# yz-cnsdqz/PSI-release

Measured on AMD Instinct MI355X. Metric: fitting iters/sec (SMPL-X+SDF+Chamfer), PROX-E batch=32, higher is better.
Workload: dtype f32

## Files before the change

### psi-release_amd/csrc/fit.hip

```cpp
#include "psi_internal.h"
#include "blob.h"
#ifdef PSI_HEAD_STOPS
__device__ int psi_dbg_sstop;
#define PSI_SSTOP(k) do { if (psi_dbg_sstop == (k)) return; } while (0)
__device__ int psi_dbg_pstop;
#define PSI_PSTOP(k) do { if (psi_dbg_pstop == (k)) asm volatile("s_endpgm"); } while (0)
__device__ int psi_dbg_cstop;
#define PSI_CSTOP() do { if (psi_dbg_cstop) asm volatile("s_endpgm"); } while (0)
#define PSI_TRACE(lo, hi) PsiBlockTrace trace_((lo), (hi))
__device__ unsigned long long psi_dbg_tl[4 * 8192];
__device__ unsigned long long psi_dbg_tlw[2 * 4 * 8192];
struct PsiBlockTrace {
    unsigned long long t0;
    int kind;
    int sel_lo, sel_hi;
    __device__ PsiBlockTrace(int lo = 9, int hi = 10) : t0(wall_clock64()), kind(0), sel_lo(lo), sel_hi(hi) {}
    __device__ ~PsiBlockTrace()
    {
        const unsigned bid = blockIdx.y * gridDim.x + blockIdx.x;
        if (psi_dbg_sstop < sel_lo || psi_dbg_sstop > sel_hi || bid >= 8192) return;
        if ((threadIdx.x & 63) == 0 && threadIdx.x < 256) {
            unsigned long long *w = psi_dbg_tlw + 2 * (4 * (size_t)bid + (threadIdx.x >> 6));
            w[0] = wall_clock64();
            w[1] = (unsigned long long)__builtin_amdgcn_s_getreg((31 << 11) | 4);
        }
        if (threadIdx.x != 0) return;
        unsigned long long *o = psi_dbg_tl + 4 * (size_t)bid;
        o[0] = t0;
        o[1] = wall_clock64();
        o[2] = (unsigned long long)__builtin_amdgcn_s_getreg((31 << 11) | 4) | ((unsigned long long)__builtin_amdgcn_s_getreg((31 << 11) | 20) << 32);
        o[3] = (unsigned long long)kind;
    }
};
extern "C" int psi_dbg_timeline(unsigned long long *out, int nblocks)
{
    return (int)hipMemcpyFromSymbol(out, HIP_SYMBOL(psi_dbg_tl), sizeof(unsigned long long) * 4 * (size_t)(nblocks < 8192 ? nblocks : 8192));
}
extern "C" int psi_dbg_timeline_waves(unsigned long long *out, int nblocks)
{
    return (int)hipMemcpyFromSymbol(out, HIP_SYMBOL(psi_dbg_tlw), sizeof(unsigned long long) * 8 * (size_t)(nblocks < 8192 ? nblocks : 8192));
}
#endif
#include "lbs_device.h"
#include "chain_plan.h"
#include "lbs_joint_device.h"
#include "sdf_device.h"
#include "nnindex_device.h"
#include <initializer_list>
#include <limits.h>
#include <memory>
#include <math.h>
#include <stdlib.h>
#include <string.h>
#include <type_traits>
#include <vector>

namespace {

constexpr int NH = 512;
constexpr int NZ = 32;
constexpr int NJ6 = 126;
constexpr int XD = 75;
#ifndef PSI_HEAD_THREADS
#define PSI_HEAD_THREADS 512
#endif
constexpr int HB = PSI_HEAD_THREADS;
static_assert(HB >= 384 && HB % 128 == 0, "the head / tail kernels place work on threads up to 256 + 75");
constexpr int KQ = HB / 128;
constexpr int KS3 = HB / 32;
constexpr int OS1 = HB / 8;
typedef float f4 __attribute__((ext_vector_type(4)));

struct FitDev {
    int B, V, Vpad, J, NB, n_c, m, D, align_corners, world, ncomp, nfp, nsdfblk;
    int indep;
    float w_rec, w_vp, w_contact, w_col, cconst;
    float lr, beta1, beta2, eps;
    float one_m_beta1, one_m_beta2;
    double lr_d, beta1_d, beta2_d;
    const float *W1T, *b1, *W2T, *b2, *W3T, *b3;
    const float *W1, *W2, *W3;
    const float *lhc, *rhc, *pose_mean;
    const int *vid;
    const int *cs_ptr, *cs_idx;
    const int *cs_first;
    const float *scene, *sdf, *gmin, *gmax;
    const float *sdf_cells;
    const float *Wct;
    float *x, *xhr, *cam, *adam_m, *adam_v;
    int *step;
    float *h1, *h2, *o6, *betas20, *pose, *transl, *verts, *og, *gq, *fpart, *penpart, *recpart, *vppart;
    float *cverts;
    float *g_betas, *g_pose, *g_transl, *g_rot;
    unsigned long long *hx_o6, *hx_gh1;
    unsigned *hx_epoch;
    int *hx_err;
    int hc;
#ifdef PSI_HEAD_STOPS
    int stop_h, stop_t;
#define HSTOP(k) do { if (f.stop_h == (k)) return; } while (0)
#define TSTOP(k) do { if (f.stop_t == (k)) return; } while (0)
#else
#define HSTOP(k)
#define TSTOP(k)
#endif
    int *nn_hint;
    float *history;
    int max_hist;
    int fused_bwd, ncp, ncp3;
    float *glc, *gvpc, *vpc;
    float *gtc_part;
#ifndef PSI_GV_SLOTS
#define PSI_GV_SLOTS 1024
#endif
    static_assert(PSI_GV_SLOTS >= 128, "one slot per body and class at least: fused_bwd runs batches up to 128 (merged_scene)");
    unsigned *gvbits;
    int gv_sps;
    const float *dirs_ch;
    const float *WTt_c;
    float *gA_part, *gfeat_part;
    float *spb;
    int nsv, nsv_c, nsn_m, nsn_c, spm, spc;
    unsigned long long *penmask;
    int pen_skip;
};

__device__ __forceinline__ float leaky(float v, float slope) { return v > 0.0f ? v : v * slope; }

__device__ __forceinline__ void gs_forward(const float *x6, float *R)
{
    float a1[3] = {x6[0], x6[2], x6[4]}, a2[3] = {x6[1], x6[3], x6[5]};
    float n1 = fmaxf(sqrtf(a1[0] * a1[0] + a1[1] * a1[1] + a1[2] * a1[2]), 1e-12f);
    float b1[3] = {a1[0] / n1, a1[1] / n1, a1[2] / n1};
    float d = b1[0] * a2[0] + b1[1] * a2[1] + b1[2] * a2[2];
    float u[3] = {a2[0] - d * b1[0], a2[1] - d * b1[1], a2[2] - d * b1[2]};
    float n2 = fmaxf(sqrtf(u[0] * u[0] + u[1] * u[1] + u[2] * u[2]), 1e-12f);
    float b2[3] = {u[0] / n2, u[1] / n2, u[2] / n2};
    float b3[3] = {b1[1] * b2[2] - b1[2] * b2[1], b1[2] * b2[0] - b1[0] * b2[2], b1[0] * b2[1] - b1[1] * b2[0]};
    for (int r = 0; r < 3; r++) {
        R[r * 3 + 0] = b1[r];
        R[r * 3 + 1] = b2[r];
        R[r * 3 + 2] = b3[r];
    }
}

__device__ __forceinline__ void gs_backward(const float *x6, const float *gR, float *g6)
{
    float a1[3] = {x6[0], x6[2], x6[4]}, a2[3] = {x6[1], x6[3], x6[5]};
    float n1 = fmaxf(sqrtf(a1[0] * a1[0] + a1[1] * a1[1] + a1[2] * a1[2]), 1e-12f);
    float b1[3] = {a1[0] / n1, a1[1] / n1, a1[2] / n1};
    float d = b1[0] * a2[0] + b1[1] * a2[1] + b1[2] * a2[2];
    float u[3] = {a2[0] - d * b1[0], a2[1] - d * b1[1], a2[2] - d * b1[2]};
    float n2 = fmaxf(sqrtf(u[0] * u[0] + u[1] * u[1] + u[2] * u[2]), 1e-12f);
    float b2[3] = {u[0] / n2, u[1] / n2, u[2] / n2};
    float gb1[3] = {gR[0], gR[3], gR[6]}, gb2[3] = {gR[1], gR[4], gR[7]}, gb3[3] = {gR[2], gR[5], gR[8]};
    gb1[0] += b2[1] * gb3[2] - b2[2] * gb3[1];
    gb1[1] += b2[2] * gb3[0] - b2[0] * gb3[2];
    gb1[2] += b2[0] * gb3[1] - b2[1] * gb3[0];
    gb2[0] += gb3[1] * b1[2] - gb3[2] * b1[1];
    gb2[1] += gb3[2] * b1[0] - gb3[0] * b1[2];
    gb2[2] += gb3[0] * b1[1] - gb3[1] * b1[0];
    float p = b2[0] * gb2[0] + b2[1] * gb2[1] + b2[2] * gb2[2];
    float gu[3] = {(gb2[0] - b2[0] * p) / n2, (gb2[1] - b2[1] * p) / n2, (gb2[2] - b2[2] * p) / n2};
    float q = gu[0] * b1[0] + gu[1] * b1[1] + gu[2] * b1[2];
    float ga2[3] = {gu[0] - b1[0] * q, gu[1] - b1[1] * q, gu[2] - b1[2] * q};
    for (int i = 0; i < 3; i++) gb1[i] += -d * gu[i] - q * a2[i];
    float r = b1[0] * gb1[0] + b1[1] * gb1[1] + b1[2] * gb1[2];
    float ga1[3] = {(gb1[0] - b1[0] * r) / n1, (gb1[1] - b1[1] * r) / n1, (gb1[2] - b1[2] * r) / n1};
    g6[0] = ga1[0]; g6[2] = ga1[1]; g6[4] = ga1[2];
    g6[1] = ga2[0]; g6[3] = ga2[1]; g6[5] = ga2[2];
}

__device__ __forceinline__ void rotmat_to_aa(const float *R, float *aa)
{
    const float m00 = R[0], m01 = R[3], m02 = R[6], m10 = R[1], m11 = R[4], m12 = R[7], m20 = R[2], m21 = R[5], m22 = R[8];
    float q[4], t;
    if (m22 < 1e-6f) {
        if (m00 > m11) {
            t = 1 + m00 - m11 - m22;
            q[0] = m12 - m21; q[1] = t; q[2] = m01 + m10; q[3] = m20 + m02;
        } else {
            t = 1 - m00 + m11 - m22;
            q[0] = m20 - m02; q[1] = m01 + m10; q[2] = t; q[3] = m12 + m21;
        }
    } else {
        if (m00 < -m11) {
            t = 1 - m00 - m11 + m22;
            q[0] = m01 - m10; q[1] = m20 + m02; q[2] = m12 + m21; q[3] = t;
        } else {
            t = 1 + m00 + m11 + m22;
            q[0] = t; q[1] = m12 - m21; q[2] = m20 - m02; q[3] = m01 - m10;
        }
    }
    float sc = sqrtf(t);
    for (int i = 0; i < 4; i++) q[i] = q[i] / sc * 0.5f;
    float s2 = q[1] * q[1] + q[2] * q[2] + q[3] * q[3];
    float s = sqrtf(s2);
    float two_theta = 2.0f * (q[0] < 0.0f ? atan2f(-s, -q[0]) : atan2f(s, q[0]));
    float k = s2 > 0.0f ? two_theta / s : 2.0f;
    aa[0] = q[1] * k; aa[1] = q[2] * k; aa[2] = q[3] * k;
}

__device__ __forceinline__ float block_sum(float v, float *sh)
{
#pragma unroll
    for (int o = 32; o > 0; o >>= 1) v += __shfl_down(v, o, 64);
    __syncthreads();
    if ((threadIdx.x & 63) == 0) sh[threadIdx.x >> 6] = v;
    __syncthreads();
    float s = 0;
    for (int i = 0; i < (int)(blockDim.x >> 6); i++) s += sh[i];
    return s;
}

__device__ __forceinline__ void block_sum2(float &a, float &c, float *sh2)
{
#pragma unroll
    for (int o = 32; o > 0; o >>= 1) {
        a += __shfl_down(a, o, 64);
        c += __shfl_down(c, o, 64);
    }
    __syncthreads();
    if ((threadIdx.x & 63) == 0) {
        sh2[2 * (threadIdx.x >> 6)] = a;
        sh2[2 * (threadIdx.x >> 6) + 1] = c;
    }
    __syncthreads();
    float sa = 0, sc = 0;
    for (int i = 0; i < (int)(blockDim.x >> 6); i++) {
        sa += sh2[2 * i];
        sc += sh2[2 * i + 1];
    }
    a = sa;
    c = sc;
}

__device__ __forceinline__ void hx_put(unsigned long long *p, float v, unsigned tag)
{
    __hip_atomic_store(p, ((unsigned long long)tag << 32) | (unsigned long long)__float_as_uint(v), __ATOMIC_RELAXED, __HIP_MEMORY_SCOPE_AGENT);
}
__device__ __forceinline__ unsigned long long hx_peek(unsigned long long *p)
{
    return __hip_atomic_load(p, __ATOMIC_RELAXED, __HIP_MEMORY_SCOPE_AGENT);
}
constexpr int HX_MAX_POLLS = 1 << 20;
__device__ __forceinline__ float hx_value(unsigned long long *p, unsigned long long w, unsigned tag, int *err)
{
    int polls = 0;
    while ((unsigned)(w >> 32) != tag) {
        if (++polls > HX_MAX_POLLS) {
            *err = 1;
            break;
        }
        __builtin_amdgcn_s_sleep(1);
        w = hx_peek(p);
    }
    return __uint_as_float((unsigned)w);
}

template <int C, bool LINKS_IN_HEAD>
__global__ __launch_bounds__(HB) void head_fwd_kernel(FitDev f, PsiLbsView lv)
{
    constexpr int NS = NH / C;
    constexpr int NQ = NS / 4;
    constexpr int KSPL = HB / NQ;
    constexpr int KPER = NH / KSPL;
    constexpr int KPER3 = NS / KS3;
    constexpr int K1 = NZ / KQ;
    constexpr int PRE2 = C > 1 ? 16 : 0;
    constexpr int PRE3 = C > 1 ? (KPER3 < 4 ? KPER3 : 4) : 0;
    static_assert(KPER % 16 == 0 && KPER3 >= 1 && NS >= 64, "cluster too wide for the thread layout");
    const int b = blockIdx.x / C, c = blockIdx.x % C, t = threadIdx.x;
    const bool last = c == C - 1;
    __shared__ float sx[XD + 5], sh1[NH], sh2[NS], so6[128], red[HB / 64], spose[PSI_JP * 3], sbetas[32], sJ[PSI_JP][3];
    __shared__ f4 part4[HB], part3[KS3][32];
    const int og1 = t & 127, kq1 = t >> 7, og2 = t % NQ, ks2 = t / NQ, og3 = t & 31, ks3 = t >> 5;
    const float *w1 = f.W1T + (size_t)(kq1 * K1) * NH + og1 * 4;
    const float *w2 = f.W2T + (size_t)(ks2 * KPER) * NH + c * NS + og2 * 4;
    const float *w3 = f.W3T + (size_t)(c * NS + ks3 * KPER3) * 128 + og3 * 4;
    f4 w1p[K1], w2p[PRE2 ? PRE2 : 1], w3p[PRE3 ? PRE3 : 1];
#pragma unroll
    for (int k = 0; k < K1; k++) w1p[k] = *(const f4 *)(w1 + (size_t)k * NH);
#pragma unroll
    for (int k = 0; k < PRE2; k++) w2p[k] = *(const f4 *)(w2 + (size_t)k * NH);
#pragma unroll
    for (int k = 0; k < PRE3; k++) w3p[k] = *(const f4 *)(w3 + (size_t)k * 128);
    const float *x = f.x + (size_t)b * XD;
    if (t < XD) sx[t] = x[t];
    if (t >= 64 && t < 96) sbetas[t - 64] = t - 64 < 10 ? x[9 + (t - 64)] : 0.0f;
    unsigned tag = 0;
    float pm[3] = {0, 0, 0}, b3v = 0.0f;
    PsiJump jp;
    for (int r = 0; r < PSI_NJUMP; r++) jp.a[r] = -1;
    if (C > 1) tag = f.hx_epoch[b] + 1u;
    f4 b1v = {0, 0, 0, 0};
    if (t < 128) b1v = *(const f4 *)(f.b1 + t * 4);
    const float b2v = t < NS ? f.b2[c * NS + t] : 0.0f;
    if (last) {
        if (t < 22)
            for (int e = 0; e < 3; e++) pm[e] = f.pose_mean[t * 3 + e];
        if (t < 128) b3v = f.b3[t];
        if (LINKS_IN_HEAD) jp = psi_load_jump(lv.m);
    }
    __syncthreads();
    HSTOP(1);
    if (c == 0) {
        float dr = t < XD ? fabsf(f.xhr[(size_t)b * XD + t] - sx[t]) : 0.0f;
        float sr = block_sum(dr, red);
        float dz = t < NZ ? sx[19 + t] * sx[19 + t] : 0.0f;
        float sz = block_sum(dz, red);
        if (t == 0) {
            f.recpart[b] = sr;
            f.vppart[b] = sz;
        }
    }
    if (last) {
        if (t >= 64 && t < 64 + 9) {
            int e = 66 + (t - 64);
            spose[e] = f.pose_mean[e];
        } else if (t >= 128 && t < 128 + 90) {
            int e = t - 128;
            const float *comp = e < 45 ? f.lhc : f.rhc;
            const float *hx = sx + (e < 45 ? 51 : 63);
            int cc = e < 45 ? e : e - 45;
            float a = 0;
            for (int i = 0; i < f.ncomp; i++) a += hx[i] * comp[i * 45 + cc];
            spose[75 + e] = a + f.pose_mean[75 + e];
        }
        psi_pose_fwd_rest(lv.m, sbetas, sJ);
    }
    HSTOP(2);
    const float *z = sx + 19;
    {
        f4 a = {0, 0, 0, 0};
#pragma unroll
        for (int k = 0; k < K1; k++) a += w1p[k] * z[kq1 * K1 + k];
        part4[kq1 * 128 + og1] = a;
    }
    __syncthreads();
    if (t < 128) {
        f4 a = b1v;
#pragma unroll
        for (int q = 0; q < KQ; q++) a += part4[q * 128 + t];
        for (int e = 0; e < 4; e++) sh1[t * 4 + e] = leaky(a[e], 0.2f);
    }
    __syncthreads();
    HSTOP(3);
    {
        f4 a0 = {0, 0, 0, 0}, a1 = {0, 0, 0, 0};
        const float *h = sh1 + ks2 * KPER;
#pragma unroll
        for (int k = 0; k < PRE2; k += 2) {
            a0 += w2p[k] * h[k];
            a1 += w2p[k + 1] * h[k + 1];
        }
#pragma unroll 8
        for (int k = PRE2; k < KPER; k += 2) {
            a0 += *(const f4 *)(w2 + (size_t)k * NH) * h[k];
            a1 += *(const f4 *)(w2 + (size_t)(k + 1) * NH) * h[k + 1];
        }
        part4[ks2 * NQ + og2] = a0 + a1;
    }
    __syncthreads();
    if (t < NS) {
        float a = b2v;
        const float *p = (const float *)part4;
#pragma unroll
        for (int q = 0; q < KSPL; q++) a += p[q * NS + t];
        a = leaky(a, 0.2f);
        sh2[t] = a;
        f.h2[(size_t)b * NH + c * NS + t] = a;
    }
    if (c == 0)
        for (int o = t; o < NH; o += HB) f.h1[(size_t)b * NH + o] = sh1[o];
    __syncthreads();
    HSTOP(4);
    {
        f4 a = {0, 0, 0, 0};
        const float *h = sh2 + ks3 * KPER3;
#pragma unroll
        for (int k = 0; k < PRE3; k++) a += w3p[k] * h[k];
#pragma unroll
        for (int k = PRE3; k < KPER3; k++) a += *(const f4 *)(w3 + (size_t)k * 128) * h[k];
        part3[ks3][og3] = a;
    }
    __syncthreads();
    HSTOP(5);
    if (t < 128) {
        float a = 0.0f;
        const float *p = (const float *)part3;
#pragma unroll
        for (int ks = 0; ks < KS3; ks++) a += p[ks * 128 + t];
        if (C == 1) {
            so6[t] = a + b3v;
        } else if (!last) {
            hx_put(f.hx_o6 + ((size_t)b * C + c) * 128 + t, a, tag);
        } else {
            unsigned long long *p8 = f.hx_o6 + (size_t)b * C * 128 + t;
            unsigned long long w[C - 1 ? C - 1 : 1];
#pragma unroll
            for (int cc = 0; cc < C - 1; cc++) w[cc] = hx_peek(p8 + cc * 128);
            float o = b3v;
#pragma unroll
            for (int cc = 0; cc < C - 1; cc++) o += hx_value(p8 + cc * 128, w[cc], tag, f.hx_err);
            so6[t] = o + a;
        }
    }
    if (C > 1 && !last) return;
    __syncthreads();
    HSTOP(6);
    if (t < NJ6) f.o6[(size_t)b * 128 + t] = so6[t];
    if (t < 22) {
        float R[9], aa[3];
        gs_forward(t == 0 ? sx + 3 : so6 + (t - 1) * 6, R);
        rotmat_to_aa(R, aa);
        for (int e = 0; e < 3; e++) spose[t * 3 + e] = aa[e] + pm[e];
    }
    __syncthreads();
    HSTOP(7);
    if constexpr (LINKS_IN_HEAD) {
        psi_pose_fwd_chain(lv.m, spose, nullptr, f.B, b, sJ, jp, lv.feat, lv.R, lv.G, lv.A, nullptr);
    } else {
        float R[9];
        psi_pose_fwd_rot(lv.m, spose, b, t, lv.feat, lv.R, R);
    }
    HSTOP(8);
    psi_pose_fwd_rest_store(lv.m, sbetas, f.B, b, sJ, lv.feat, lv.Jl);
    for (int i = t; i < f.J * 3; i += HB) f.pose[(size_t)b * f.J * 3 + i] = spose[i];
    if (t < f.NB) f.betas20[(size_t)b * f.NB + t] = sbetas[t];
    if (t >= 64 && t < 67) f.transl[(size_t)b * 3 + (t - 64)] = sx[t - 64];
    if (C > 1 && t == 0) f.hx_epoch[b] = tag;
}

struct SdfPenEpilogue {
    PsiSdfGrid G;
    const float *sdf, *gmin, *gmax;
    float *og, *penpart;
    int D, align_corners, Vpad;
    const int *contact_of;
    float s[2];
    bool neg[2];
    float *cverts;
    const int *cs_ptr, *cs_idx;
    int n_c;
    float *gl, *gvp, *gtp;
    int Npad, B;
    float gm[2][3], gs[2][3];
    float gvmax[2];
    unsigned *gmaxp;
    int gv_sps;
    unsigned long long *penmask;
    __device__ __forceinline__ void store(float *verts, size_t body_off, int b, int v, unsigned v12, float x, float y, float z) const
    {
        if (!contact_of) {
            if (verts) psi_st(verts + body_off, v12, psi_p3{x, y, z});
            return;
        }
        const int cw = psi_ld<int>(contact_of, (unsigned)v * 4u);
        if (!(cw >> 24)) return;
        float *row = cverts + (size_t)b * n_c * 3;
        psi_st(row, (unsigned)(cw & 0xffffff) * 12u, psi_p3{x, y, z});
        if ((cw >> 24) > 1)
            for (int ci = cs_ptr[v] + 1; ci < cs_ptr[v + 1]; ci++) psi_st(row, (unsigned)cs_idx[ci] * 12u, psi_p3{x, y, z});
    }
    __device__ __forceinline__ void vertex(int n, int b, int v, float x, float y, float z, bool live) { vertex_at(G, n, b, v, x, y, z, live); }
    __device__ __forceinline__ void vertex_at(const PsiSdfGrid &G, int n, int b, int v, float x, float y, float z, bool live)
    {
        s[n] = 0.0f;
        neg[n] = false;
#pragma unroll
        for (int a = 0; a < 3; a++) gm[n][a] = 0.0f;
        if (!live) return;
        float g[3];
        if (G.cells) {
            bool in[3];
            const float val = psi_sdf_sample_cells(G, x, y, z, g, in);
            neg[n] = val < 0.0f;
#pragma unroll
            for (int a = 0; a < 3; a++) g[a] = (neg[n] && in[a]) ? g[a] : 0.0f;
            s[n] = neg[n] ? -val : 0.0f;
        } else {
            const float val = psi_trilinear(sdf, gmin, gmax, x, y, z, D, align_corners, g);
            neg[n] = val < 0.0f;
#pragma unroll
            for (int a = 0; a < 3; a++) g[a] = neg[n] ? g[a] : 0.0f;
            s[n] = neg[n] ? -val : 0.0f;
        }
        if (gl) {
#pragma unroll
            for (int a = 0; a < 3; a++) gm[n][a] = g[a];
            return;
        }
        psi_st(og + (size_t)b * Vpad * 4, (unsigned)v * 16u, f4{g[0], g[1], g[2], 0.0f});
    }
    __device__ __forceinline__ void backward(int n, int b, unsigned v12, const psi_f2 (&T2)[6], const float *C)
    {
        if (!gl) return;
        const float gx = gm[n][0], gy = gm[n][1], gz = gm[n][2];
        float lx = gx, ly = gy, lz = gz;
        if (C) {
            lx = psi_dot3(C[0], C[4], C[8], gx, gy, gz);
            ly = psi_dot3(C[1], C[5], C[9], gx, gy, gz);
            lz = psi_dot3(C[2], C[6], C[10], gx, gy, gz);
        }
        psi_st(gl + (size_t)b * Npad, v12, psi_p3{lx, ly, lz});
        const float vx = psi_dot3(T2[0].x, T2[2].x, T2[4].x, lx, ly, lz), vy = psi_dot3(T2[0].y, T2[2].y, T2[4].y, lx, ly, lz),
                    vz = psi_dot3(T2[1].x, T2[3].x, T2[5].x, lx, ly, lz);
        psi_st(gvp + (size_t)b * Npad, v12, psi_p3{vx, vy, vz});
        gvmax[n] = fmaxf(gvmax[n], fmaxf(fabsf(vx), fmaxf(fabsf(vy), fabsf(vz))));
        gs[n][0] = lx; gs[n][1] = ly; gs[n][2] = lz;
    }
    __device__ __forceinline__ void finish(int n, int b, int vblock, int nvb)
    {
        __shared__ psi_f2 red[PSI_SKIN_BLK / 64];
        __shared__ float red3[PSI_SKIN_BLK / 64][3];
        __shared__ float redm[PSI_SKIN_BLK / 64];
        const float ws = psi_wave_sum(s[n]);
        const unsigned long long negm = __builtin_amdgcn_ballot_w64(neg[n]);
        const float wc = (float)(int)__builtin_popcountll(negm);
        if ((threadIdx.x & 63) == 0) red[threadIdx.x >> 6] = (psi_f2){ws, wc};
        if (gl) {
            if ((threadIdx.x & 63) == 0) penmask[((size_t)b * nvb + vblock) * (PSI_SKIN_BLK / 64) + (threadIdx.x >> 6)] = negm;
            const float sx = psi_wave_sum(gs[n][0]), sy = psi_wave_sum(gs[n][1]), sz = psi_wave_sum(gs[n][2]);
            float mx = gvmax[n];
#pragma unroll
            for (int o2 = 32; o2 > 0; o2 >>= 1) mx = fmaxf(mx, __shfl_xor(mx, o2, 64));
            if ((threadIdx.x & 63) == 0) {
                red3[threadIdx.x >> 6][0] = sx;
                red3[threadIdx.x >> 6][1] = sy;
                red3[threadIdx.x >> 6][2] = sz;
                redm[threadIdx.x >> 6] = mx;
            }
        }
        __syncthreads();
        if (gl && threadIdx.x == 64) {
            float mx = redm[0];
#pragma unroll
            for (int w = 1; w < PSI_SKIN_BLK / 64; w++) mx = fmaxf(mx, redm[w]);
            if (mx > 0.0f) atomicMax(gmaxp + (size_t)b * gv_sps + (vblock & (gv_sps - 1)), __float_as_uint(mx));
        }
        if (threadIdx.x == 0) {
            psi_f2 a = red[0];
#pragma unroll
            for (int w = 1; w < PSI_SKIN_BLK / 64; w++) a += red[w];
            *(psi_f2 *)(penpart + ((size_t)b * nvb + vblock) * 2) = a;
        }
        if (gl && threadIdx.x < 3) {
            float a = 0.0f;
#pragma unroll
            for (int w = 0; w < PSI_SKIN_BLK / 64; w++) a += red3[w][threadIdx.x];
            gtp[((size_t)vblock * B + b) * 4 + threadIdx.x] = a;
        }
    }
};

struct SdfPenEpilogueScenes : SdfPenEpilogue {
    const PsiSdfGrid *gtab;
    const int *slot;
    PsiSdfGrid Gb[2];
    template <int NB>
    __device__ __forceinline__ void load_grids(int b0, int B)
    {
#pragma unroll
        for (int n = 0; n < NB; n++) Gb[n] = gtab[slot[min(b0 + n, B - 1)]];
    }
    __device__ __forceinline__ void vertex(int n, int b, int v, float x, float y, float z, bool live) { vertex_at(Gb[n], n, b, v, x, y, z, live); }
};

template <bool SCENES>
using SdfEpilogue = std::conditional_t<SCENES, SdfPenEpilogueScenes, SdfPenEpilogue>;

template <bool SCENES>
static inline SdfEpilogue<SCENES> make_sdf_epilogue(const FitDev &f, const PsiSdfGrid &G, bool contact_vertices_only, const PsiLbsView *bwd,
                                                    const PsiSdfGrid *gtab = nullptr, const int *slot = nullptr)
{
    SdfEpilogue<SCENES> e;
    static_cast<SdfPenEpilogue &>(e) = {SCENES ? PsiSdfGrid{} : G, f.sdf, f.gmin, f.gmax, f.og, f.penpart, f.D, f.align_corners, f.Vpad,
                                        contact_vertices_only ? f.cs_first : nullptr, {0.0f, 0.0f}, {false, false}, f.cverts, f.cs_ptr, f.cs_idx, f.n_c,
                                        nullptr, nullptr, nullptr, 0, f.B, {}, {}, {0.0f, 0.0f}, f.gvbits, f.gv_sps, nullptr};
    if (bwd) {
        e.penmask = f.penmask;
        e.gl = bwd->gl;
        e.gvp = bwd->g_vp;
        e.gtp = bwd->gt_part_w;
        e.Npad = bwd->m.Npad;
    }
    if constexpr (SCENES) {
        e.gtab = gtab;
        e.slot = slot;
        e.Gb[0] = e.Gb[1] = PsiSdfGrid{};
    }
    return e;
}

template <int LPQ>
__device__ __forceinline__ void psi_contact_part_sums(float x, float (&out)[psi_sum_parts_per_wave(LPQ)])
{
    x += psi_dpp<0xB1, 0xf>(x);
    x += psi_dpp<0x4E, 0xf>(x);
    x += psi_dpp<0x124, 0xf>(x);
    x += psi_dpp<0x128, 0xf>(x);
    x += psi_dpp<0x142, 0xa>(x);
    if (psi_sum_part_lanes(LPQ) == 64) x += psi_dpp<0x143, 0xc>(x);
#pragma unroll
    for (int p = 0; p < psi_sum_parts_per_wave(LPQ); p++)
        out[p] = __builtin_bit_cast(float, __builtin_amdgcn_readlane(__builtin_bit_cast(int, x), psi_sum_last_lane(LPQ, p)));
}

template <int LPQ, int SPW = 1>
struct ContactSkinSrc {
    static_assert(LPQ == 2 || LPQ == 4, "the query's lane group skins its own vertex with 2 or 4 lanes");
    static_assert(SPW == 1 || (SPW == 2 && LPQ == 2), "two slices per workgroup: the 2-lane search");
    static constexpr int NT = SPW * psikd::kd_threads(LPQ);
    static constexpr int NST = (PSI_JP * 6 + NT - 1) / NT;
    static constexpr int CT0 = NT == 128 ? 80 : 128;
    FitDev f;
    LbsDev m;
    const float *As, *v_posed;
    psi_f2 (*sA)[6];
    psi_f2 st[NST];
    float ct;
    int v;
    float px, py, pz;
    float *sCT;
    static constexpr int NWQ = PSI_JP / 4 - 2, NWE = 10;
    f4 wq[NWE];
    int jslot;
    float (*sTR)[9] = nullptr;
    float gvm = 0.0f;
    float gs[3] = {0.0f, 0.0f, 0.0f};
    int bq = 0;
    bool live = false;
    __device__ __forceinline__ void issue(int b, int j, bool active)
    {
        jslot = j;
        bq = b;
        live = active;
#pragma unroll
        for (int q = 0; q < NST; q++) {
            const int idx = threadIdx.x + q * NT;
            st[q] = idx < m.J * 6 ? psi_ld<psi_f2>(As + (size_t)b * m.J * 12, (unsigned)idx * 8u) : (psi_f2){0.0f, 0.0f};
        }
        const int k = (int)threadIdx.x - CT0;
        ct = 0.0f;
        if (k >= 0 && k < 12) ct = f.cam[(size_t)b * 16 + k];
        else if (k >= 12 && k < 15) ct = f.transl[(size_t)b * 3 + (k - 12)];
        v = f.vid[j];
    }
    __device__ __forceinline__ void fetch(int b)
    {
        const psi_p3 p = psi_ld<psi_p3>(v_posed + (size_t)b * m.Npad, (unsigned)v * 12u);
        px = p.x; py = p.y; pz = p.z;
        const f4 *wrow = (const f4 *)(f.Wct + (size_t)jslot * PSI_JP);
#pragma unroll
        for (int q = 0; q < NWE; q++) wq[q] = wrow[q];
    }
    __device__ __forceinline__ void prepare(int)
    {
        psi_f2 (*sA_)[6] = psi_transform_stage<1>()[0];
        __shared__ float sCT_[16];
        __shared__ float sTR_[SPW * psikd::kd_qpb(LPQ)][9];
#pragma unroll
        for (int q = 0; q < NST; q++) {
            const int idx = threadIdx.x + q * NT;
            if (idx < PSI_JP * 6) (&sA_[0][0])[idx] = st[q];
        }
        const int k = (int)threadIdx.x - CT0;
        if (k >= 0 && k < 16) sCT_[k] = ct;
        __syncthreads();
        sA = sA_;
        sCT = sCT_;
        sTR = sTR_;
    }
    __device__ __forceinline__ void point(int b, int j, int c, float &qx, float &qy, float &qz) const
    {
        if constexpr (LPQ == 2) {
            const f4 *wrow = (const f4 *)(f.Wct + (size_t)j * PSI_JP);
            psi_f2 T0 = {0.0f, 0.0f}, T1 = {0.0f, 0.0f}, U0 = {0.0f, 0.0f}, U1 = {0.0f, 0.0f};
#pragma unroll
            for (int q = 0; q < NWQ; q++) {
                const f4 w4 = q < NWE ? wq[q] : wrow[q];
#pragma unroll
                for (int t = 0; t < 4; t++) {
                    const psi_f2 w2 = {w4[t], w4[t]};
                    T0 = __builtin_elementwise_fma(w2, sA[q * 4 + t][2 * c], T0);
                    T1 = __builtin_elementwise_fma(w2, sA[q * 4 + t][2 * c + 1], T1);
                    U0 = __builtin_elementwise_fma(w2, sA[q * 4 + t][4], U0);
                    U1 = __builtin_elementwise_fma(w2, sA[q * 4 + t][5], U1);
                }
            }
            if (f.fused_bwd) {
                float *tr = sTR[threadIdx.x / LPQ];
                tr[3 * c] = T0.x; tr[3 * c + 1] = T0.y; tr[3 * c + 2] = T1.x;
                if (c == 0) { tr[6] = U0.x; tr[7] = U0.y; tr[8] = U1.x; }
                if (c == 0 && live) psi_st(f.vpc + (size_t)b * f.ncp3, (unsigned)j * 12u, psi_p3{px, py, pz});
            }
            const float xr = psi_dot3p(T0.x, T0.y, T1.x, T1.y, px, py, pz) + sCT[12 + c];
            const float xr2 = psi_dot3p(U0.x, U0.y, U1.x, U1.y, px, py, pz) + sCT[14];
            const int base = (threadIdx.x & 63) & ~1;
            const float x = __shfl(xr, base, 64), y = __shfl(xr, base + 1, 64), z = __shfl(xr2, base, 64);
            const float *C = sCT;
            qx = psi_dot3p(C[0], C[1], C[2], C[3], x, y, z);
            qy = psi_dot3p(C[4], C[5], C[6], C[7], x, y, z);
            qz = psi_dot3p(C[8], C[9], C[10], C[11], x, y, z);
            return;
        }
        const int r = c < 2 ? c : 2;
        const f4 *wrow = (const f4 *)(f.Wct + (size_t)j * PSI_JP);
        psi_f2 T0 = {0.0f, 0.0f}, T1 = {0.0f, 0.0f};
#pragma unroll
        for (int q = 0; q < NWQ; q++) {
            const f4 w4 = q < NWE ? wq[q] : wrow[q];
#pragma unroll
            for (int t = 0; t < 4; t++) {
                const psi_f2 w2 = {w4[t], w4[t]};
                T0 = __builtin_elementwise_fma(w2, sA[q * 4 + t][2 * r], T0);
                T1 = __builtin_elementwise_fma(w2, sA[q * 4 + t][2 * r + 1], T1);
            }
        }
        if (f.fused_bwd && c < 3) {
            float *tr = &sTR[threadIdx.x / LPQ][3 * c];
            tr[0] = T0.x; tr[1] = T0.y; tr[2] = T1.x;
        }
        float xr = psi_dot3p(T0.x, T0.y, T1.x, T1.y, px, py, pz) + sCT[12 + r];
        const int base = (threadIdx.x & 63) & ~3;
        const float x = __shfl(xr, base, 64), y = __shfl(xr, base + 1, 64), z = __shfl(xr, base + 2, 64);
        const float *C = sCT;
        qx = psi_dot3p(C[0], C[1], C[2], C[3], x, y, z);
        qy = psi_dot3p(C[4], C[5], C[6], C[7], x, y, z);
        qz = psi_dot3p(C[8], C[9], C[10], C[11], x, y, z);
    }
    __device__ __forceinline__ void contact_post(size_t, float gx, float gy, float gz)
    {
        if (!f.fused_bwd) return;
        const float *C = sCT;
        const float lx = psi_dot3(C[0], C[4], C[8], gx, gy, gz), ly = psi_dot3(C[1], C[5], C[9], gx, gy, gz), lz = psi_dot3(C[2], C[6], C[10], gx, gy, gz);
        const float *R = sTR[threadIdx.x / LPQ];
        const size_t row = (size_t)bq * f.ncp3;
        const unsigned off = (unsigned)jslot * 12u;
        psi_st(f.glc + row, off, psi_p3{lx, ly, lz});
        const float vx = psi_dot3(R[0], R[3], R[6], lx, ly, lz), vy = psi_dot3(R[1], R[4], R[7], lx, ly, lz), vz = psi_dot3(R[2], R[5], R[8], lx, ly, lz);
        psi_st(f.gvpc + row, off, psi_p3{vx, vy, vz});
        gvm = fmaxf(fabsf(vx), fmaxf(fabsf(vy), fabsf(vz)));
        if constexpr (LPQ != 2) psi_st(f.vpc + row, off, psi_p3{px, py, pz});
        gs[0] = lx; gs[1] = ly; gs[2] = lz;
    }
    __device__ __forceinline__ void contact_finish(int b, int bx, int nbx)
    {
        if (!f.fused_bwd) return;
        constexpr int PPW = psi_sum_parts_per_wave(LPQ);
        __shared__ float wsum3_[SPW == 2 ? 1 : psi_sum_parts(LPQ)][3];
        __shared__ float wmax_[SPW == 2 ? 1 : psi_sum_waves(LPQ)];
        float (*wsum3)[3] = wsum3_;
        float *wmax = wmax_;
        if constexpr (SPW == 2) {
            static_assert(sizeof(psi_f2) * 6 * PSI_JP >= sizeof(float) * (SPW * psi_sum_parts(LPQ) * 3 + SPW * psi_sum_waves(LPQ)), "the staging area holds both tables");
            float *dead = (float *)&psi_transform_stage<1>()[0][0][0];
            wsum3 = (float (*)[3])dead;
            wmax = dead + SPW * psi_sum_parts(LPQ) * 3;
        }
        const int pr = SPW == 2 ? (bx & 1) : 0, t0 = pr * psi_sum_wg_pair_threads(LPQ);
        float sx[PPW], sy[PPW], sz[PPW];
        psi_contact_part_sums<LPQ>(gs[0], sx);
        psi_contact_part_sums<LPQ>(gs[1], sy);
        psi_contact_part_sums<LPQ>(gs[2], sz);
        float mx = gvm;
#pragma unroll
        for (int o2 = 32; o2 > 0; o2 >>= 1) mx = fmaxf(mx, __shfl_xor(mx, o2, 64));
        if ((threadIdx.x & 63) == 0) {
#pragma unroll
            for (int p = 0; p < PPW; p++) {
                const unsigned s = SPW == 2 ? psi_sum_wg_slot(LPQ, SPW, threadIdx.x >> 6, p) : psi_sum_slot(LPQ, threadIdx.x >> 6, p);
                wsum3[s][0] = sx[p];
                wsum3[s][1] = sy[p];
                wsum3[s][2] = sz[p];
            }
            wmax[threadIdx.x >> 6] = mx;
        }
        __syncthreads();
        if ((int)threadIdx.x == t0 + 64) {
            float m2 = wmax[pr * psi_sum_waves(LPQ)];
#pragma unroll
            for (int w = 1; w < psi_sum_waves(LPQ); w++) m2 = fmaxf(m2, wmax[pr * psi_sum_waves(LPQ) + w]);
            if (m2 > 0.0f) atomicMax(f.gvbits + PSI_GV_SLOTS + (size_t)b * f.gv_sps + (bx & (f.gv_sps - 1)), __float_as_uint(m2));
        }
        if ((int)threadIdx.x >= t0 && (int)threadIdx.x < t0 + 3) {
            float a = 0.0f;
#pragma unroll
            for (int w = 0; w < psi_sum_parts(LPQ); w++) a += wsum3[pr * psi_sum_parts(LPQ) + w][(int)threadIdx.x - t0];
            f.gtc_part[((size_t)b * nbx + bx) * 4 + ((int)threadIdx.x - t0)] = a;
        }
    }
};

#ifdef PSI_HEAD_STOPS
extern "C" int psi_dbg_kd_mark(unsigned long long *out, int nblocks)
{
    return (int)hipMemcpyFromSymbol(out, HIP_SYMBOL(psi_kd_mark), sizeof(unsigned long long) * 4 * (size_t)(nblocks < 8192 ? nblocks : 8192));
}
extern "C" int psi_dbg_kd_reason(int *out) { return (int)hipMemcpyFromSymbol(out, HIP_SYMBOL(psi_kd_reason), sizeof(int) * 8); }
extern "C" int psi_dbg_kd_stat(int *out, int nblocks)
{
    return (int)hipMemcpyFromSymbol(out, HIP_SYMBOL(psi_kd_stat), sizeof(int) * 4 * (size_t)(nblocks < 8192 ? nblocks : 8192));
}
#endif
template <bool SCENES>
using SceneTrees = std::conditional_t<SCENES, const psikd::KdDev *__restrict__, psikd::KdDev>;

template <int NB, bool SCENES, int LPQ, int SPW>
__global__ __launch_bounds__(256, 6) void fwd_scene_kernel(FitDev f, LbsDev m, const float *__restrict__ As, const float *__restrict__ v_posed,
                                                           SceneTrees<SCENES> T, int n_kd, int nqb, int rows, float gscale, int skin_first, SdfEpilogue<SCENES> epi,
                                                           int *__restrict__ kd_stack)
{
    extern __shared__ int smem_i[];
#ifdef PSI_HEAD_STOPS
    if (psi_dbg_sstop == 1 && (int)blockIdx.x >= n_kd) return;
    if (psi_dbg_sstop == 2 && (int)blockIdx.x < n_kd) return;
    if (psi_dbg_sstop == 3) return;
    PsiBlockTrace trace;
    if (threadIdx.x < 4 && blockIdx.x < 8192) psi_kd_stat[4 * blockIdx.x + threadIdx.x] = 0;
    trace.kind = skin_first ? ((int)blockIdx.x >= (int)gridDim.x - n_kd) : ((int)blockIdx.x < n_kd);
#endif
    int bid = blockIdx.x;
    bool is_kd;
    if (skin_first) {
        const int n_sk = (int)gridDim.x - n_kd;
        is_kd = bid >= n_sk;
        if (is_kd) bid -= n_sk;
    } else {
        is_kd = bid < n_kd;
        if (!is_kd) bid -= n_kd;
    }
    if (is_kd) {
        const int b = bid / nqb, bx = bid % nqb;
        psikd::KdDev tree = psikd::KdDev();
        const psikd::KdDev *__restrict__ tab = nullptr;
        const int *slot = nullptr;
        if constexpr (SCENES) {
            tab = T;
            slot = epi.slot;
        } else tree = T;
        psikd::kd_query_body<LPQ, true, SCENES, SPW>(tree, ContactSkinSrc<LPQ, SPW>{f, m, As, v_posed, nullptr, {}, 0.0f, 0, 0.0f, 0.0f, 0.0f, nullptr, {}, 0}, f.n_c, (float *)nullptr, (int *)nullptr,
                                           f.cconst, gscale, f.fused_bwd ? (float *)nullptr : f.gq, f.fpart, f.nn_hint, rows, tab, slot, bx, b, SPW == 2 ? f.nfp : nqb, smem_i, kd_stack);
    } else {
        const int i = bid;
        if constexpr (SCENES) epi.template load_grids<NB>((i / f.nsdfblk) * NB, f.B);
        psi_skin_fwd_body<NB, PsiBlendCompact>(m, As, v_posed, f.transl, f.cam, f.B, f.verts, epi, i % f.nsdfblk, (i / f.nsdfblk) * NB, f.nsdfblk);
    }
}

template <int NB, bool SCENES>
__global__ __launch_bounds__(PSI_SKIN_BLK, 6) void skin_fwd_sdf_kernel(LbsDev m, const float *__restrict__ As, const float *__restrict__ v_posed,
                                                                     const float *__restrict__ transl, const float *__restrict__ cam_ext,
                                                                     int B, float *__restrict__ verts, SdfEpilogue<SCENES> epi)
{
    if constexpr (SCENES) epi.template load_grids<NB>((int)blockIdx.y * NB, B);
    psi_skin_fwd_body<NB, PsiBlendPipelined>(m, As, v_posed, transl, cam_ext, B, verts, epi, (int)blockIdx.x, (int)blockIdx.y * NB, (int)gridDim.x);
}

__global__ void contact_weight_table_kernel(const float *__restrict__ WT, int Vpad, const int *__restrict__ vid, int n_c, int J, float *__restrict__ Wct)
{
    const int i = blockIdx.x * 256 + threadIdx.x;
    if (i >= n_c * PSI_JP) return;
    const int slot = i / PSI_JP, j = i % PSI_JP;
    Wct[i] = j < J ? WT[(size_t)j * Vpad + vid[slot]] : 0.0f;
}

__global__ __launch_bounds__(1024) void loss_finalize_kernel(FitDev f, float *stats)
{
    __shared__ float red[16];
    const int t = threadIdx.x, nt = 1024;
    auto total = [&](const float *p, int n, int stride) {
        float a0 = 0, a1 = 0, a2 = 0, a3 = 0;
        int i = t;
        for (; i + 3 * nt < n; i += 4 * nt) {
            a0 += p[(size_t)i * stride];
            a1 += p[(size_t)(i + nt) * stride];
            a2 += p[(size_t)(i + 2 * nt) * stride];
            a3 += p[(size_t)(i + 3 * nt) * stride];
        }
        for (; i < n; i += nt) a0 += p[(size_t)i * stride];
        return block_sum((a0 + a1) + (a2 + a3), red);
    };
    float s_rec = total(f.recpart, f.B, 1);
    float s_vp = total(f.vppart, f.B, 1);
    float s_f = total(f.fpart, f.B * f.nfp, 1);
    float s_pen = total(f.penpart, f.B * f.nsdfblk, 2);
    float n_pen = total(f.penpart + 1, f.B * f.nsdfblk, 2);
    if (t == 0) {
        stats[0] = s_rec; stats[1] = s_vp; stats[2] = s_f; stats[3] = s_pen; stats[4] = n_pen; stats[5] = 0.0f;
        *f.step += 1;
    }
}

__device__ __forceinline__ void fit_stats_body(const FitDev &f, float *__restrict__ stats)
{
    __shared__ float red[16];
    const int t = threadIdx.x, nt = blockDim.x;
    if (f.indep) {
        float a0 = 0, a1 = 0, a2 = 0, a3 = 0;
        for (int b = t; b < f.B; b += nt) {
            a0 += f.recpart[b];
            a1 += f.vppart[b];
            float sf = 0, sp = 0, cn = 0;
            for (int k = 0; k < f.nfp; k++) sf += f.fpart[(size_t)b * f.nfp + k];
            for (int k = 0; k < f.nsdfblk; k++) {
                sp += f.penpart[2 * ((size_t)b * f.nsdfblk + k)];
                cn += f.penpart[2 * ((size_t)b * f.nsdfblk + k) + 1];
            }
            a2 += sf;
            a3 += cn > 0.0f ? sp / cn : 0.0f;
            f.spb[b] = cn > 0.0f ? -f.w_col / cn : 0.0f;
        }
        const float s0 = block_sum(a0, red), s1 = block_sum(a1, red), s2 = block_sum(a2, red), s3 = block_sum(a3, red);
        if (t == 0) {
            stats[0] = s0; stats[1] = s1; stats[2] = s2; stats[3] = s3; stats[4] = 0.0f; stats[5] = 0.0f;
            *f.step += 1;
        }
        return;
    }
    auto total = [&](const float *p, int n, int stride) {
        float a0 = 0, a1 = 0, a2 = 0, a3 = 0;
        int i = t;
        for (; i + 3 * nt < n; i += 4 * nt) {
            a0 += p[(size_t)i * stride];
            a1 += p[(size_t)(i + nt) * stride];
            a2 += p[(size_t)(i + 2 * nt) * stride];
            a3 += p[(size_t)(i + 3 * nt) * stride];
        }
        for (; i < n; i += nt) a0 += p[(size_t)i * stride];
        return block_sum((a0 + a1) + (a2 + a3), red);
    };
    const float s_rec = total(f.recpart, f.B, 1);
    const float s_vp = total(f.vppart, f.B, 1);
    const float s_f = total(f.fpart, f.B * f.nfp, 1);
    const float s_pen = total(f.penpart, f.B * f.nsdfblk, 2);
    const float n_pen = total(f.penpart + 1, f.B * f.nsdfblk, 2);
    if (t == 0) {
        stats[0] = s_rec; stats[1] = s_vp; stats[2] = s_f; stats[3] = s_pen; stats[4] = n_pen; stats[5] = 0.0f;
        *f.step += 1;
    }
}

#ifndef PSI_FIT_PF_MODEL
#define PSI_FIT_PF_MODEL 1
#endif
#ifndef PSI_FIT_PF_CONTACT
#define PSI_FIT_PF_CONTACT 2
#endif
template <int MT, int PF_MODEL, int PF_CONTACT>
__global__ __launch_bounds__(256) __attribute__((amdgpu_waves_per_eu(2, 2))) void fit_bwd_joint_kernel(
    FitDev f, LbsDev m, const float *__restrict__ g_vp, const float *__restrict__ gl, const float *__restrict__ v_posed, PsiSkaPlan ska, int n_blend,
    int kgroups, float *__restrict__ stats)
{
    const int n_ska = ska.n_ska;
    constexpr int SMEM_B = psi_blend_bwd_h_smem_f4<(MT + 1) / 2>();
    __shared__ f4 smem[SMEM_B > SKA_SMEM_F4 ? SMEM_B : SKA_SMEM_F4];
    const int bid = blockIdx.x;
#ifdef PSI_HEAD_STOPS
    PsiBlockTrace trace(11, 11);
    trace.kind = bid < n_ska ? (bid < ska.n_c ? 1 : 0) : (bid < n_ska + n_blend ? 2 : 4);
#endif
    if (bid < n_ska) {
        int sl, b0, nbody;
        psi_ska_map(ska, bid, sl, b0, nbody);
        float *part = f.gA_part + (size_t)sl * f.B * PSI_JP * 16;
        if (sl < f.nsv) {
            const PsiSkaSlice o = {m.WTt + (size_t)sl * 4 * PSI_JP * 64, gl + (size_t)sl * 768, v_posed + (size_t)sl * 768, (size_t)m.Npad, part};
            const unsigned all = (1u << min(nbody, f.B - b0)) - 1u;
            const unsigned live = f.pen_skip ? psi_pen_slice_live(f.penmask, f.Vpad / 64, sl, f.B, b0, nbody) : all;
            skin_bwd_A_zero(o, b0, all & ~live);
            if (live) skin_bwd_A_dispatch_live(o, b0, live, smem);
        } else {
            const int c = sl - f.nsv;
            const PsiSkaSlice o = {f.WTt_c + (size_t)c * 4 * PSI_JP * 64, f.glc + (size_t)c * 768, f.vpc + (size_t)c * 768, (size_t)f.ncp3, part};
            skin_bwd_A_dispatch(o, f.B, b0, nbody, smem);
        }
    } else if (bid < n_ska + n_blend) {
        int kg, slice, bg;
        psi_blend_bwd_place(bid - n_ska, kgroups, f.nsn_m + f.nsn_c, kg, slice, bg);
#ifdef PSI_HEAD_STOPS
        trace.kind = slice < f.nsn_m ? 2 : 3;
#endif
        float *part = f.gfeat_part + (size_t)slice * f.B * m.Kpad;
        const float dsc_inv = m.dirs_unscale * PSI_FEAT_SCALE;
        if (slice < f.nsn_m) {
            const PsiBlendBwdColsH o = {m.dirs_bh, g_vp, (size_t)m.Npad, m.Kpad, m.Npad / 16, f.gvbits, f.gv_sps, dsc_inv, f.pen_skip ? f.penmask : nullptr, f.Vpad / 64};
            blend_bwd_h_body<(MT + 1) / 2, PF_MODEL>(o, f.B, slice * f.spm, (slice + 1) * f.spm, part, kg, bg, smem);
        } else {
            const int c = slice - f.nsn_m;
            const PsiBlendBwdColsH o = {f.dirs_ch, f.gvpc, (size_t)f.ncp3, m.Kpad, f.ncp3 / 16, f.gvbits + PSI_GV_SLOTS, f.gv_sps, dsc_inv, nullptr, 0};
            blend_bwd_h_body<(MT + 1) / 2, PF_CONTACT>(o, f.B, c * f.spc, (c + 1) * f.spc, part, kg, bg, smem);
        }
    } else {
        fit_stats_body(f, stats);
    }
}

__global__ __launch_bounds__(256) void fit_reduce_kernel(FitDev f, PsiLbsView lv, const float *__restrict__ stats)
{
    const int B = f.B, Kpad = lv.m.Kpad;
    const long nA = (long)B * PSI_JP * 16, nF = (long)B * Kpad, nT = (long)B * 4;
    const long t = (long)blockIdx.x * 256 + threadIdx.x;
    const long i = t / PSI_RSPL;
    const int s0 = (int)(t % PSI_RSPL);
    float spg = 0.0f;
    if (!f.indep) {
        const float N = stats[4];
        spg = N > 0.0f ? -f.w_col / N : 0.0f;
    }
    if (i < nA) {
        const int b = (int)(i / (PSI_JP * 16));
        const float sp = f.indep ? f.spb[b] : spg;
        float r = 0.0f;
        if ((i & 15) < 12) {
            const float pen = psi_sum_slices_split<12>(f.gA_part + i, (size_t)nA, f.nsv, s0);
            const float con = psi_sum_slices_split<2>(f.gA_part + (size_t)f.nsv * nA + i, (size_t)nA, f.nsv_c, s0);
            r = __builtin_fmaf(sp, pen, con);
        }
        if (s0 == 0) ((float *)lv.gA)[i] = r;
    } else if (i < nA + nF) {
        const long k = i - nA;
        const int b = (int)(k / Kpad);
        const float sp = f.indep ? f.spb[b] : spg;
        const float pen = psi_sum_slices_split<8>(f.gfeat_part + k, (size_t)nF, f.nsn_m, s0);
        const float con = psi_sum_slices_split<2>(f.gfeat_part + (size_t)f.nsn_m * nF + k, (size_t)nF, f.nsn_c, s0);
        if (s0 == 0) ((float *)lv.gfeat)[k] = __builtin_fmaf(sp, pen, con);
    } else if (i < nA + nF + nT) {
        const long k = i - nA - nF;
        const int b = (int)(k >> 2), c = (int)(k & 3), cc = c < 3 ? c : 0;
        const float sp = f.indep ? f.spb[b] : spg;
        const float pen = psi_sum_slices_split<12>(lv.gt_part + (size_t)b * 4 + cc, (size_t)B * 4, lv.nvb, s0);
        const float con = psi_sum_slices_split<8>(f.gtc_part + (size_t)b * f.nfp * 4 + cc, (size_t)4, f.nfp, s0);
        if (s0 == 0 && c < 3) f.g_transl[(size_t)b * 3 + c] = __builtin_fmaf(sp, pen, con);
    }
    if (t >= 64 && t < 64 + 2 * PSI_GV_SLOTS) f.gvbits[t - 64] = 0u;
    if (t == 0) {
        const int it = *f.step - 1;
        if (it >= 0) {
            float *h = f.history + (size_t)(it % f.max_hist) * 4;
            if (f.indep) {
                h[0] = f.w_rec * stats[0] / ((float)B * XD);
                h[1] = f.w_vp * stats[1] / ((float)B * NZ);
                h[2] = f.w_contact * stats[2] / ((float)B * f.n_c);
                h[3] = f.w_col * stats[3] / (float)B;
            } else {
                const float Bg = (float)B * (float)f.world, N = stats[4];
                h[0] = f.w_rec * stats[0] / (Bg * XD);
                h[1] = f.w_vp * stats[1] / (Bg * NZ);
                h[2] = f.w_contact * stats[2] / (Bg * f.n_c);
                h[3] = N > 0.0f ? f.w_col * stats[3] / N : 0.0f;
            }
        }
    }
}

__global__ void contact_weight_tiles_kernel(const float *__restrict__ Wct, int n_c, int ncp, float *__restrict__ WTt_c)
{
    const int i = blockIdx.x * 256 + threadIdx.x;
    if (i >= ncp * PSI_JP) return;
    const int tile = i / (PSI_JP * 64), j = (i / 64) % PSI_JP, s = tile * 64 + (i & 63);
    WTt_c[i] = s < n_c ? Wct[(size_t)s * PSI_JP + j] : 0.0f;
}
__global__ void contact_dirs_h_kernel(const float *__restrict__ dirs_bh, int Kpad, const int *__restrict__ vid, int n_c, int ncp3, float *__restrict__ dirs_ch)
{
    const size_t i = (size_t)blockIdx.x * 256 + threadIdx.x, n_all = (size_t)ncp3 * Kpad;
    if (i >= n_all) return;
    const int ne = (int)(i & 7), kr = (int)((i >> 3) & 31), nh = (int)((i >> 8) & 1), KT = Kpad / 32;
    const int kt = (int)((i >> 9) % KT), s = (int)((i >> 9) / KT);
    const int n = s * 16 + nh * 8 + ne;
    const int slot = n / 3, comp = n - 3 * slot;
    _Float16 hi = (_Float16)0.0f, lo = (_Float16)0.0f;
    if (slot < n_c) {
        const int sn = 3 * vid[slot] + comp;
        const size_t so = ((((size_t)(sn >> 4) * KT + kt) * 2) * 2 + ((sn >> 3) & 1)) * 256 + (size_t)kr * 8 + (sn & 7);
        hi = ((const _Float16 *)dirs_bh)[so];
        lo = ((const _Float16 *)dirs_bh)[so + 512];
    }
    const size_t o = ((((size_t)s * KT + kt) * 2) * 2 + nh) * 256 + (size_t)kr * 8 + ne;
    ((_Float16 *)dirs_ch)[o] = hi;
    ((_Float16 *)dirs_ch)[o + 512] = lo;
}
template <bool LOCAL>
struct FitGradSource {
    FitDev f;
    float *stats;
    float N;
    float *sNb;
    int b0;
    static constexpr int NPF = 4;
    psi_f2 pp[NPF];
    bool pp_valid;
    struct Pre { float og[3], q[3]; int cw; };
    __device__ __forceinline__ Pre issue(int b, int v, bool live)
    {
        Pre p;
        p.cw = live ? psi_ld<int>(f.cs_first, (unsigned)v * 4u) : 0;
        for (int e = 0; e < 3; e++) { p.og[e] = 0.0f; p.q[e] = 0.0f; }
        if (live) {
            const f4 o = psi_ld<f4>(f.og + (size_t)b * f.Vpad * 4, (unsigned)v * 16u);
            p.og[0] = o.x; p.og[1] = o.y; p.og[2] = o.z;
        }
        pp_valid = LOCAL && !f.indep;
        if (pp_valid) {
            const int n = f.B * f.nsdfblk;
#pragma unroll
            for (int k = 0; k < NPF; k++) {
                const int i = threadIdx.x + k * PSI_SKIN_BLK;
                pp[k] = i < n ? *(const psi_f2 *)(f.penpart + 2 * (size_t)i) : (psi_f2){0.0f, 0.0f};
            }
        }
        return p;
    }
    __device__ __forceinline__ void issue_late(Pre &p, int b) const
    {
        if (p.cw >> 24) {
            const psi_p3 q = psi_ld<psi_p3>(f.gq + (size_t)b * f.n_c * 3, (unsigned)(p.cw & 0xffffff) * 12u);
            p.q[0] = q.x; p.q[1] = q.y; p.q[2] = q.z;
        }
    }
    __device__ __forceinline__ void take(const Pre &p, int b, int v, float &gx, float &gy, float &gz) const
    {
        const float Nb = sNb ? sNb[b - b0] : N;
        const float sp = Nb > 0.0f ? -f.w_col / Nb : 0.0f;
        gx = sp * p.og[0]; gy = sp * p.og[1]; gz = sp * p.og[2];
        const int cnt = p.cw >> 24;
        if (cnt) { gx += p.q[0]; gy += p.q[1]; gz += p.q[2]; }
        if (cnt > 1)
            for (int ci = f.cs_ptr[v] + 1; ci < f.cs_ptr[v + 1]; ci++) {
                const float *q = f.gq + ((size_t)b * f.n_c + f.cs_idx[ci]) * 3;
                gx += q[0]; gy += q[1]; gz += q[2];
            }
    }
    __device__ __forceinline__ void prepare(int b0_, int nb)
    {
        const int t = threadIdx.x;
        const bool first = blockIdx.x == 0 && blockIdx.y == 0;
        b0 = b0_;
        sNb = nullptr;
        __shared__ float red[4];
        if (f.indep) {
            __shared__ float sN[PSI_SKIN_MB];
            for (int i0 = 0; i0 < nb; i0 += PSI_SKIN_BLK / 64) {
                const int i = i0 + (t >> 6);
                float c = 0.0f;
                if (i < nb)
                    for (int k = t & 63; k < f.nsdfblk; k += 64) c += f.penpart[2 * ((size_t)(b0 + i) * f.nsdfblk + k) + 1];
                c = psi_wave_sum(c);
                if (i < nb && (t & 63) == 0) sN[i] = c;
            }
            __syncthreads();
            sNb = sN;
            N = 0.0f;
            if (first) {
                float a0 = 0, a1 = 0, a2 = 0, a3 = 0;
                for (int b = t; b < f.B; b += PSI_SKIN_BLK) {
                    a0 += f.recpart[b];
                    a1 += f.vppart[b];
                    float sf = 0, sp = 0, cn = 0;
                    for (int k = 0; k < f.nfp; k++) sf += f.fpart[(size_t)b * f.nfp + k];
                    for (int k = 0; k < f.nsdfblk; k++) {
                        sp += f.penpart[2 * ((size_t)b * f.nsdfblk + k)];
                        cn += f.penpart[2 * ((size_t)b * f.nsdfblk + k) + 1];
                    }
                    a2 += sf;
                    a3 += cn > 0.0f ? sp / cn : 0.0f;
                }
                const float s0 = block_sum(a0, red), s1 = block_sum(a1, red), s2 = block_sum(a2, red), s3 = block_sum(a3, red);
                if (t == 0) {
                    if (LOCAL) {
                        stats[0] = s0; stats[1] = s1; stats[2] = s2; stats[3] = s3; stats[4] = 0.0f; stats[5] = 0.0f;
                        *f.step += 1;
                    }
                    const int it = *f.step - 1;
                    if (it >= 0) {
                        float *h = f.history + (size_t)(it % f.max_hist) * 4;
                        h[0] = f.w_rec * s0 / ((float)f.B * XD);
                        h[1] = f.w_vp * s1 / ((float)f.B * NZ);
                        h[2] = f.w_contact * s2 / ((float)f.B * f.n_c);
                        h[3] = f.w_col * s3 / (float)f.B;
                    }
                }
            }
            return;
        }
        float st[5];
        if (LOCAL) {
            float a = 0, c = 0;
            int i = t;
            if (pp_valid) {
#pragma unroll
                for (int k = 0; k < NPF; k++) { a += pp[k].x; c += pp[k].y; }
                i += NPF * PSI_SKIN_BLK;
            }
            for (; i < f.B * f.nsdfblk; i += PSI_SKIN_BLK) {
                a += f.penpart[2 * i];
                c += f.penpart[2 * i + 1];
            }
            __shared__ float red2[2 * PSI_SKIN_BLK / 64];
            block_sum2(a, c, red2);
            st[3] = a;
            st[4] = c;
            if (first) {
                a = 0;
                for (int i = t; i < f.B; i += PSI_SKIN_BLK) a += f.recpart[i];
                st[0] = block_sum(a, red);
                a = 0;
                for (int i = t; i < f.B; i += PSI_SKIN_BLK) a += f.vppart[i];
                st[1] = block_sum(a, red);
                a = 0;
                for (int i = t; i < f.B * f.nfp; i += PSI_SKIN_BLK) a += f.fpart[i];
                st[2] = block_sum(a, red);
            }
        } else {
#pragma unroll
            for (int i = 0; i < 5; i++) st[i] = stats[i];
        }
        N = st[4];
        if (first && t == 0) {
            if (LOCAL) {
                stats[0] = st[0]; stats[1] = st[1]; stats[2] = st[2]; stats[3] = st[3]; stats[4] = st[4]; stats[5] = 0.0f;
                *f.step += 1;
            }
            const float Bg = (float)f.B * (float)f.world;
            int it = *f.step - 1;
            if (it >= 0) {
                float *h = f.history + (size_t)(it % f.max_hist) * 4;
                h[0] = f.w_rec * st[0] / (Bg * XD);
                h[1] = f.w_vp * st[1] / (Bg * NZ);
                h[2] = f.w_contact * st[2] / (Bg * f.n_c);
                h[3] = N > 0.0f ? f.w_col * st[3] / N : 0.0f;
            }
        }
    }
    __device__ __forceinline__ void load(int b, int v, float &gx, float &gy, float &gz) const
    {
        const float Nb = sNb ? sNb[b - b0] : N;
        const float sp = Nb > 0.0f ? -f.w_col / Nb : 0.0f;
        const f4 o = *(const f4 *)(f.og + ((size_t)b * f.Vpad + v) * 4);
        gx = sp * o.x; gy = sp * o.y; gz = sp * o.z;
        for (int ci = f.cs_ptr[v]; ci < f.cs_ptr[v + 1]; ci++) {
            const float *q = f.gq + ((size_t)b * f.n_c + f.cs_idx[ci]) * 3;
            gx += q[0]; gy += q[1]; gz += q[2];
        }
    }
};

template <int C, bool ADAM>
__global__ __launch_bounds__(HB) void head_bwd_adam_kernel(FitDev f, PsiLbsView lv, float *__restrict__ g_out)
{
    constexpr int NS = NH / C, NQ = NS / 4;
    constexpr int OSPL = HB / NQ;
    constexpr int OPER = 128 / OSPL;
    constexpr int RPER = NS / KQ;
    constexpr int O1 = NH / OS1;
    constexpr int PRE3 = C > 1 ? (OPER < 16 ? OPER : 16) : 0;
    constexpr int PRE2 = C > 1 ? 16 : 0;
    static_assert(RPER % 16 == 0, "cluster too wide for the thread layout");
    const int b = blockIdx.x / C, c = blockIdx.x % C, t = threadIdx.x;
    const bool last = c == C - 1;
    __shared__ float sx[XD + 5], sg6[128], sga2[NS], sga1[NH], sgx[XD + 5];
    __shared__ float sgbetas[32], sgpose[PSI_JP * 3], sgrot[PSI_JP * 9];
    __shared__ f4 part4[HB], part1[OS1][8];
    const int og3 = t % NQ, os3 = t / NQ, og2 = t & 127, kq2 = t >> 7, kg1 = t & 7, os1 = t >> 3;
    const int o0 = os3 * OPER, o1 = min(o0 + OPER, NJ6);
    const float *w3 = f.W3 + c * NS + og3 * 4;
    const float *w2 = f.W2 + (size_t)(c * NS + kq2 * RPER) * NH + og2 * 4;
    const float *w1 = f.W1 + (size_t)(os1 * O1) * NZ + kg1 * 4;
    f4 w3p[PRE3 ? PRE3 : 1], w2p[PRE2 ? PRE2 : 1], w1p[O1];
#pragma unroll
    for (int i = 0; i < PRE3; i++) w3p[i] = *(const f4 *)(w3 + (size_t)min(o0 + i, NJ6 - 1) * NH);
#pragma unroll
    for (int i = 0; i < PRE2; i++) w2p[i] = *(const f4 *)(w2 + (size_t)i * NH);
    const float *h1 = f.h1 + (size_t)b * NH, *h2 = f.h2 + (size_t)b * NH;
    const float h2v = t < NS ? h2[c * NS + t] : 0.0f;
    unsigned tag = 0;
    if (C > 1) tag = f.hx_epoch[f.B + b] + 1u;
    float h1v = 0.0f, xhrv = 0.0f, am = 0.0f, av = 0.0f, step_size = 0.0f, bc2_sqrt = 1.0f;
    int step = 0;
    const int ta = (int)threadIdx.x - 256;
    float o6v[6] = {0, 0, 0, 0, 0, 0}, gtv = 0.0f;
    if (t >= 1 && t < 22)
        for (int i = 0; i < 6; i++) o6v[i] = f.o6[(size_t)b * 128 + (t - 1) * 6 + i];
    if (t >= 128 && t < 128 + 3) gtv = f.g_transl[(size_t)b * 3 + (t - 128)];
    TSTOP(1);
    if (last) {
#pragma unroll
        for (int i = 0; i < O1; i++) w1p[i] = *(const f4 *)(w1 + (size_t)i * NZ);
        h1v = h1[t];
        if (ADAM && ta >= 0 && ta < XD) {
            xhrv = f.xhr[(size_t)b * XD + ta];
            am = f.adam_m[(size_t)b * XD + ta];
            av = f.adam_v[(size_t)b * XD + ta];
            step = *f.step;
            const double bc1 = 1.0 - pow(f.beta1_d, (double)step);
            const double bc2 = 1.0 - pow(f.beta2_d, (double)step);
            step_size = (float)(f.lr_d / bc1);
            bc2_sqrt = (float)sqrt(bc2);
        }
    }
    psi_pose_bwd_body(lv.m, f.pose + (size_t)b * f.J * 3, lv.R, lv.Jl, lv.G, lv.gA + (size_t)b * PSI_JP * 16, lv.gfeat + (size_t)b * lv.m.Kpad, b,
                      sgbetas, sgpose, sgrot);
    const float *x = f.x + (size_t)b * XD;
    if (t < XD) { sx[t] = x[t]; sgx[t] = 0.0f; }
    if (t < 128) sg6[t] = 0.0f;
    __syncthreads();
    TSTOP(2);
    if (c == 0) {
        for (int i = t; i < f.J * 9; i += HB) f.g_rot[(size_t)b * f.J * 9 + i] = sgrot[i];
        for (int i = t; i < f.J * 3; i += HB) f.g_pose[(size_t)b * f.J * 3 + i] = sgpose[i];
        if (t < f.NB) f.g_betas[(size_t)b * f.NB + t] = sgbetas[t];
    }
    if (t == 0) {
        float g6[6];
        gs_backward(sx + 3, sgrot, g6);
        for (int i = 0; i < 6; i++) sgx[3 + i] = g6[i];
    } else if (t >= 1 && t < 22) {
        float g6[6];
        gs_backward(o6v, sgrot + t * 9, g6);
        for (int i = 0; i < 6; i++) sg6[(t - 1) * 6 + i] = g6[i];
    } else if (t >= 64 && t < 64 + 2 * f.ncomp) {
        int i = t - 64;
        const float *comp = i < f.ncomp ? f.lhc : f.rhc;
        int ii = i < f.ncomp ? i : i - f.ncomp;
        const float *gp = sgpose + (i < f.ncomp ? 75 : 120);
        float a = 0;
        for (int e = 0; e < 45; e++) a += comp[ii * 45 + e] * gp[e];
        sgx[(i < f.ncomp ? 51 : 63) + ii] = a;
    } else if (t >= 128 && t < 128 + 3) {
        sgx[t - 128] = gtv;
    } else if (t >= 160 && t < 160 + 10) {
        sgx[9 + (t - 160)] = sgbetas[t - 160];
    }
    __syncthreads();
    TSTOP(3);
    {
        f4 a = {0, 0, 0, 0};
#pragma unroll
        for (int i = 0; i < PRE3; i++) a += w3p[i] * sg6[o0 + i];
#pragma unroll 8
        for (int o = o0 + PRE3; o < o1; o++) a += *(const f4 *)(w3 + (size_t)o * NH) * sg6[o];
        part4[os3 * NQ + og3] = a;
    }
    __syncthreads();
    if (t < NS) {
        float a = 0.0f;
        const float *p = (const float *)part4;
#pragma unroll
        for (int q = 0; q < OSPL; q++) a += p[q * NS + t];
        sga2[t] = a * (h2v > 0.0f ? 1.0f : 0.2f);
    }
    __syncthreads();
    TSTOP(4);
    {
        f4 a0 = {0, 0, 0, 0}, a1 = {0, 0, 0, 0};
        const float *g = sga2 + kq2 * RPER;
#pragma unroll
        for (int o = 0; o < PRE2; o += 2) {
            a0 += w2p[o] * g[o];
            a1 += w2p[o + 1] * g[o + 1];
        }
#pragma unroll 8
        for (int o = PRE2; o < RPER; o += 2) {
            a0 += *(const f4 *)(w2 + (size_t)o * NH) * g[o];
            a1 += *(const f4 *)(w2 + (size_t)(o + 1) * NH) * g[o + 1];
        }
        part4[kq2 * 128 + og2] = a0 + a1;
    }
    __syncthreads();
    TSTOP(5);
    {
        const float *p = (const float *)part4;
        float a = p[t];
#pragma unroll
        for (int q = 1; q < KQ; q++) a += p[q * NH + t];
        if (C == 1) {
            sga1[t] = a * (h1[t] > 0.0f ? 1.0f : 0.2f);
        } else if (!last) {
            hx_put(f.hx_gh1 + ((size_t)b * C + c) * NH + t, a, tag);
            return;
        } else {
            unsigned long long *p8 = f.hx_gh1 + (size_t)b * C * NH + t;
            unsigned long long w[C - 1 ? C - 1 : 1];
#pragma unroll
            for (int cc = 0; cc < C - 1; cc++) w[cc] = hx_peek(p8 + (size_t)cc * NH);
            float o = 0.0f;
#pragma unroll
            for (int cc = 0; cc < C - 1; cc++) o += hx_value(p8 + (size_t)cc * NH, w[cc], tag, f.hx_err);
            sga1[t] = (o + a) * (h1v > 0.0f ? 1.0f : 0.2f);
        }
    }
    __syncthreads();
    TSTOP(6);
    {
        f4 a = {0, 0, 0, 0};
        if (C == 1) {
#pragma unroll
            for (int i = 0; i < O1; i++) a += *(const f4 *)(w1 + (size_t)i * NZ) * sga1[os1 * O1 + i];
        } else {
#pragma unroll
            for (int i = 0; i < O1; i++) a += w1p[i] * sga1[os1 * O1 + i];
        }
        part1[os1][kg1] = a;
    }
    __syncthreads();
    if (t < 8) {
        f4 a = {0, 0, 0, 0};
        for (int os = 0; os < OS1; os++) a += part1[os][t];
        for (int e = 0; e < 4; e++) sgx[19 + t * 4 + e] = a[e];
    }
    __syncthreads();
    TSTOP(7);
    if (C > 1 && t == 0) f.hx_epoch[f.B + b] = tag;
    if (!ADAM) {
        if (t < XD) g_out[(size_t)b * XD + t] = sgx[t];
        return;
    }
    if (ta >= 0 && ta < XD) {
        const float Bg = f.indep ? 1.0f : (float)f.B * (float)f.world;
        float g = sgx[ta];
        float df = xhrv - sx[ta];
        g += f.w_rec / (Bg * XD) * (df > 0.0f ? -1.0f : (df < 0.0f ? 1.0f : 0.0f));
        if (ta >= 19 && ta < 19 + NZ) g += f.w_vp / (Bg * NZ) * 2.0f * sx[ta];
        size_t o = (size_t)b * XD + ta;
        float m = am * f.beta1 + f.one_m_beta1 * g;
        float v = av * f.beta2 + f.one_m_beta2 * g * g;
        f.adam_m[o] = m;
        f.adam_v[o] = v;
        float denom = sqrtf(v) / bc2_sqrt + f.eps;
        f.x[o] = sx[ta] - step_size * (m / denom);
    }
}

__global__ void sdf_to_cells_kernel(const float *__restrict__ src, float *__restrict__ dst, int D)
{
    const int nbr = D >> 2;
    const size_t i = (size_t)blockIdx.x * 256 + threadIdx.x, n = (size_t)D * D * D * 8;
    if (i >= n) return;
    const int c = (int)(i & 7), l = (int)((i >> 3) & 63);
    const size_t br = i >> 9;
    const int bz = (int)(br % nbr), by = (int)((br / nbr) % nbr), bx = (int)(br / ((size_t)nbr * nbr));
    const int ix = min(4 * bx + (l >> 4) + (c >> 2), D - 1), iy = min(4 * by + ((l >> 2) & 3) + ((c >> 1) & 1), D - 1),
              iz = min(4 * bz + (l & 3) + (c & 1), D - 1);
    dst[i] = src[((size_t)ix * D + iy) * D + iz];
}

__global__ void scene_slots_kernel(const int *__restrict__ src, int *__restrict__ dst, int B, int S)
{
    const int b = blockIdx.x * 256 + threadIdx.x;
    if (b < B) dst[b] = min(max(src[b], 0), S - 1);
}

__global__ void adam_reset_kernel(float *m, float *v, int *step, int n)
{
    int i = blockIdx.x * 256 + threadIdx.x;
    if (i < n) { m[i] = 0.0f; v[i] = 0.0f; }
    if (i == 0) *step = 0;
}

}

#ifndef PSI_FIT_SEARCH_LANES_DEFAULT
#define PSI_FIT_SEARCH_LANES_DEFAULT 2
#endif
#ifndef PSI_GRAPH_UNROLL
#define PSI_GRAPH_UNROLL 10
#endif
constexpr int GRAPH_UNROLL = PSI_GRAPH_UNROLL;

struct FitKnobs {
    bool split_scene, keep_verts, no_fused_bwd, sdf_linear, scene_skin_first, bwdv_mb, no_pen_skip, bwd_pf1, chain_in_head;
    int head_cluster, skin_nb, ska_nbody, search_lanes, search_spw;
#ifdef PSI_HEAD_STOPS
    int head_stop, tail_stop, skin_stop;
#endif
};

static FitKnobs fit_read_knobs()
{
    auto is = [](const char *name, char c) { const char *v = getenv(name); return v && v[0] == c; };
    auto num = [](const char *name) { const char *v = getenv(name); return v ? atoi(v) : 0; };
    FitKnobs k = {};
    k.split_scene = is("PSI_SPLIT_SCENE", '1');
    k.keep_verts = is("PSI_KEEP_VERTS", '1');
    k.no_fused_bwd = is("PSI_FIT_FUSED_BWD", '0');
    k.no_pen_skip = is("PSI_FIT_PEN_SKIP", '0');
    k.bwd_pf1 = is("PSI_FIT_BWD_PF", '1');
    k.chain_in_head = is("PSI_FIT_CHAIN_IN_HEAD", '1');
    k.sdf_linear = is("PSI_SDF_LINEAR", '1');
    k.scene_skin_first = is("PSI_SCENE_ORDER", '1');
    k.bwdv_mb = is("PSI_BWDV_MB", '1');
    const int hc = num("PSI_HEAD_CLUSTER");
    if (hc == 1 || hc == 2 || hc == 4 || hc == 8) k.head_cluster = hc;
    if (getenv("PSI_SKIN_NB")) k.skin_nb = num("PSI_SKIN_NB") == 2 ? 2 : 1;
    k.ska_nbody = psi_ska_nbody_override(SKA_NBODY);
    const int sl = num("PSI_FIT_SEARCH_LANES");
    if (sl == 2 || sl == 4) k.search_lanes = sl;
    if (num("PSI_FIT_SEARCH_SPW") == 1) k.search_spw = 1;
#ifdef PSI_HEAD_STOPS
    k.head_stop = num("PSI_HEAD_STOP");
    k.tail_stop = num("PSI_TAIL_STOP");
    k.skin_stop = num("PSI_SKIN_STOP");
#endif
    return k;
}

struct FitModes {
    bool self_skin;
    bool merged_scene;
    bool keep_verts;
    bool fused_bwd;
    int skin_nb;
    int search_lanes;
    int search_spw;
    int hc;
    int gv_sps;
    PsiStreamSplit split;
    PsiChainPlan chain;
};

static FitModes fit_decide(const psi_fit_config *cfg, const FitKnobs &knobs, int J, int ncp3, const PsiLbsCounts &mc, int cus)
{
    FitModes d = {};
    d.self_skin = cfg->nn_mode == 1 && J <= PSI_JP - 8 && psikd::kd_qpb(psikd::LPQ_OPS) == psikd::kd_qpb(2);
    d.search_lanes = knobs.search_lanes ? knobs.search_lanes : mc.compressed_weights ? 4 : PSI_FIT_SEARCH_LANES_DEFAULT;
    d.merged_scene = d.self_skin && cfg->B <= 128 && !knobs.split_scene;
    d.search_spw = d.search_lanes == 2 && !knobs.search_spw ? 2 : 1;
    d.keep_verts = !d.merged_scene || knobs.keep_verts;
    const long bodies = (long)cfg->B * (cfg->concurrent_engines > 1 ? cfg->concurrent_engines : 1);
    d.hc = bodies <= 32 ? 8 : bodies <= 64 ? 4 : bodies <= 128 ? 2 : 1;
    if (knobs.head_cluster) d.hc = knobs.head_cluster;
    d.gv_sps = 16;
    while (d.gv_sps > 1 && (long)d.gv_sps * cfg->B > PSI_GV_SLOTS) d.gv_sps >>= 1;
    d.split = psi_stream_split(mc.Npad / 16, ncp3 / 16, mc.nsn);
    d.fused_bwd = d.merged_scene && !knobs.no_fused_bwd && d.split.nsn_c > 0;
    d.skin_nb = cfg->B > 128 && !mc.compressed_weights ? 2 : 1;
    if (knobs.skin_nb) d.skin_nb = knobs.skin_nb;
    d.chain = knobs.chain_in_head ? PsiChainPlan{0, 0} : psi_chain_plan(cfg->B, d.hc, mc.blend_wg, mc.blend_gy, cus);
    return d;
}

struct FitPlan {
    int mt;
    int kgroups, n_blend;
    PsiSkaPlan ska;
    bool pf1;
};
static FitPlan fit_plan_make(const FitDev &f, const LbsDev &m, int ska_nbody_override, bool pf1)
{
    FitPlan p;
    p.kgroups = m.Kpad / 64;
    p.mt = f.B > 32 ? 4 : (f.B > 16 ? 2 : 1);
    p.n_blend = p.kgroups * (f.nsn_m + f.nsn_c) * psi_cdiv(f.B, 16 * p.mt);
    p.ska = psi_ska_plan(f.B, f.nsv, f.nsv_c, SKA_NBODY, ska_nbody_override);
    p.pf1 = pf1;
    return p;
}

struct FitGraph { hipGraph_t g; hipGraphExec_t exec; bool ready; };

struct FitCaptured {
    enum Kind { Ok, Refused, Error } kind;
    int rc;
};

template <class Seq>
static FitCaptured fit_graph_capture(FitGraph *G, hipStream_t st, Seq &&seq)
{
    auto failed = [](const char *what, hipError_t he) {
        psi_set_error("%s failed: %s", what, hipGetErrorString(he));
        return FitCaptured{FitCaptured::Error, (int)he};
    };
    if (!st) {
        psi_set_error("invalid argument: graph capture needs a non-default stream");
        return {FitCaptured::Error, PSI_EINVAL};
    }
    hipError_t he = hipStreamBeginCapture(st, hipStreamCaptureModeRelaxed);
    if (he != hipSuccess) return failed("begin of the stream capture", he);
    const int rc = seq();
    hipGraph_t g = nullptr;
    he = hipStreamEndCapture(st, &g);
    if (!rc && he == hipSuccess) {
        he = hipGraphInstantiate(&G->exec, g, nullptr, nullptr, 0);
        if (he != hipSuccess) {
            (void)hipGraphDestroy(g);
            return failed("hipGraphInstantiate", he);
        }
        G->g = g;
        G->ready = true;
        return {FitCaptured::Ok, 0};
    }
    if (g) (void)hipGraphDestroy(g);
    if (!rc) (void)failed("hipStreamEndCapture", he);
    const bool refused = (he >= hipErrorStreamCaptureUnsupported && he <= hipErrorStreamCaptureWrongThread) || rc == 1000 + 4 || rc == 1000 + 5;
    return {refused ? FitCaptured::Refused : FitCaptured::Error, rc ? rc : (int)he};
}

static int fit_graph_launch(const FitGraph &G, hipStream_t st)
{
    PSI_CHECK_HIP(hipGraphLaunch(G.exec, st));
    return 0;
}

static void fit_graph_drop(FitGraph *G)
{
    if (G->ready) {
        (void)hipGraphExecDestroy(G->exec);
        (void)hipGraphDestroy(G->g);
    }
    *G = FitGraph{};
}

struct FitGraphTier { int iters; FitGraph *graph; };

template <class Seq>
static FitCaptured fit_run_graphs(hipStream_t st, int n_iter, int *done, std::initializer_list<FitGraphTier> tiers, Seq &&one)
{
    for (const FitGraphTier &t : tiers) {
        if (n_iter - *done < t.iters) continue;
        if (!t.graph->ready) {
            const FitCaptured c = fit_graph_capture(t.graph, st, [&]() {
                int rc = 0;
                for (int i = 0; i < t.iters && !rc; i++) rc = one();
                return rc;
            });
            if (c.kind != FitCaptured::Ok) return c;
        }
        for (; *done + t.iters <= n_iter; *done += t.iters)
            if (int rc = fit_graph_launch(*t.graph, st)) return {FitCaptured::Error, rc};
    }
    return {FitCaptured::Ok, 0};
}

enum {
    FIT_G_ITER_1, FIT_G_ITER_N, FIT_G_ITER_2N,
    FIT_G_HALF_FWD, FIT_G_HALF_BWD,
    FIT_G_DP_1, FIT_G_DP_N,
    FIT_N_GRAPHS
};

struct psi_fit_engine {
    FitDev d;
    PsiSdfGrid grid;
    const psi_lbs_model *lbs;
    psi_nn_index *nn_index;
    float *lbs_ws;
    PsiLbsView lv;
    void *nn_ws;
    char *blob;
    PsiBlob table;
    float *stats_local;
    FitKnobs knobs;
    FitModes mode;
    FitPlan plan;
    int n_scenes;
    psi_nn_index **scene_index;
    float **scene_vol;
    char *scene_blob;
    psikd::KdDev *d_kd_tab;
    PsiSdfGrid *d_grid_tab;
    int *d_slot;
    int kd_rows;
    char *search_blob;
    int *kd_stack;
    FitGraph graphs[FIT_N_GRAPHS];
    const float *half_stats[2];
    const void *dp_comm;
    const float *dp_stats;
    bool dp_warm;
    bool dp_no_graph;
};

template <bool LINKS_IN_HEAD>
static void launch_head_fwd(const FitDev &f, const PsiLbsView &lv, hipStream_t st)
{
    const dim3 g(f.B * f.hc), blk(HB);
    switch (f.hc) {
    case 8: hipLaunchKernelGGL((head_fwd_kernel<8, LINKS_IN_HEAD>), g, blk, 0, st, f, lv); break;
    case 4: hipLaunchKernelGGL((head_fwd_kernel<4, LINKS_IN_HEAD>), g, blk, 0, st, f, lv); break;
    case 2: hipLaunchKernelGGL((head_fwd_kernel<2, LINKS_IN_HEAD>), g, blk, 0, st, f, lv); break;
    default: hipLaunchKernelGGL((head_fwd_kernel<1, true>), g, blk, 0, st, f, lv); break;
    }
}

static int fit_head_blend(psi_fit_engine *e, hipStream_t st)
{
    const FitDev &f = e->d;
    const PsiChainPlan &cp = e->mode.chain;
    const bool role = cp.n_links_wg > 0 && f.hc > 1;
    if (role) launch_head_fwd<false>(f, e->lv, st);
    else launch_head_fwd<true>(f, e->lv, st);
    PSI_CHECK_LAUNCH("head_fwd_kernel");
    psi_mark("head_fwd_kernel", st);
    return role ? psi_lbs_blend_forward_links(e->lbs, f.B, e->lbs_ws, cp.n_links_wg, cp.bodies_per_wave, st)
                : psi_lbs_blend_forward(e->lbs, f.B, e->lbs_ws, st);
}

template <bool ADAM>
static void launch_head_bwd(const FitDev &f, const PsiLbsView &lv, float *g_out, hipStream_t st)
{
    const dim3 g(f.B * f.hc), blk(HB);
    switch (f.hc) {
    case 8: hipLaunchKernelGGL((head_bwd_adam_kernel<8, ADAM>), g, blk, 0, st, f, lv, g_out); break;
    case 4: hipLaunchKernelGGL((head_bwd_adam_kernel<4, ADAM>), g, blk, 0, st, f, lv, g_out); break;
    case 2: hipLaunchKernelGGL((head_bwd_adam_kernel<2, ADAM>), g, blk, 0, st, f, lv, g_out); break;
    default: hipLaunchKernelGGL((head_bwd_adam_kernel<1, ADAM>), g, blk, 0, st, f, lv, g_out); break;
    }
}

enum class FitStats {
    Finalize,
    Backward,
    Caller
};

static inline FitStats fit_stats_source(const psi_fit_engine *e, FitStats wish)
{
    return wish == FitStats::Backward && !e->mode.fused_bwd && e->d.B >= PSI_SKIN_MB_MIN_B ? FitStats::Finalize : wish;
}

static int fit_launch_stats(psi_fit_engine *e, float *stats, hipStream_t st)
{
    hipLaunchKernelGGL(loss_finalize_kernel, dim3(1), dim3(1024), 0, st, e->d, stats);
    PSI_CHECK_LAUNCH("loss_finalize_kernel");
    psi_mark("loss_finalize_kernel", st);
    return 0;
}

template <int NB, bool SCENES, int LPQ, int SPW>
static void launch_fwd_scene(const psi_fit_engine *e, float gscale, hipStream_t st)
{
    const FitDev &f = e->d;
    const int nqb = psi_cdiv(f.nfp, SPW), n_kd = nqb * f.B, skin_first = e->knobs.scene_skin_first ? 1 : 0;
    const dim3 grid(n_kd + f.nsdfblk * psi_cdiv(f.B, NB));
    FitDev fk = f;
    if (!e->mode.keep_verts) fk.verts = nullptr;
    const auto epi = make_sdf_epilogue<SCENES>(f, e->grid, false, e->mode.fused_bwd ? &e->lv : nullptr, e->d_grid_tab, e->d_slot);
    SceneTrees<SCENES> T;
    int rows;
    if constexpr (SCENES) {
        T = e->d_kd_tab;
        rows = e->kd_rows;
    } else {
        T = psi_nn_index_dev(e->nn_index);
        rows = T.rows;
    }
    hipLaunchKernelGGL((fwd_scene_kernel<NB, SCENES, LPQ, SPW>), grid, dim3(256), psikd::kd_lds_bytes(LPQ, rows), st, fk, e->lv.m, e->lv.A, e->lv.v_posed, T, n_kd, nqb, rows,
                       gscale, skin_first, epi, e->kd_stack);
}

template <int NB, bool SCENES>
static void launch_skin_fwd_sdf(const psi_fit_engine *e, bool all_verts, hipStream_t st)
{
    const FitDev &f = e->d;
    hipLaunchKernelGGL((skin_fwd_sdf_kernel<NB, SCENES>), dim3(f.nsdfblk, psi_cdiv(f.B, NB)), dim3(PSI_SKIN_BLK), 0, st, e->lv.m, e->lv.A, e->lv.v_posed,
                       f.transl, f.cam, f.B, f.verts, make_sdf_epilogue<SCENES>(f, e->grid, !all_verts, nullptr, e->d_grid_tab, e->d_slot));
}

template <class L>
static void fit_scene_dispatch(const psi_fit_engine *e, L &&launch)
{
    using One = std::integral_constant<int, 1>;
    using Two = std::integral_constant<int, 2>;
    switch ((e->n_scenes ? 2 : 0) | (e->mode.skin_nb == 2 ? 1 : 0)) {
    case 0: launch(One{}, std::false_type{}); break;
    case 1: launch(Two{}, std::false_type{}); break;
    case 2: launch(One{}, std::true_type{}); break;
    default: launch(Two{}, std::true_type{}); break;
    }
}

static int fit_forward(psi_fit_engine *e, float *stats, hipStream_t st, FitStats who)
{
    FitDev &f = e->d;
    int rc = fit_head_blend(e, st);
    if (rc) return rc;
    float gscale = f.w_contact / ((f.indep ? 1.0f : (float)f.B * (float)f.world) * (float)f.n_c);
    if (e->nn_index && e->mode.merged_scene) {
        fit_scene_dispatch(e, [&](auto nb, auto scenes) {
            if (e->mode.search_lanes == 2 && e->mode.search_spw == 2) launch_fwd_scene<decltype(nb)::value, decltype(scenes)::value, 2, 2>(e, gscale, st);
            else if (e->mode.search_lanes == 2) launch_fwd_scene<decltype(nb)::value, decltype(scenes)::value, 2, 1>(e, gscale, st);
            else launch_fwd_scene<decltype(nb)::value, decltype(scenes)::value, 4, 1>(e, gscale, st);
        });
        PSI_CHECK_LAUNCH("fwd_scene_kernel");
        psi_mark("fwd_scene_kernel", st);
    } else {
        const bool all_verts = !e->nn_index || e->knobs.keep_verts;
        fit_scene_dispatch(e, [&](auto nb, auto scenes) { launch_skin_fwd_sdf<decltype(nb)::value, decltype(scenes)::value>(e, all_verts, st); });
        PSI_CHECK_LAUNCH("skin_fwd_sdf_kernel");
        psi_mark("skin_fwd_sdf_kernel", st);
        if (e->n_scenes)
            rc = psi_nn_index_contact_set(e->d_kd_tab, e->d_slot, e->kd_rows, all_verts ? f.verts : f.cverts, all_verts ? (long)f.V * 3 : (long)f.n_c * 3,
                                          all_verts ? f.vid : nullptr, f.B, f.n_c, f.cconst, gscale, f.gq, f.fpart, f.nn_hint, st);
        else if (e->nn_index && !all_verts)
            rc = psi_nn_index_contact(e->nn_index, f.cverts, (long)f.n_c * 3, nullptr, f.B, f.n_c, f.cconst, gscale, f.gq, f.fpart, f.nn_hint, st);
        else if (e->nn_index)
            rc = psi_nn_index_contact(e->nn_index, f.verts, (long)f.V * 3, f.vid, f.B, f.n_c, f.cconst, gscale, f.gq, f.fpart, f.nn_hint, st);
        else
            rc = psi_nn_contact(f.verts, (long)f.V * 3, f.vid, f.scene, f.B, f.n_c, f.m, e->nn_ws, f.cconst, gscale, f.gq, f.fpart, nullptr, st);
        if (rc) return rc;
    }
    return fit_stats_source(e, who) == FitStats::Finalize ? fit_launch_stats(e, stats, st) : 0;
}

static int fit_backward_joint(psi_fit_engine *e, float *stats, hipStream_t st, FitStats who)
{
    FitDev &f = e->d;
    const FitPlan &p = e->plan;
    const dim3 grid(p.ska.n_ska + p.n_blend + (fit_stats_source(e, who) == FitStats::Backward ? 1 : 0));
#define PSI_LAUNCH_FIT_JOINT(MT_, PFM_, PFC_)                                                                                      \
    hipLaunchKernelGGL((fit_bwd_joint_kernel<MT_, PFM_, PFC_>), grid, dim3(256), 0, st, f, e->lv.m, e->lv.g_vp, e->lv.gl, e->lv.v_posed, p.ska, p.n_blend, p.kgroups, stats)
#define PSI_LAUNCH_FIT_JOINT_MT(MT_)                                                                                               \
    do {                                                                                                                           \
        if (p.pf1) PSI_LAUNCH_FIT_JOINT(MT_, 1, 1);                                                                                \
        else PSI_LAUNCH_FIT_JOINT(MT_, PSI_FIT_PF_MODEL, PSI_FIT_PF_CONTACT);                                                      \
    } while (0)
    if (p.mt == 4) PSI_LAUNCH_FIT_JOINT_MT(4);
    else if (p.mt == 2) PSI_LAUNCH_FIT_JOINT_MT(2);
    else PSI_LAUNCH_FIT_JOINT_MT(1);
#undef PSI_LAUNCH_FIT_JOINT_MT
#undef PSI_LAUNCH_FIT_JOINT
    PSI_CHECK_LAUNCH("fit_bwd_joint_kernel");
    psi_mark("bwd_joint_kernel", st);
    return 0;
}

static int fit_backward_tail(psi_fit_engine *e, float *stats, hipStream_t st)
{
    FitDev &f = e->d;
    const long nred = (long)f.B * PSI_JP * 16 + (long)f.B * e->lv.m.Kpad + (long)f.B * 4;
    hipLaunchKernelGGL(fit_reduce_kernel, dim3(psi_cdiv(nred * PSI_RSPL, 256)), dim3(256), 0, st, f, e->lv, stats);
    PSI_CHECK_LAUNCH("fit_reduce_kernel");
    psi_mark("reduce_partials_kernel", st);
    launch_head_bwd<true>(f, e->lv, nullptr, st);
    PSI_CHECK_LAUNCH("head_bwd_adam_kernel");
    psi_mark("head_bwd_adam_kernel", st);
    return 0;
}

static int fit_backward(psi_fit_engine *e, float *stats, hipStream_t st, FitStats who)
{
    FitDev &f = e->d;
    if (e->mode.fused_bwd) {
        int rc = fit_backward_joint(e, stats, st, who);
        return rc ? rc : fit_backward_tail(e, stats, st);
    }
    const bool big = f.B >= PSI_SKIN_MB_MIN_B;
    const bool mb = big && (e->lv.m.Wc || e->knobs.bwdv_mb);
    const dim3 bgrid(f.nsdfblk, mb ? psi_cdiv(f.B, PSI_SKIN_MB) : f.B);
#define PSI_LAUNCH_BWD_V(...)                                                                                                      \
    hipLaunchKernelGGL((psi_skin_bwd_v_kernel<__VA_ARGS__>), bgrid, dim3(PSI_SKIN_BLK), 0, st, e->lv.m, e->lv.A, src, f.cam, f.B, e->lv.gl, e->lv.g_vp, e->lv.gt_part_w)
    if (fit_stats_source(e, who) == FitStats::Backward) {
        const FitGradSource<true> src{f, stats, 0.0f, nullptr, 0, {}, false};
        if (mb) psi_launch_skin_bwd_v_mb(e->lv.m, e->lv.A, src, f.cam, f.B, e->lv.gl, e->lv.g_vp, e->lv.gt_part_w, st);
        else PSI_LAUNCH_BWD_V(FitGradSource<true>);
    } else {
        const FitGradSource<false> src{f, stats, 0.0f, nullptr, 0, {}, false};
        if (mb) psi_launch_skin_bwd_v_mb(e->lv.m, e->lv.A, src, f.cam, f.B, e->lv.gl, e->lv.g_vp, e->lv.gt_part_w, st);
        else if (big) PSI_LAUNCH_BWD_V(FitGradSource<false>, PsiBlendPipelined);
        else PSI_LAUNCH_BWD_V(FitGradSource<false>);
    }
#undef PSI_LAUNCH_BWD_V
    PSI_CHECK_LAUNCH("skin_bwd_v_grad_kernel");
    psi_mark("skin_bwd_v_grad_kernel", st);
    int rc = psi_lbs_backward_joint_parts(e->lbs, f.B, e->lbs_ws, f.g_transl, st);
    if (rc) return rc;
    launch_head_bwd<true>(f, e->lv, nullptr, st);
    PSI_CHECK_LAUNCH("head_bwd_adam_kernel");
    psi_mark("head_bwd_adam_kernel", st);
    return 0;
}

static int fit_build_scenes(psi_fit_engine *e, const psi_fit_scene *h_scenes, int S);

static inline size_t fit_x_bytes(const FitDev &f) { return (size_t)f.B * XD * 4; }
static inline size_t fit_cam_bytes(const FitDev &f) { return (size_t)f.B * 16 * 4; }
static inline size_t fit_hint_bytes(const FitDev &f) { return (size_t)f.B * f.n_c * 4; }
static inline hipError_t fit_hints_reset(const FitDev &f, hipStream_t st) { return hipMemsetAsync(f.nn_hint, 0xff, fit_hint_bytes(f), st); }

static inline size_t sdf_cells_bytes(int D) { return (size_t)D * D * D * 32; }
static void sdf_cells_fill(const float *d_sdf, float *d_cells, int D)
{
    hipLaunchKernelGGL(sdf_to_cells_kernel, dim3((unsigned)psi_cdiv((long)(sdf_cells_bytes(D) / 4), 256)), dim3(256), 0, 0, d_sdf, d_cells, D);
}

static int fit_scene_index(psi_nn_index **out, const float *d_verts, int m, hipError_t *err)
{
    std::vector<float> hs((size_t)m * 3);
    *err = hipMemcpy(hs.data(), d_verts, hs.size() * 4, hipMemcpyDeviceToHost);
    return *err == hipSuccess ? psi_nn_index_create(out, hs.data(), m) : (int)*err;
}

template <int NB, bool SCENES, int SPW>
static size_t fwd_scene_static_lds()
{
    hipFuncAttributes a;
    if (hipFuncGetAttributes(&a, reinterpret_cast<const void *>(&fwd_scene_kernel<NB, SCENES, 2, SPW>)) != hipSuccess) {
        (void)hipGetLastError();
        return 0;
    }
    return a.sharedSizeBytes;
}
static int fit_search_shape(psi_fit_engine *e)
{
    const FitDev &f = e->d;
    const char *who = e->n_scenes ? "psi_fit_create_scenes" : "psi_fit_create";
    const int rows = e->n_scenes ? e->kd_rows : psi_nn_index_dev(e->nn_index).rows;
    int dev = 0, lds_cu = 0;
    PSI_CHECK_HIP(hipGetDevice(&dev));
    if (hipDeviceGetAttribute(&lds_cu, hipDeviceAttributeMaxSharedMemoryPerMultiprocessor, dev) != hipSuccess) {
        (void)hipGetLastError();
        lds_cu = 0;
    }
    size_t s1 = 0, s2 = 0;
    fit_scene_dispatch(e, [&](auto nb, auto scenes) {
        s1 = fwd_scene_static_lds<decltype(nb)::value, decltype(scenes)::value, 1>();
        s2 = fwd_scene_static_lds<decltype(nb)::value, decltype(scenes)::value, 2>();
    });
    e->mode.search_spw = psi_search_stack_fits(f.n_c, rows) ? psi_search_spw_for((size_t)lds_cu, s1, s2, psikd::kd_lds_bytes(2, rows), 6) : 1;
    if (e->mode.search_spw != 2) return 0;
    PsiBlob T;
    T.raw(e->kd_stack, psi_search_stack_bytes(f.B, f.n_c, rows));
    return psi_blob_realise(T, &e->search_blob, who);
}

static int fit_create(psi_fit_engine **out, const psi_lbs_model *lbs, const psi_fit_config *cfg,
                      const float *h_w1, const float *h_b1, const float *h_w2, const float *h_b2,
                      const float *h_w3, const float *h_b3, const float *h_lh_comp, const float *h_rh_comp,
                      const float *h_pose_mean, const int32_t *h_contact_ids,
                      const float *d_scene_verts, const float *d_sdf, const float *h_gmin, const float *h_gmax,
                      const psi_fit_scene *h_scenes, int S)
{
    PSI_REQUIRE(out && lbs && cfg && h_w1 && h_b1 && h_w2 && h_b2 && h_w3 && h_b3 && h_lh_comp && h_rh_comp && h_pose_mean &&
                h_contact_ids && d_scene_verts && d_sdf && h_gmin && h_gmax, "null pointer");
    int V, J, NB;
    psi_lbs_dims(lbs, &V, &J, &NB);
    PSI_REQUIRE(J == 55 && NB >= 10 && NB <= 32, "the fused engine is SMPL-X shaped (J=55, 10..32 betas)");
    PSI_REQUIRE(cfg->B > 0 && cfg->n_contact > 0 && cfg->n_contact < (1 << 24) && cfg->m_scene > 0 && cfg->D >= 2 && cfg->world_size >= 1, "bad sizes");
    PSI_REQUIRE(cfg->num_pca_comps > 0 && cfg->num_pca_comps <= 12, "1..12 hand PCA components");
    PSI_REQUIRE(!(cfg->independent_bodies && cfg->world_size > 1), "independent bodies have no cross-rank coupling: use world_size 1");
    for (int i = 0; i < 66; i++) PSI_REQUIRE(h_pose_mean[i] == 0.0f, "pose_mean must be zero for global_orient/body joints");
    for (int i = 0; i < cfg->n_contact; i++) PSI_REQUIRE(h_contact_ids[i] >= 0 && h_contact_ids[i] < V, "contact id out of range");
    PsiLbsCounts mc;
    if (int rcv = psi_lbs_counts(lbs, cfg->B, &mc)) return rcv;
    psi_fit_engine *e = new psi_fit_engine();
    std::unique_ptr<psi_fit_engine, void (*)(psi_fit_engine *)> owner(e, psi_fit_destroy);
    const FitKnobs &knobs = e->knobs = fit_read_knobs();
    e->lbs = lbs;
    FitDev &f = e->d;
    f.B = cfg->B; f.V = V; f.J = J; f.NB = NB; f.n_c = cfg->n_contact; f.m = cfg->m_scene; f.D = cfg->D;
    f.align_corners = cfg->align_corners; f.world = cfg->world_size; f.ncomp = cfg->num_pca_comps;
    f.indep = cfg->independent_bodies ? 1 : 0;
    f.w_rec = cfg->w_rec; f.w_vp = cfg->w_vposer; f.w_contact = cfg->w_contact; f.w_col = cfg->w_collision; f.cconst = cfg->contact_const;
    f.lr = cfg->lr; f.beta1 = cfg->beta1; f.beta2 = cfg->beta2; f.eps = cfg->eps;
    f.lr_d = cfg->lr_d != 0.0 ? cfg->lr_d : (double)cfg->lr;
    f.beta1_d = cfg->beta1_d != 0.0 ? cfg->beta1_d : (double)cfg->beta1;
    f.beta2_d = cfg->beta2_d != 0.0 ? cfg->beta2_d : (double)cfg->beta2;
    f.one_m_beta1 = (float)(1.0 - f.beta1_d);
    f.one_m_beta2 = (float)(1.0 - f.beta2_d);
    f.nsdfblk = psi_cdiv(V, 256);
    f.Vpad = f.nsdfblk * 256;
    f.nfp = cfg->nn_mode == 1 ? psi_nn_index_fparts(f.n_c) : psi_nn_contact_fparts(f.n_c);
    f.max_hist = cfg->max_history > 0 ? cfg->max_history : 1024;
    f.ncp = psi_cdiv(f.n_c, 256) * 256;
    f.ncp3 = 3 * f.ncp;
    f.nsv = mc.nsv;
    f.nsv_c = f.ncp / 256;
    f.scene = d_scene_verts;
    f.sdf = d_sdf;
    int dev = 0, cus = 0;
    PSI_CHECK_HIP(hipGetDevice(&dev));
    PSI_CHECK_HIP(hipDeviceGetAttribute(&cus, hipDeviceAttributeMultiprocessorCount, dev));
    const FitModes &mode = e->mode = fit_decide(cfg, knobs, J, f.ncp3, mc, cus);
    f.hc = mode.hc;
    f.gv_sps = mode.gv_sps;
    f.fused_bwd = mode.fused_bwd ? 1 : 0;
    f.pen_skip = mode.fused_bwd && !knobs.no_pen_skip ? 1 : 0;
    f.nsn_m = mode.split.nsn_m; f.nsn_c = mode.split.nsn_c; f.spm = mode.split.spm; f.spc = mode.split.spc;
#ifdef PSI_HEAD_STOPS
    f.stop_h = knobs.head_stop;
    f.stop_t = knobs.tail_stop;
    (void)hipMemcpyToSymbol(HIP_SYMBOL(psi_dbg_sstop), &knobs.skin_stop, sizeof(int));
    (void)hipMemcpyToSymbol(HIP_SYMBOL(psi_dbg_pstop), &f.stop_t, sizeof(int));
    const int cstop = knobs.head_stop == 9;
    (void)hipMemcpyToSymbol(HIP_SYMBOL(psi_dbg_cstop), &cstop, sizeof(int));
#endif
    const size_t B = (size_t)f.B;
    std::vector<float> W1T((size_t)NZ * NH), W2T((size_t)NH * NH), W3T((size_t)NH * 128, 0.0f), b3p(128, 0.0f);
    memcpy(b3p.data(), h_b3, NJ6 * 4);
    for (int o = 0; o < NH; o++) for (int k = 0; k < NZ; k++) W1T[(size_t)k * NH + o] = h_w1[(size_t)o * NZ + k];
    for (int o = 0; o < NH; o++) for (int k = 0; k < NH; k++) W2T[(size_t)k * NH + o] = h_w2[(size_t)o * NH + k];
    for (int o = 0; o < NJ6; o++) for (int k = 0; k < NH; k++) W3T[(size_t)k * 128 + o] = h_w3[(size_t)o * NH + k];
    std::vector<int> cs_ptr(V + 1, 0), cs_idx(f.n_c), cs_first(V, 0);
    for (int i = 0; i < f.n_c; i++) cs_ptr[h_contact_ids[i] + 1]++;
    for (int v = 0; v < V; v++) cs_ptr[v + 1] += cs_ptr[v];
    {
        std::vector<int> fill(cs_ptr.begin(), cs_ptr.end() - 1);
        for (int i = 0; i < f.n_c; i++) cs_idx[fill[h_contact_ids[i]]++] = i;
        for (int v = 0; v < V; v++)
            if (cs_ptr[v + 1] > cs_ptr[v]) cs_first[v] = cs_idx[cs_ptr[v]] | (std::min(cs_ptr[v + 1] - cs_ptr[v], 127) << 24);
    }
    const size_t hand_pca = (size_t)f.ncomp * 45 * 4, hidden = B * NH * 4, betas = B * NB * 4, pose = B * J * 3 * 4, transl = B * 3 * 4,
                 crows = B * f.n_c * 3 * 4, per_body = B * 4, slot_rows = B * f.ncp3 * 4;
    PsiBlob &T = e->table;
    T.upload(f.W1T, W1T.data(), W1T.size() * 4);
    T.upload(f.b1, h_b1, NH * 4);
    T.upload(f.W2T, W2T.data(), W2T.size() * 4);
    T.upload(f.b2, h_b2, NH * 4);
    T.upload(f.W3T, W3T.data(), W3T.size() * 4);
    T.upload(f.b3, b3p.data(), 128 * 4);
    T.upload(f.W1, h_w1, (size_t)NH * NZ * 4);
    T.upload(f.W2, h_w2, (size_t)NH * NH * 4);
    T.upload(f.W3, h_w3, (size_t)NJ6 * NH * 4);
    T.upload(f.lhc, h_lh_comp, hand_pca);
    T.upload(f.rhc, h_rh_comp, hand_pca);
    T.upload(f.pose_mean, h_pose_mean, (size_t)J * 3 * 4);
    T.upload(f.vid, h_contact_ids, (size_t)f.n_c * sizeof(int32_t));
    T.upload(f.cs_ptr, cs_ptr.data(), cs_ptr.size() * sizeof(int));
    T.upload(f.cs_idx, cs_idx.data(), cs_idx.size() * sizeof(int));
    T.upload(f.cs_first, cs_first.data(), cs_first.size() * sizeof(int));
    T.upload(f.gmin, h_gmin, 12);
    T.upload(f.gmax, h_gmax, 12);
    T.zero_begin = T.size;
    T.zero(f.x, fit_x_bytes(f));
    T.zero(f.xhr, fit_x_bytes(f));
    T.zero(f.cam, fit_cam_bytes(f));
    T.zero(f.adam_m, fit_x_bytes(f), "adam_m");
    T.zero(f.adam_v, fit_x_bytes(f), "adam_v");
    T.zero(f.step, 256);
    T.zero(f.h1, hidden);
    T.zero(f.h2, hidden);
    T.zero(f.o6, B * 128 * 4);
    T.zero(f.betas20, betas);
    T.zero(f.pose, pose, "pose");
    T.zero(f.transl, transl);
    T.zero(f.verts, B * V * 3 * 4, "verts");
    T.zero(f.cverts, crows);
    T.zero(f.og, B * f.Vpad * 4 * 4);
    T.zero(f.gq, crows);
    T.zero(f.fpart, B * f.nfp * 4, "fpart");
    T.zero(f.penpart, B * f.nsdfblk * 2 * 4);
    T.zero(f.recpart, per_body);
    T.zero(f.vppart, per_body);
    T.zero(f.g_betas, betas);
    T.zero(f.g_pose, pose, "g_pose");
    T.zero(f.g_transl, transl, "g_transl");
    T.zero(f.g_rot, B * J * 9 * 4, "g_rot");
    T.zero(f.history, (size_t)f.max_hist * 4 * 4);
    T.zero(e->stats_local, 256);
    T.ones(f.nn_hint, fit_hint_bytes(f), "nn_hint");
    T.zero(f.hx_o6, B * f.hc * 128 * 8);
    T.zero(f.hx_gh1, B * f.hc * NH * 8);
    T.zero(f.hx_epoch, 2 * B * 4);
    T.zero(f.Wct, (size_t)f.n_c * PSI_JP * 4);
    if (mode.fused_bwd) {
        T.zero(f.glc, slot_rows, "glc");
        T.zero(f.gvpc, slot_rows, "gvpc");
        T.zero(f.vpc, slot_rows, "vpc");
        T.zero(f.gtc_part, B * f.nfp * 4 * 4, "gtc_part");
        T.zero(f.gvbits, 2 * PSI_GV_SLOTS * 4);
        T.zero(f.WTt_c, (size_t)f.ncp * PSI_JP * 4);
        T.zero(f.dirs_ch, (size_t)f.ncp3 * mc.Kpad * 4);
        T.zero(f.gA_part, (size_t)(f.nsv + f.nsv_c) * B * PSI_JP * 16 * 4);
        T.zero(f.gfeat_part, (size_t)(f.nsn_m + f.nsn_c) * B * mc.Kpad * 4);
        T.zero(f.spb, per_body, "spb");
        T.zero(f.penmask, B * (f.Vpad / 64) * 8, "penmask");
    }
    const bool cells = !h_scenes && psi_sdf_cells_fit(f.D) && !knobs.sdf_linear;
    if (cells) T.zero(f.sdf_cells, sdf_cells_bytes(f.D));
    T.zero(e->lbs_ws, psi_lbs_workspace_floats(lbs, f.B) * 4);
    T.zero(e->nn_ws, psi_nn_ws_bytes(f.B, f.n_c, f.m));
    if (int rc = psi_blob_realise(T, &e->blob, "psi_fit_create")) return rc;
    f.hx_err = f.step + 1;
    if (int rcv = psi_lbs_view(lbs, f.B, e->lbs_ws, &e->lv)) return rcv;
    e->plan = fit_plan_make(f, e->lv.m, knobs.ska_nbody, knobs.bwd_pf1);
    hipLaunchKernelGGL(contact_weight_table_kernel, dim3(psi_cdiv((long)f.n_c * PSI_JP, 256)), dim3(256), 0, 0, e->lv.m.WT, e->lv.m.Vpad, f.vid,
                       f.n_c, J, (float *)f.Wct);
    if (mode.fused_bwd) {
        hipLaunchKernelGGL(contact_weight_tiles_kernel, dim3(psi_cdiv((long)f.ncp * PSI_JP, 256)), dim3(256), 0, 0, f.Wct, f.n_c, f.ncp, (float *)f.WTt_c);
        hipLaunchKernelGGL(contact_dirs_h_kernel, dim3(psi_cdiv((long)f.ncp3 * e->lv.m.Kpad, 256)), dim3(256), 0, 0, e->lv.m.dirs_bh, e->lv.m.Kpad, f.vid,
                           f.n_c, f.ncp3, (float *)f.dirs_ch);
    }
    if (cells) sdf_cells_fill(d_sdf, (float *)f.sdf_cells, f.D);
    e->grid = psi_sdf_grid_make(f.sdf_cells, h_gmin, h_gmax, f.D, f.align_corners);
    hipError_t err = hipDeviceSynchronize();
    if (err == hipSuccess) err = hipGetLastError();
    if (err != hipSuccess) {
        psi_set_error("psi_fit_create: layout kernels failed: %s", hipGetErrorString(err));
        return (int)err;
    }
    if (h_scenes) {
        if (int rc = fit_build_scenes(e, h_scenes, S)) return rc;
    } else if (cfg->nn_mode == 1) {
        if (int rc = fit_scene_index(&e->nn_index, d_scene_verts, f.m, &err)) return rc;
    }
    if (e->nn_index && mode.merged_scene && mode.search_spw == 2)
        if (int rc = fit_search_shape(e)) return rc;
    owner.release();
    *out = e;
    return 0;
}

extern "C" int psi_fit_create(psi_fit_engine **out, const psi_lbs_model *lbs, const psi_fit_config *cfg,
                              const float *h_w1, const float *h_b1, const float *h_w2, const float *h_b2,
                              const float *h_w3, const float *h_b3, const float *h_lh_comp, const float *h_rh_comp,
                              const float *h_pose_mean, const int32_t *h_contact_ids,
                              const float *d_scene_verts, const float *d_sdf, const float *h_gmin, const float *h_gmax)
{
    return fit_create(out, lbs, cfg, h_w1, h_b1, h_w2, h_b2, h_w3, h_b3, h_lh_comp, h_rh_comp, h_pose_mean, h_contact_ids, d_scene_verts, d_sdf,
                      h_gmin, h_gmax, nullptr, 0);
}

static int fit_build_scenes(psi_fit_engine *e, const psi_fit_scene *h_scenes, int S)
{
    FitDev &f = e->d;
    e->n_scenes = S;
    e->scene_index = new psi_nn_index *[S]();
    e->scene_vol = new float *[S]();
    std::vector<psikd::KdDev> kd(S);
    std::vector<PsiSdfGrid> grids(S);
    for (int s = 0; s < S; s++) {
        const psi_fit_scene &sc = h_scenes[s];
        const int D = sc.D;
        const size_t bytes = sdf_cells_bytes(D);
        hipError_t err = hipMalloc((void **)&e->scene_vol[s], bytes);
        if (err != hipSuccess) {
            (void)hipGetLastError();
            e->scene_vol[s] = nullptr;
            psi_set_error("psi_fit_create_scenes: no memory for the copy of scene %d's volume (%zu bytes, 8 x the volume): %s", s, bytes, hipGetErrorString(err));
            return PSI_ENOMEM;
        }
        sdf_cells_fill(sc.d_sdf, e->scene_vol[s], D);
        grids[s] = psi_sdf_grid_make(e->scene_vol[s], sc.gmin, sc.gmax, D, f.align_corners);
        if (int rc = fit_scene_index(&e->scene_index[s], sc.d_verts, sc.m, &err)) {
            if (err != hipSuccess) psi_set_error("psi_fit_create_scenes: reading scene %d's vertices failed: %s", s, hipGetErrorString(err));
            return rc;
        }
        kd[s] = psi_nn_index_dev(e->scene_index[s]);
        e->kd_rows = std::max(e->kd_rows, kd[s].rows);
    }
    e->nn_index = e->scene_index[0];
    PsiBlob T;
    T.upload(e->d_kd_tab, kd.data(), sizeof(psikd::KdDev) * S);
    T.upload(e->d_grid_tab, grids.data(), sizeof(PsiSdfGrid) * S);
    T.zero(e->d_slot, sizeof(int) * (size_t)f.B);
    if (int rc = psi_blob_realise(T, &e->scene_blob, "psi_fit_create_scenes")) return rc;
    hipError_t err = hipDeviceSynchronize();
    if (err == hipSuccess) err = hipGetLastError();
    if (err != hipSuccess) {
        psi_set_error("psi_fit_create_scenes: layout kernels failed: %s", hipGetErrorString(err));
        return (int)err;
    }
    return 0;
}

extern "C" int psi_fit_create_scenes(psi_fit_engine **out, const psi_lbs_model *lbs, const psi_fit_config *cfg,
                                     const float *h_w1, const float *h_b1, const float *h_w2, const float *h_b2,
                                     const float *h_w3, const float *h_b3, const float *h_lh_comp, const float *h_rh_comp,
                                     const float *h_pose_mean, const int32_t *h_contact_ids,
                                     const psi_fit_scene *h_scenes, int S)
{
    PSI_REQUIRE(out, "null pointer");
    *out = nullptr;
    PSI_REQUIRE(cfg, "null pointer");
    PSI_REQUIRE(S >= 1, "psi_fit_create_scenes: S must be at least 1");
    PSI_REQUIRE(h_scenes, "psi_fit_create_scenes: null scene table");
    PSI_REQUIRE(cfg->nn_mode == 1, "psi_fit_create_scenes: nn_mode must be 1 (there is no brute-force search over several scenes)");
    PSI_REQUIRE(cfg->world_size <= 1, "psi_fit_create_scenes: world_size > 1 (data-parallel runs over several scenes) is not supported");
    for (int s = 0; s < S; s++) {
        const psi_fit_scene &sc = h_scenes[s];
        PSI_REQUIRE(sc.d_verts && sc.d_sdf, "psi_fit_create_scenes: null scene pointer");
        PSI_REQUIRE(sc.m > 0, "psi_fit_create_scenes: a scene without vertices");
        if (!psi_sdf_cells_fit(sc.D)) {
            psi_set_error("invalid argument: psi_fit_create_scenes: D = %d of scene %d: D must be a multiple of 4, at least 4 and at most %d (the engine samples "
                          "a cell-major copy of the volume and has no plain-volume fallback)", sc.D, s, PSI_SDF_CELLS_MAX_D);
            return PSI_EINVAL;
        }
    }
    psi_fit_config c = *cfg;
    c.m_scene = h_scenes[0].m;
    c.D = h_scenes[0].D;
    c.world_size = 1;
    return fit_create(out, lbs, &c, h_w1, h_b1, h_w2, h_b2, h_w3, h_b3, h_lh_comp, h_rh_comp, h_pose_mean, h_contact_ids, h_scenes[0].d_verts,
                      h_scenes[0].d_sdf, h_scenes[0].gmin, h_scenes[0].gmax, h_scenes, S);
}

extern "C" int psi_fit_scene_count(const psi_fit_engine *e) { return e ? (e->n_scenes ? e->n_scenes : 1) : 0; }

extern "C" int psi_fit_set_scene_slots(psi_fit_engine *e, const int32_t *d_slot, void *stream)
{
    PSI_REQUIRE(e && d_slot, "null pointer");
    hipStream_t st = (hipStream_t)stream;
    hipStreamCaptureStatus cap = hipStreamCaptureStatusNone;
    PSI_CHECK_HIP(hipStreamIsCapturing(st, &cap));
    PSI_REQUIRE(cap == hipStreamCaptureStatusNone, "psi_fit_set_scene_slots: not inside a stream capture (the captured iterations read the engine's own slot buffer)");
    FitDev &f = e->d;
    if (e->n_scenes) {
        hipLaunchKernelGGL(scene_slots_kernel, dim3(psi_cdiv(f.B, 256)), dim3(256), 0, st, (const int *)d_slot, e->d_slot, f.B, e->n_scenes);
        PSI_CHECK_LAUNCH("scene_slots_kernel");
    }
    PSI_CHECK_HIP(fit_hints_reset(f, st));
    return 0;
}

extern "C" void psi_fit_destroy(psi_fit_engine *e)
{
    if (!e) return;
    if (e->scene_index) {
        for (int s = 0; s < e->n_scenes; s++)
            if (e->scene_index[s]) psi_nn_index_destroy(e->scene_index[s]);
        delete[] e->scene_index;
    } else if (e->nn_index) psi_nn_index_destroy(e->nn_index);
    if (e->scene_vol) {
        for (int s = 0; s < e->n_scenes; s++) (void)hipFree(e->scene_vol[s]);
        delete[] e->scene_vol;
    }
    (void)hipFree(e->scene_blob);
    (void)hipFree(e->search_blob);
    for (FitGraph &G : e->graphs) fit_graph_drop(&G);
    (void)hipFree(e->blob);
    delete e;
}

extern "C" int psi_fit_set_problem(psi_fit_engine *e, const float *d_xhr, const float *d_x_init, const float *d_cam_ext,
                                   int reset_optimizer, void *stream)
{
    PSI_REQUIRE(e && d_xhr && d_cam_ext, "null pointer");
    FitDev &f = e->d;
    hipStream_t st = (hipStream_t)stream;
    PSI_CHECK_HIP(hipMemcpyAsync(f.xhr, d_xhr, fit_x_bytes(f), hipMemcpyDeviceToDevice, st));
    PSI_CHECK_HIP(hipMemcpyAsync(f.x, d_x_init ? d_x_init : d_xhr, fit_x_bytes(f), hipMemcpyDeviceToDevice, st));
    PSI_CHECK_HIP(hipMemcpyAsync(f.cam, d_cam_ext, fit_cam_bytes(f), hipMemcpyDeviceToDevice, st));
    PSI_CHECK_HIP(fit_hints_reset(f, st));
    if (reset_optimizer) {
        hipLaunchKernelGGL(adam_reset_kernel, dim3(psi_cdiv((long)f.B * XD, 256)), dim3(256), 0, st, f.adam_m, f.adam_v, f.step, f.B * XD);
        PSI_CHECK_LAUNCH("adam_reset_kernel");
    psi_mark("adam_reset_kernel", st);
    }
    return 0;
}

static int fit_iteration(psi_fit_engine *e, hipStream_t st)
{
    int rc = fit_forward(e, e->stats_local, st, FitStats::Backward);
    return rc ? rc : fit_backward(e, e->stats_local, st, FitStats::Backward);
}

static int fit_half(psi_fit_engine *e, int which, float *stats, int use_graph, hipStream_t st)
{
    auto half = [&]() { return which == 0 ? fit_forward(e, stats, st, FitStats::Finalize) : fit_backward(e, stats, st, FitStats::Caller); };
    if (!use_graph) return half();
    FitGraph *G = &e->graphs[FIT_G_HALF_FWD + which];
    if (G->ready && e->half_stats[which] != stats) fit_graph_drop(G);
    if (!G->ready) {
        const FitCaptured c = fit_graph_capture(G, st, half);
        if (c.kind != FitCaptured::Ok) return c.rc;
        e->half_stats[which] = stats;
    }
    return fit_graph_launch(*G, st);
}

extern "C" int psi_fit_forward(psi_fit_engine *e, float *d_stats, int use_graph, void *stream)
{
    PSI_REQUIRE(e, "null engine");
    return fit_half(e, 0, d_stats ? d_stats : e->stats_local, use_graph, (hipStream_t)stream);
}

extern "C" int psi_fit_backward_step(psi_fit_engine *e, const float *d_stats, int use_graph, void *stream)
{
    PSI_REQUIRE(e, "null engine");
    return fit_half(e, 1, (float *)(d_stats ? d_stats : e->stats_local), use_graph, (hipStream_t)stream);
}

extern "C" int psi_fit_iterate(psi_fit_engine *e, int n_iter, int use_graph, void *stream)
{
    PSI_REQUIRE(e && n_iter >= 0, "bad arguments");
    PSI_REQUIRE(e->d.world == 1, "psi_fit_iterate is the single-process path; data-parallel runs call forward / all-reduce / backward_step");
    hipStream_t st = (hipStream_t)stream;
    auto one = [&]() { return fit_iteration(e, st); };
    int done = 0, rc = 0;
    if (!use_graph) {
        for (; done < n_iter && !rc; done++) rc = one();
        return rc;
    }
    return fit_run_graphs(st, n_iter, &done,
                          {{2 * GRAPH_UNROLL, &e->graphs[FIT_G_ITER_2N]}, {GRAPH_UNROLL, &e->graphs[FIT_G_ITER_N]}, {1, &e->graphs[FIT_G_ITER_1]}}, one).rc;
}

extern "C" int psi_fit_iterate_dp(psi_fit_engine *e, psi_dp_comm *comm, int n_iter, int use_graph, float *d_stats, void *stream)
{
    PSI_REQUIRE(e && comm && n_iter >= 0, "bad arguments");
    PSI_REQUIRE(psi_dp_world(comm) == e->d.world, "the communicator's size differs from psi_fit_config.world_size");
    hipStream_t st = (hipStream_t)stream;
    float *stats = d_stats ? d_stats : e->stats_local;
    auto one = [&]() -> int {
        if (e->mode.fused_bwd) {
            int rc = fit_forward(e, stats, st, FitStats::Backward);
            if (!rc) rc = fit_backward_joint(e, stats, st, FitStats::Backward);
            if (!rc) rc = psi_dp_allreduce_sum(comm, stats, 6, st);
            return rc ? rc : fit_backward_tail(e, stats, st);
        }
        int rc = fit_forward(e, stats, st, FitStats::Finalize);
        if (!rc) rc = psi_dp_allreduce_sum(comm, stats, 6, st);
        if (!rc) rc = fit_backward(e, stats, st, FitStats::Finalize);
        return rc;
    };
    if (e->dp_comm != comm || e->dp_stats != stats) {
        fit_graph_drop(&e->graphs[FIT_G_DP_1]);
        fit_graph_drop(&e->graphs[FIT_G_DP_N]);
        e->dp_warm = e->dp_warm && e->dp_comm == comm;
        e->dp_comm = comm;
        e->dp_stats = stats;
    }
    int done = 0;
    auto eager = [&](int upto) {
        int rc = 0;
        for (; done < upto && !rc; done++) rc = one();
        return rc;
    };
    if (!use_graph || (!e->dp_warm && n_iter > 0)) {
        if (int rc = eager(use_graph ? 1 : n_iter)) return rc;
        e->dp_warm = true;
        if (!use_graph) return 0;
    }
    if (!e->dp_no_graph) {
        const FitCaptured c = fit_run_graphs(st, n_iter, &done, {{GRAPH_UNROLL, &e->graphs[FIT_G_DP_N]}, {1, &e->graphs[FIT_G_DP_1]}}, one);
        if (c.kind != FitCaptured::Refused) return c.rc;
        (void)hipGetLastError();
        e->dp_no_graph = true;
    }
    return eager(n_iter);
}

extern "C" int psi_fit_chain_mode(const psi_fit_engine *e)
{
    return e && e->mode.chain.n_links_wg > 0 && e->d.hc > 1 ? 1 : 0;
}

extern "C" int psi_fit_dp_mode(const psi_fit_engine *e)
{
    if (!e || !e->dp_warm) return 0;
    return e->dp_no_graph ? 2 : 1;
}

extern "C" int psi_fit_decode_forward(psi_fit_engine *e, const float *d_x75, const float *d_cam_ext, float *d_verts, void *stream)
{
    PSI_REQUIRE(e && d_x75 && d_cam_ext && d_verts, "null pointer");
    FitDev &f = e->d;
    hipStream_t st = (hipStream_t)stream;
    PSI_CHECK_HIP(hipMemcpyAsync(f.x, d_x75, fit_x_bytes(f), hipMemcpyDeviceToDevice, st));
    PSI_CHECK_HIP(hipMemcpyAsync(f.cam, d_cam_ext, fit_cam_bytes(f), hipMemcpyDeviceToDevice, st));
    int rc = fit_head_blend(e, st);
    if (rc) return rc;
    hipLaunchKernelGGL(psi_skin_fwd_kernel<PsiSkinNoEpilogue>, dim3(f.nsdfblk, f.B), dim3(PSI_SKIN_BLK), 0, st, e->lv.m, e->lv.A,
                       e->lv.v_posed, f.transl, f.cam, f.B, d_verts, PsiSkinNoEpilogue());
    PSI_CHECK_LAUNCH("skin_fwd_kernel");
    return 0;
}

extern "C" int psi_fit_decode_backward(psi_fit_engine *e, const float *d_grad_verts, float *d_grad_x75, void *stream)
{
    PSI_REQUIRE(e && d_grad_verts && d_grad_x75, "null pointer");
    FitDev &f = e->d;
    hipStream_t st = (hipStream_t)stream;
    if (f.B >= PSI_SKIN_MB_MIN_B)
        psi_launch_skin_bwd_v_mb(e->lv.m, e->lv.A, PsiGradFromMemory{d_grad_verts, f.V}, f.cam, f.B, e->lv.gl, e->lv.g_vp, e->lv.gt_part_w, st);
    else
        hipLaunchKernelGGL(psi_skin_bwd_v_kernel<PsiGradFromMemory>, dim3(f.nsdfblk, f.B), dim3(PSI_SKIN_BLK), 0, st, e->lv.m, e->lv.A,
                           PsiGradFromMemory{d_grad_verts, f.V}, f.cam, f.B, e->lv.gl, e->lv.g_vp, e->lv.gt_part_w);
    PSI_CHECK_LAUNCH("skin_bwd_v_kernel");
    int rc = psi_lbs_backward_joint_parts(e->lbs, f.B, e->lbs_ws, f.g_transl, st);
    if (rc) return rc;
    launch_head_bwd<false>(f, e->lv, d_grad_x75, st);
    PSI_CHECK_LAUNCH("head_bwd_kernel");
    return 0;
}

extern "C" int psi_fit_profile(psi_fit_engine *e, int n_rep, char *h_names, int name_stride, float *h_ms, int max_stages,
                               int *h_n_stages, void *stream)
{
    PSI_REQUIRE(e && h_names && h_ms && h_n_stages && n_rep > 0 && max_stages > 0 && name_stride >= 16, "bad arguments");
    PSI_REQUIRE(e->d.world == 1, "profile the single-process path");
    hipStream_t st = (hipStream_t)stream;
    PsiStageTimer tm;
    memset(&tm, 0, sizeof(tm));
    for (int i = 0; i < 48; i++) PSI_CHECK_HIP(hipEventCreate(&tm.ev[i]));
    std::vector<double> acc(48, 0.0);
    int n_st = 0, rc = 0;
    for (int r = 0; r < n_rep && !rc; r++) {
        tm.n = 0;
        (void)hipEventRecord(tm.ev[0], st);
        tm.name[0] = "start";
        tm.n = 1;
        g_psi_timer = &tm;
        rc = fit_iteration(e, st);
        g_psi_timer = nullptr;
        if (rc) break;
        PSI_CHECK_HIP(hipStreamSynchronize(st));
        n_st = tm.n - 1;
        for (int i = 1; i < tm.n; i++) {
            float ms = 0;
            (void)hipEventElapsedTime(&ms, tm.ev[i - 1], tm.ev[i]);
            acc[i - 1] += ms;
        }
    }
    for (int i = 0; i < 48; i++) (void)hipEventDestroy(tm.ev[i]);
    if (rc) return rc;
    if (n_st > max_stages) n_st = max_stages;
    for (int i = 0; i < n_st; i++) {
        h_ms[i] = (float)(acc[i] / n_rep);
        strncpy(h_names + (size_t)i * name_stride, tm.name[i + 1], name_stride - 1);
        h_names[(size_t)i * name_stride + name_stride - 1] = 0;
    }
    *h_n_stages = n_st;
    return 0;
}

extern "C" int psi_fit_read(psi_fit_engine *e, float *d_x_out, float *d_history_out, int n_hist, int *h_step, void *stream)
{
    PSI_REQUIRE(e, "null engine");
    FitDev &f = e->d;
    hipStream_t st = (hipStream_t)stream;
    if (d_x_out) PSI_CHECK_HIP(hipMemcpyAsync(d_x_out, f.x, fit_x_bytes(f), hipMemcpyDeviceToDevice, st));
    if (d_history_out && n_hist > 0) {
        if (n_hist > f.max_hist) n_hist = f.max_hist;
        PSI_CHECK_HIP(hipMemcpyAsync(d_history_out, f.history, (size_t)n_hist * 16, hipMemcpyDeviceToDevice, st));
    }
    if (h_step) {
        int hs[2] = {0, 0};
        PSI_CHECK_HIP(hipMemcpyAsync(hs, f.step, 8, hipMemcpyDeviceToHost, st));
        PSI_CHECK_HIP(hipStreamSynchronize(st));
        *h_step = hs[0];
        if (hs[1]) {
            (void)hipMemsetAsync(f.hx_err, 0, 4, st);
            psi_set_error("psi_fit_read: a head / tail cluster exchange timed out (a producer workgroup never published its partials); "
                          "the results of this fit are invalid.  PSI_HEAD_CLUSTER=1 runs the kernels without clusters");
            return 902;
        }
    }
    return 0;
}

extern "C" int psi_fit_read_losses(psi_fit_engine *e, int adam_step, float *d_out4, void *stream)
{
    PSI_REQUIRE(e && d_out4 && adam_step >= 1, "bad arguments");
    FitDev &f = e->d;
    PSI_CHECK_HIP(hipMemcpyAsync(d_out4, f.history + (size_t)((adam_step - 1) % f.max_hist) * 4, 16, hipMemcpyDeviceToDevice, (hipStream_t)stream));
    return 0;
}

extern "C" int psi_fit_search_shape(const psi_fit_engine *e, int *lanes, int *slices, int *workgroups)
{
    PSI_REQUIRE(e && lanes && slices && workgroups, "null pointer");
    const bool shared = e->nn_index && e->mode.merged_scene;
    *lanes = shared ? e->mode.search_lanes : 0;
    *slices = shared ? e->mode.search_spw : 0;
    *workgroups = shared ? e->d.B * psi_cdiv(e->d.nfp, e->mode.search_spw) : 0;
    return 0;
}

extern "C" int psi_fit_copy_buffer(psi_fit_engine *e, const char *name, float *d_out, long n_floats, void *stream)
{
    PSI_REQUIRE(e && name && d_out && n_floats >= 0, "bad arguments");
    FitDev &f = e->d;
    const PsiLbsView &lv = e->lv;
    const float *src = nullptr;
    long cap = 0;
    if (const PsiBuf *b = e->table.find(name)) { src = (const float *)(e->blob + b->off); cap = (long)(b->bytes / 4); }
    const struct { const char *name; const float *src; long cap; } more[] = {
        {"stats", e->stats_local, 8},
        {"gA", lv.gA, (long)f.B * PSI_JP * 16},
        {"gfeat", lv.gfeat, (long)f.B * lv.m.Kpad},
        {"gl", lv.gl, (long)f.B * lv.m.Npad},
        {"g_vp", lv.g_vp, (long)f.B * lv.m.Npad},
        {"v_posed", lv.v_posed, (long)f.B * lv.m.Npad},
        {"R", lv.R, (long)f.B * lv.m.J * 12},
        {"G", lv.G, (long)f.B * lv.m.J * 12},
        {"A", lv.A, (long)f.B * lv.m.J * 12 + PSI_A_TAIL * 12},
        {"feat", lv.feat, (long)((f.B + 31) & ~31) * lv.m.Kpad},
    };
    for (const auto &b : more)
        if (!strcmp(name, b.name)) { src = b.src; cap = b.cap; }
    if (!strcmp(name, "verts") && e->nn_index) {
        hipLaunchKernelGGL(psi_skin_fwd_kernel<PsiSkinNoEpilogue>, dim3(f.nsdfblk, f.B), dim3(PSI_SKIN_BLK), 0, (hipStream_t)stream, lv.m, lv.A,
                           lv.v_posed, f.transl, f.cam, f.B, f.verts, PsiSkinNoEpilogue());
        PSI_CHECK_LAUNCH("skin_fwd_kernel");
    }
    PSI_REQUIRE(src != nullptr, "unknown buffer name");
    PSI_REQUIRE(n_floats <= cap, "buffer is smaller than requested");
    PSI_CHECK_HIP(hipMemcpyAsync(d_out, src, (size_t)n_floats * 4, hipMemcpyDeviceToDevice, (hipStream_t)stream));
    return 0;
}
```

### psi-release_amd/csrc/lbs_device.h

```cpp
#pragma once
#ifndef PSI_TRACE
#define PSI_TRACE(lo, hi)
#endif
#ifndef PSI_SSTOP
#define PSI_SSTOP(k)
#endif
#ifndef PSI_CSTOP
#define PSI_CSTOP()
#endif
#ifndef PSI_PSTOP
#define PSI_PSTOP(k)
#endif
#include <hip/hip_runtime.h>

typedef float psi_f4 __attribute__((ext_vector_type(4)));

constexpr int PSI_JP = 64;
constexpr int PSI_SUB_MAX = PSI_JP * (PSI_JP + 1) / 2;
constexpr int PSI_ITEM_MAX = 2 * PSI_JP;
constexpr int PSI_NJUMP = 6;
constexpr int PSI_WNZ = 8;
constexpr int PSI_A_TAIL = 16;

struct LbsDev {
    int V, J, NB, P, K, Kpad, N, Npad, Vpad, maxlevel, njump;
    int dirs_tile;
    float dirs_unscale;
    const float *dirs, *v_template, *WT, *J_t, *J_s;
    const float *dirs_bh;
    const float *WTt;
    const float *Wc;
    const unsigned *Wj;
    const int *parents, *level, *child_ptr, *child_idx;
    const int *jump;
    const unsigned char *sub_list;
    const unsigned int *sub_item;
    const unsigned char *sub_first;
    int n_sub, n_items;
};

struct PsiLbsView {
    LbsDev m;
    float *feat, *R, *Jl, *G, *A, *v_posed, *gl, *g_vp, *gt_part_w;
    const float *gA_part, *gfeat_part, *gt_part;
    const float *gA, *gfeat;
    int nsv, nsn, nvb;
};

__device__ __forceinline__ void psi_rodrigues(const float *aa, float *R)
{
#pragma clang fp contract(off)
    float x = aa[0] + 1e-8f, y = aa[1] + 1e-8f, z = aa[2] + 1e-8f;
    float angle = sqrtf(__builtin_fmaf(y, y, x * x) + z * z);
    float rx = aa[0] / angle, ry = aa[1] / angle, rz = aa[2] / angle;
    float s = sinf(angle), c1 = 1.0f - cosf(angle);
    const float cxy = c1 * (rx * ry), cxz = c1 * (rx * rz), cyz = c1 * (ry * rz);
    R[0] = 1.0f - c1 * __builtin_fmaf(ry, ry, rz * rz);
    R[1] = cxy - rz * s;
    R[2] = __builtin_fmaf(ry, s, cxz);
    R[3] = __builtin_fmaf(rz, s, cxy);
    R[4] = __builtin_fmaf(-(rx * rx + rz * rz), c1, 1.0f);
    R[5] = cyz - rx * s;
    R[6] = cxz - ry * s;
    R[7] = __builtin_fmaf(rx, s, cyz);
    R[8] = __builtin_fmaf(-__builtin_fmaf(ry, ry, rx * rx), c1, 1.0f);
}

__device__ __forceinline__ void psi_pose_fwd_rest(const LbsDev &m, const float *betas_b, float (*sJ)[3])
{
    for (int q = threadIdx.x; q < m.J * 3; q += blockDim.x) {
        float a = m.J_t[q];
        const float *js = m.J_s + (size_t)q * m.NB;
        for (int l = 0; l < m.NB; l++) a += js[l] * betas_b[l];
        (&sJ[0][0])[q] = a;
    }
}

constexpr float PSI_FEAT_SCALE = 16.0f;
__device__ __forceinline__ void psi_feat_store(const LbsDev &m, float *__restrict__ feat, int b, int k, float v)
{
    float x = v * PSI_FEAT_SCALE;
    x = x > 65504.0f ? 65504.0f : (x < -65504.0f ? -65504.0f : x);
    const _Float16 hi = (_Float16)x;
    const _Float16 lo = (_Float16)((x - (float)hi) * 2048.0f);
    _Float16 *o = (_Float16 *)feat + (((size_t)(b >> 5) * (m.Kpad >> 4) + (k >> 4)) * 4 + ((k >> 3) & 1)) * 256 + (size_t)(b & 31) * 8 + (k & 7);
    o[0] = hi;
    o[512] = lo;
}

__device__ __forceinline__ void psi_pose_fwd_rest_store(const LbsDev &m, const float *betas_b, int B, int b, const float (*sJ)[3],
                                                        float *__restrict__ feat, float *__restrict__ Jls)
{
    const int j = threadIdx.x, nthr = blockDim.x;
    for (int q = j; q < m.J * 3; q += nthr) Jls[(size_t)b * m.J * 3 + q] = (&sJ[0][0])[q];
    for (int l = j; l < m.NB; l += nthr) psi_feat_store(m, feat, b, l, betas_b[l]);
    for (int l = m.K + j; l < m.Kpad; l += nthr) psi_feat_store(m, feat, b, l, 0.0f);
}

struct PsiJump { int a[PSI_NJUMP]; };

__device__ __forceinline__ PsiJump psi_load_jump(const LbsDev &m)
{
    PsiJump jp;
#pragma unroll
    for (int r = 0; r < PSI_NJUMP; r++) jp.a[r] = (threadIdx.x < m.J && r < m.njump) ? m.jump[r * PSI_JP + threadIdx.x] : -1;
    return jp;
}

__device__ __forceinline__ void psi_pose_fwd_rot(const LbsDev &m, const float *pose_b, int b, int j, float *feat, float *Rs, float (&R)[9])
{
    if (j < m.J) {
        psi_rodrigues(pose_b + j * 3, R);
        psi_f4 *Ro = (psi_f4 *)(Rs + ((size_t)b * m.J + j) * 12);
        Ro[0] = psi_f4{R[0], R[1], R[2], 0.0f};
        Ro[1] = psi_f4{R[3], R[4], R[5], 0.0f};
        Ro[2] = psi_f4{R[6], R[7], R[8], 0.0f};
        if (j >= 1)
            for (int e = 0; e < 9; e++) {
                int k = m.NB + (j - 1) * 9 + e;
                psi_feat_store(m, feat, b, k, R[e] - ((e == 0 || e == 4 || e == 8) ? 1.0f : 0.0f));
            }
    }
}

__device__ __forceinline__ void psi_pose_fwd_links(const LbsDev &m, const float *transl, int B, int b, int j, int nthr, const float (&R)[9],
                                                   const float (*J3)[3], const PsiJump &jp, float (*sG)[12], int (*sJmp)[PSI_JP], float *Gs,
                                                   float *As, float *joints)
{
#pragma clang fp contract(off)
    const bool act = j < m.J;
    float Jl[3] = {0, 0, 0};
    float G[12];
    if (act) {
        const int par = jp.a[0];
        for (int c = 0; c < 3; c++) Jl[c] = J3[j][c];
        for (int r = 0; r < 3; r++) {
            for (int c = 0; c < 3; c++) G[r * 4 + c] = R[r * 3 + c];
            G[r * 4 + 3] = par >= 0 ? Jl[r] - J3[par][r] : Jl[r];
        }
        for (int e = 0; e < 12; e++) sG[j][e] = G[e];
    }
#pragma nounroll
    for (int r = 0; r < m.njump && j < 64; r++) {
        __builtin_amdgcn_wave_barrier();
        const int a = sJmp[r][j];
        float P[12];
        if (act && a >= 0)
            for (int e = 0; e < 12; e++) P[e] = sG[a][e];
        __builtin_amdgcn_wave_barrier();
        if (act && a >= 0) {
            float N[12];
            for (int q = 0; q < 3; q++) {
                const float p0 = P[q * 4 + 0], p1 = P[q * 4 + 1], p2 = P[q * 4 + 2];
                for (int c = 0; c < 2; c++) N[q * 4 + c] = __builtin_fmaf(p2, G[8 + c], __builtin_fmaf(p0, G[c], p1 * G[4 + c]));
                N[q * 4 + 2] = p2 * G[10] + (q < 2 ? __builtin_fmaf(p0, G[2], p1 * G[6]) : p0 * G[2] + p1 * G[6]);
                N[q * 4 + 3] = P[q * 4 + 3] + (q < 2 ? __builtin_fmaf(p2, G[11], __builtin_fmaf(p1, G[7], p0 * G[3]))
                                                    : p2 * G[11] + __builtin_fmaf(p0, G[3], p1 * G[7]));
            }
            for (int e = 0; e < 12; e++) { G[e] = N[e]; sG[j][e] = N[e]; }
        }
    }
    if (act) {
        psi_f4 *Go = (psi_f4 *)(Gs + ((size_t)b * m.J + j) * 12), *Ao = (psi_f4 *)(As + ((size_t)b * m.J + j) * 12);
        for (int r = 0; r < 3; r++) {
            Go[r] = psi_f4{G[r * 4 + 0], G[r * 4 + 1], G[r * 4 + 2], G[r * 4 + 3]};
            Ao[r] = psi_f4{G[r * 4 + 0], G[r * 4 + 1], G[r * 4 + 2],
                           G[r * 4 + 3] - (G[r * 4 + 2] * Jl[2] + __builtin_fmaf(G[r * 4 + 0], Jl[0], G[r * 4 + 1] * Jl[1]))};
        }
        if (joints)
            for (int r = 0; r < 3; r++) joints[((size_t)b * m.J + j) * 3 + r] = G[r * 4 + 3] + (transl ? transl[(size_t)b * 3 + r] : 0.0f);
    }
    if (b == B - 1)
        for (int q = j; q < PSI_A_TAIL * 3; q += nthr) ((psi_f4 *)(As + (size_t)B * m.J * 12))[q] = psi_f4{0.0f, 0.0f, 0.0f, 0.0f};
}

__device__ __forceinline__ void psi_pose_fwd_chain(const LbsDev &m, const float *pose_b, const float *__restrict__ transl, int B, int b,
                                                   const float (*sJ)[3], const PsiJump &jp, float *__restrict__ feat,
                                                   float *__restrict__ Rs, float *__restrict__ Gs, float *__restrict__ As,
                                                   float *__restrict__ joints)
{
    const int j = threadIdx.x;
    __shared__ float sG[PSI_JP][12];
    __shared__ int sJmp[PSI_NJUMP][PSI_JP];
    float R[9];
    if (j < PSI_JP)
#pragma unroll
        for (int r = 0; r < PSI_NJUMP; r++) sJmp[r][j] = jp.a[r];
    psi_pose_fwd_rot(m, pose_b, b, j, feat, Rs, R);
    PSI_CSTOP();
    __syncthreads();
    psi_pose_fwd_links(m, transl, B, b, j, blockDim.x, R, sJ, jp, sG, sJmp, Gs, As, joints);
}


__device__ __forceinline__ void psi_pose_fwd_body(const LbsDev &m, const float *betas_b, const float *pose_b,
                                                  const float *__restrict__ transl, int B, int b, float *__restrict__ feat,
                                                  float *__restrict__ Rs, float *__restrict__ Jls, float *__restrict__ Gs,
                                                  float *__restrict__ As, float *__restrict__ joints)
{
    __shared__ float sJ[PSI_JP][3];
    const PsiJump jp = psi_load_jump(m);
    psi_pose_fwd_rest(m, betas_b, sJ);
    __syncthreads();
    psi_pose_fwd_rest_store(m, betas_b, B, b, sJ, feat, Jls);
    psi_pose_fwd_chain(m, pose_b, transl, B, b, sJ, jp, feat, Rs, Gs, As, joints);
}


constexpr int PSI_POSE_JSP = 8;
struct PsiPoseBwdPre {
    float aa[3], js[PSI_POSE_JSP], G[12], Jl[3], P[12];
    int cp0, cp1, par;
};
struct PsiPoseBwdShared {
    float sX[PSI_JP][12];
    float sS[PSI_JP][12];
    float sP[PSI_ITEM_MAX][12];
    unsigned int sItem[PSI_ITEM_MAX];
    unsigned char sList[PSI_SUB_MAX], sFirst[PSI_JP + 1];
    float sgJ[PSI_JP][3];
    float sgrel[PSI_JP][3];
    int sChild[PSI_JP];
    float sgb[32][32];
};

__device__ __forceinline__ PsiPoseBwdPre psi_pose_bwd_issue(const LbsDev &m, const float *pose_b, const float *__restrict__ Jls,
                                                            const float *__restrict__ Gs, int b, bool want_betas, bool want_pose,
                                                            PsiPoseBwdShared &sh)
{
    const int j = threadIdx.x, nthr = blockDim.x;
    const bool act = j < m.J;
    PsiPoseBwdPre p;
    for (int e = 0; e < 3; e++) p.aa[e] = 0.0f;
    if (act && want_pose)
        for (int e = 0; e < 3; e++) p.aa[e] = pose_b[j * 3 + e];
    constexpr int JSP = PSI_POSE_JSP;
    const int nq = m.J * 3;
    const int npart = m.NB > 0 ? min(32, max(1, nthr / m.NB)) : 1;
    const int per = (nq + npart - 1) / npart;
    const bool par_ok = m.NB <= 32, js_pre = want_betas && par_ok && per <= JSP && j < npart * m.NB;
    const int bpart = m.NB > 0 ? j / m.NB : 0, bl = j - bpart * m.NB;
    for (int i = 0; i < JSP; i++) p.js[i] = 0.0f;
    if (js_pre)
        for (int i = 0; i < JSP; i++) {
            const int q = bpart * per + i;
            if (i < per && q < nq) p.js[i] = m.J_s[(size_t)q * m.NB + bl];
        }
    p.cp0 = act ? m.child_ptr[j] : 0;
    p.cp1 = act ? m.child_ptr[j + 1] : 0;
    p.par = act ? m.parents[j] : -1;
    if (j < m.J - 1) sh.sChild[j] = m.child_idx[j];
    for (int i = j; i < m.n_sub; i += nthr) sh.sList[i] = m.sub_list[i];
    for (int i = j; i < m.n_items; i += nthr) sh.sItem[i] = m.sub_item[i];
    for (int i = j; i <= m.J; i += nthr) sh.sFirst[i] = m.sub_first[i];
    for (int e = 0; e < 12; e++) { p.G[e] = 0.0f; p.P[e] = 0.0f; }
    for (int c = 0; c < 3; c++) p.Jl[c] = 0.0f;
    if (act) {
        const psi_f4 *Gp = (const psi_f4 *)(Gs + ((size_t)b * m.J + j) * 12);
        for (int r = 0; r < 3; r++) {
            const psi_f4 gg = Gp[r];
            for (int c = 0; c < 4; c++) p.G[r * 4 + c] = gg[c];
        }
        for (int c = 0; c < 3; c++) p.Jl[c] = Jls[((size_t)b * m.J + j) * 3 + c];
    }
    if (act && p.par >= 0) {
        const psi_f4 *Pp = (const psi_f4 *)(Gs + ((size_t)b * m.J + p.par) * 12);
        for (int r = 0; r < 3; r++) {
            const psi_f4 pr = Pp[r];
            for (int c = 0; c < 4; c++) p.P[r * 4 + c] = pr[c];
        }
    }
    return p;
}

__device__ __forceinline__ void psi_pose_bwd_finish(const LbsDev &m, const PsiPoseBwdPre &pre, PsiPoseBwdShared &sh, const float *gA_b,
                                                    const float *gfeat_b, float *g_betas_b, float *g_pose_b, float *g_rot_b)
{
    const int j = threadIdx.x, nthr = blockDim.x;
    const bool act = j < m.J;
    float (&sX)[PSI_JP][12] = sh.sX;
    float (&sS)[PSI_JP][12] = sh.sS;
    float (&sP)[PSI_ITEM_MAX][12] = sh.sP;
    unsigned int (&sItem)[PSI_ITEM_MAX] = sh.sItem;
    unsigned char (&sList)[PSI_SUB_MAX] = sh.sList;
    unsigned char (&sFirst)[PSI_JP + 1] = sh.sFirst;
    float (&sgJ)[PSI_JP][3] = sh.sgJ;
    float (&sgrel)[PSI_JP][3] = sh.sgrel;
    int (&sChild)[PSI_JP] = sh.sChild;
    float gf9[9];
    const float *aa = pre.aa;
    for (int e = 0; e < 9; e++) gf9[e] = 0.0f;
    if (act && (g_pose_b || g_rot_b) && j >= 1)
        for (int e = 0; e < 9; e++) gf9[e] = gfeat_b[m.NB + (j - 1) * 9 + e];
    constexpr int JSP = PSI_POSE_JSP;
    const int nq = m.J * 3;
    const int npart = m.NB > 0 ? min(32, max(1, nthr / m.NB)) : 1;
    const int per = (nq + npart - 1) / npart;
    const bool par_ok = m.NB <= 32, js_pre = g_betas_b && par_ok && per <= JSP && j < npart * m.NB;
    const int bpart = m.NB > 0 ? j / m.NB : 0, bl = j - bpart * m.NB;
    const float *js = pre.js;
    const int cp0 = pre.cp0, cp1 = pre.cp1, par = pre.par;
    float G[12], gJ[3] = {0, 0, 0};
    for (int e = 0; e < 12; e++) G[e] = pre.G[e];
    if (act) {
        const psi_f4 *Ap = (const psi_f4 *)(gA_b + j * 16);
        float gA[12], Jl[3];
        for (int r = 0; r < 3; r++) {
            const psi_f4 aa4 = Ap[r];
            for (int c = 0; c < 4; c++) gA[r * 4 + c] = aa4[c];
        }
        for (int c = 0; c < 3; c++) Jl[c] = pre.Jl[c];
        float go[9], w[3];
        for (int r = 0; r < 3; r++) {
            w[r] = gA[r * 4 + 3];
            for (int c = 0; c < 3; c++) go[r * 3 + c] = gA[r * 4 + c] - w[r] * Jl[c];
        }
        for (int c = 0; c < 3; c++)
            gJ[c] = -(G[0 * 4 + c] * gA[0 * 4 + 3] + G[1 * 4 + c] * gA[1 * 4 + 3] + G[2 * 4 + c] * gA[2 * 4 + 3]);
        for (int r = 0; r < 3; r++) {
            for (int c = 0; c < 3; c++)
                sX[j][r * 3 + c] = go[r * 3 + 0] * G[c * 4 + 0] + go[r * 3 + 1] * G[c * 4 + 1] + go[r * 3 + 2] * G[c * 4 + 2] + w[r] * G[c * 4 + 3];
            sX[j][9 + r] = w[r];
        }
    }
    const float *P = pre.P;
    __syncthreads();
    PSI_PSTOP(21);
    for (int i = j; i < m.n_items * 12; i += nthr) {
        const int it = i / 12, e = i - it * 12;
        const unsigned int d = sItem[it];
        const unsigned char *l = sList + (d & 0xffffu);
        const int cnt = (int)(d >> 16);
        float a = 0.0f;
        for (int q = 0; q < cnt; q++) a += sX[l[q]][e];
        sP[it][e] = a;
    }
    __syncthreads();
    for (int i = j; i < m.J * 12; i += nthr) {
        const int jj = i / 12, e = i - jj * 12;
        float a = 0.0f;
        for (int it = sFirst[jj]; it < sFirst[jj + 1]; it++) a += sP[it][e];
        sS[jj][e] = a;
    }
    __syncthreads();
    PSI_PSTOP(22);
    float gR[9], grel[3] = {0, 0, 0};
    for (int e = 0; e < 9; e++) gR[e] = 0.0f;
    if (act) {
        float gG[12];
        for (int r = 0; r < 3; r++) {
            const float wr = sS[j][9 + r];
            float T[3];
            for (int k = 0; k < 3; k++) T[k] = sS[j][r * 3 + k] - wr * G[k * 4 + 3];
            for (int c = 0; c < 3; c++) gG[r * 4 + c] = T[0] * G[0 * 4 + c] + T[1] * G[1 * 4 + c] + T[2] * G[2 * 4 + c];
            gG[r * 4 + 3] = wr;
        }
        if (par >= 0) {
            for (int r = 0; r < 3; r++) {
                for (int c = 0; c < 3; c++) gR[r * 3 + c] = P[0 * 4 + r] * gG[0 * 4 + c] + P[1 * 4 + r] * gG[1 * 4 + c] + P[2 * 4 + r] * gG[2 * 4 + c];
                grel[r] = P[0 * 4 + r] * gG[0 * 4 + 3] + P[1 * 4 + r] * gG[1 * 4 + 3] + P[2 * 4 + r] * gG[2 * 4 + 3];
            }
        } else {
            for (int r = 0; r < 3; r++) {
                for (int c = 0; c < 3; c++) gR[r * 3 + c] = gG[r * 4 + c];
                grel[r] = gG[r * 4 + 3];
            }
        }
        for (int c = 0; c < 3; c++) sgrel[j][c] = grel[c];
    }
    __syncthreads();
    if (act) {
        for (int c = 0; c < 3; c++) gJ[c] += grel[c];
        for (int ci = cp0; ci < cp1; ci++)
            for (int c = 0; c < 3; c++) gJ[c] -= sgrel[sChild[ci]][c];
        for (int c = 0; c < 3; c++) sgJ[j][c] = gJ[c];
    }
    __syncthreads();
    PSI_PSTOP(23);
    if (g_betas_b) {
        float (&sgb)[32][32] = sh.sgb;
        if (js_pre) {
            float a = 0.0f;
#pragma unroll
            for (int i = 0; i < JSP; i++) {
                const int q = bpart * per + i;
                if (i < per && q < nq) a += (&sgJ[0][0])[q] * js[i];
            }
            sgb[bpart][bl] = a;
        }
        for (int i = j; i < npart * m.NB && par_ok && per > JSP; i += nthr) {
            const int part = i / m.NB, l = i - part * m.NB;
            const int q1 = min(nq, (part + 1) * per);
            float a = 0.0f;
#pragma unroll 8
            for (int q = part * per; q < q1; q++) a += (&sgJ[0][0])[q] * m.J_s[(size_t)q * m.NB + l];
            sgb[part][l] = a;
        }
        __syncthreads();
        for (int l = j; l < m.NB; l += nthr) {
            float a = gfeat_b[l];
            if (par_ok) {
                for (int part = 0; part < npart; part++) a += sgb[part][l];
            } else {
                for (int q = 0; q < nq; q++) a += (&sgJ[0][0])[q] * m.J_s[(size_t)q * m.NB + l];
            }
            g_betas_b[l] = a;
        }
    }
    PSI_PSTOP(24);
    if (act && (g_pose_b || g_rot_b)) {
        if (j >= 1)
            for (int e = 0; e < 9; e++) gR[e] += gf9[e];
        if (g_rot_b)
            for (int e = 0; e < 9; e++) g_rot_b[j * 9 + e] = gR[e];
    }
    if (act && g_pose_b) {
        float x = aa[0] + 1e-8f, y = aa[1] + 1e-8f, z = aa[2] + 1e-8f;
        float th = sqrtf(x * x + y * y + z * z);
        float d[3] = {aa[0] / th, aa[1] / th, aa[2] / th};
        float s = sinf(th), c = cosf(th), c1 = 1.0f - c;
        float K[9] = {0, -d[2], d[1], d[2], 0, -d[0], -d[1], d[0], 0};
        float KK[9];
        for (int r = 0; r < 3; r++)
            for (int q = 0; q < 3; q++) KK[r * 3 + q] = K[r * 3 + 0] * K[0 * 3 + q] + K[r * 3 + 1] * K[1 * 3 + q] + K[r * 3 + 2] * K[2 * 3 + q];
        float gs = 0, gc1 = 0;
        for (int e = 0; e < 9; e++) { gs += gR[e] * K[e]; gc1 += gR[e] * KK[e]; }
        float gK[9];
        for (int r = 0; r < 3; r++)
            for (int q = 0; q < 3; q++) {
                float a = 0;
                for (int k = 0; k < 3; k++) a += gR[r * 3 + k] * K[q * 3 + k] + K[k * 3 + r] * gR[k * 3 + q];
                gK[r * 3 + q] = s * gR[r * 3 + q] + c1 * a;
            }
        float gd[3] = {gK[7] - gK[5], gK[2] - gK[6], gK[3] - gK[1]};
        float gth = gs * c + gc1 * s;
        gth -= (gd[0] * aa[0] + gd[1] * aa[1] + gd[2] * aa[2]) / (th * th);
        float ga[3] = {gd[0] / th + gth * x / th, gd[1] / th + gth * y / th, gd[2] / th + gth * z / th};
        for (int q = 0; q < 3; q++) g_pose_b[j * 3 + q] = ga[q];
    }
}

__device__ __forceinline__ void psi_pose_bwd_body(const LbsDev &m, const float *pose_b,
                                                  const float *__restrict__ Rs, const float *__restrict__ Jls,
                                                  const float *__restrict__ Gs, const float *gA_b, const float *gfeat_b, int b,
                                                  float *g_betas_b, float *g_pose_b, float *g_rot_b)
{
    (void)Rs;
    __shared__ PsiPoseBwdShared sh;
    const PsiPoseBwdPre pre = psi_pose_bwd_issue(m, pose_b, Jls, Gs, b, g_betas_b != nullptr, g_pose_b != nullptr, sh);
    psi_pose_bwd_finish(m, pre, sh, gA_b, gfeat_b, g_betas_b, g_pose_b, g_rot_b);
}


constexpr int PSI_RSPL = 4;
template <int MAXS>
__device__ __forceinline__ void psi_slices_load(const float *__restrict__ p, size_t stride, int n, int s0, float (&v)[MAXS])
{
#pragma unroll
    for (int k = 0; k < MAXS; k++) {
        const int sl = s0 + k * PSI_RSPL;
        v[k] = sl < n ? p[(size_t)sl * stride] : 0.0f;
    }
}
template <int MAXS>
__device__ __forceinline__ float psi_slices_sum(const float (&v)[MAXS], const float *__restrict__ p, size_t stride, int n, int s0)
{
    float a0 = 0, a1 = 0;
#pragma unroll
    for (int k = 0; k < MAXS; k += 2) { a0 += v[k]; a1 += v[k + 1]; }
    float r = a0 + a1;
    for (int sl = s0 + MAXS * PSI_RSPL; sl < n; sl += PSI_RSPL) r += p[(size_t)sl * stride];
    r += __shfl_xor(r, 1, 64);
    r += __shfl_xor(r, 2, 64);
    return r;
}
template <int MAXS>
__device__ __forceinline__ float psi_sum_slices_split(const float *__restrict__ p, size_t stride, int n, int s0)
{
    float v[MAXS];
    psi_slices_load<MAXS>(p, stride, n, s0, v);
    return psi_slices_sum<MAXS>(v, p, stride, n, s0);
}


typedef float psi_f2 __attribute__((ext_vector_type(2)));
constexpr int PSI_SKIN_BLK = 256;

template <int CTRL, int ROWS>
__device__ __forceinline__ float psi_dpp(float x)
{
    return __builtin_bit_cast(float, __builtin_amdgcn_update_dpp(0, __builtin_bit_cast(int, x), CTRL, ROWS, 0xf, false));
}
__device__ __forceinline__ float psi_wave_sum(float x)
{
    x += psi_dpp<0xB1, 0xf>(x);
    x += psi_dpp<0x4E, 0xf>(x);
    x += psi_dpp<0x124, 0xf>(x);
    x += psi_dpp<0x128, 0xf>(x);
    x += psi_dpp<0x142, 0xa>(x);
    x += psi_dpp<0x143, 0xc>(x);
    return __builtin_bit_cast(float, __builtin_amdgcn_readlane(__builtin_bit_cast(int, x), 63));
}

struct psi_p3 { float x, y, z; };
template <class T>
__device__ __forceinline__ T psi_ld(const void *uniform_base, unsigned lane_off)
{
    return *(const T *)((const char *)uniform_base + lane_off);
}
template <class T>
__device__ __forceinline__ void psi_st(void *uniform_base, unsigned lane_off, const T &val)
{
    *(T *)((char *)uniform_base + lane_off) = val;
}

#ifndef PSI_DENSE_UNROLL
#define PSI_DENSE_UNROLL 11
#endif
enum PsiBlendForm { PsiBlendCompact = 0, PsiBlendPipelined = 1 };
static __device__ const psi_f2 psi_zero_row[6] = {};
template <int NB>
__device__ __forceinline__ psi_f2 (*psi_transform_stage())[PSI_JP][6]
{
    __shared__ psi_f2 sA[NB][PSI_JP][6];
    return sA;
}
template <int NB>
struct PsiBlendN {
    psi_f2 st[NB][2];
    float wk[PSI_WNZ];
    unsigned jk[PSI_WNZ / 4];
    const float *As_b[NB];
    typedef psi_f2 (*Staged)[PSI_JP][6];
    __device__ __forceinline__ void issue(const LbsDev &m, const float *__restrict__ As, const int (&b)[NB], int v)
    {
#pragma unroll
        for (int n = 0; n < NB; n++) As_b[n] = As + (size_t)b[n] * m.J * 12;
        if (m.Wc) {
#pragma unroll
            for (int n = 0; n < NB; n++)
#pragma unroll
                for (int q = 0; q < 2; q++) {
                    const int idx = threadIdx.x + q * PSI_SKIN_BLK;
                    st[n][q] = idx < m.J * 6 ? *(const psi_f2 *)(As_b[n] + idx * 2) : (psi_f2){0.0f, 0.0f};
                }
            const __amdgpu_buffer_rsrc_t rc = __builtin_amdgcn_make_buffer_rsrc((void *)m.Wc, 0, PSI_WNZ * m.Vpad * 4, 0x00020000);
            const __amdgpu_buffer_rsrc_t rj = __builtin_amdgcn_make_buffer_rsrc((void *)m.Wj, 0, PSI_WNZ / 4 * m.Vpad * 4, 0x00020000);
#pragma unroll
            for (int k = 0; k < PSI_WNZ; k++)
                wk[k] = __builtin_bit_cast(float, __builtin_amdgcn_raw_buffer_load_b32(rc, (unsigned)v * 4u, (unsigned)(k * m.Vpad) * 4u, 0));
#pragma unroll
            for (int k = 0; k < PSI_WNZ / 4; k++) jk[k] = __builtin_amdgcn_raw_buffer_load_b32(rj, (unsigned)v * 4u, (unsigned)(k * m.Vpad) * 4u, 0);
        }
    }
    __device__ __forceinline__ Staged commit(const LbsDev &m)
    {
        const Staged sA = psi_transform_stage<NB>();
        if (!m.Wc) return sA;
#pragma unroll
        for (int n = 0; n < NB; n++)
#pragma unroll
            for (int q = 0; q < 2; q++) {
                const int idx = threadIdx.x + q * PSI_SKIN_BLK;
                if (idx < m.J * 6) (&sA[n][0][0])[idx] = st[n][q];
            }
        __syncthreads();
        return sA;
    }
    template <PsiBlendForm FORM = PsiBlendCompact>
    __device__ __forceinline__ void blend(const LbsDev &m, Staged sA, int v, psi_f2 (&T2)[NB][6]) const
    {
#pragma unroll
        for (int n = 0; n < NB; n++)
#pragma unroll
            for (int e = 0; e < 6; e++) T2[n][e] = (psi_f2){0.0f, 0.0f};
        if (m.Wc) {
#pragma unroll
            for (int k = 0; k < PSI_WNZ; k++) {
                if (__builtin_amdgcn_ballot_w64(wk[k] != 0.0f) == 0) break;
                psi_f2 w2 = {wk[k], wk[k]};
                const int jj = (jk[k >> 2] >> (8 * (k & 3))) & 0xff;
#pragma unroll
                for (int n = 0; n < NB; n++)
#pragma unroll
                    for (int e = 0; e < 6; e++) T2[n][e] = __builtin_elementwise_fma(w2, sA[n][jj][e], T2[n][e]);
            }
            return;
        }
        const psi_f2 *Ab[NB];
#pragma unroll
        for (int n = 0; n < NB; n++) Ab[n] = (const psi_f2 *)As_b[n];
        const __amdgpu_buffer_rsrc_t rw = __builtin_amdgcn_make_buffer_rsrc((void *)m.WTt, 0, PSI_JP * m.Vpad * 4, 0x00020000);
        const unsigned v4 = (unsigned)(v & 63) * 4u;
        const unsigned tile_off = (unsigned)__builtin_amdgcn_readfirstlane(v >> 6) * (unsigned)(PSI_JP * 64 * 4);
        auto wload = [&](int k, unsigned ro) { return __builtin_bit_cast(float, __builtin_amdgcn_raw_buffer_load_b32(rw, v4 + k * 256, ro, 0)); };
        unsigned ro = tile_off;
        if (FORM == PsiBlendCompact || m.J > 60) {
            constexpr int GJ = PSI_DENSE_UNROLL;
            static_assert(GJ * 256 <= 4096, "joint offsets of a group must fit the load's 12-bit immediate");
            float w[GJ];
#pragma unroll
            for (int k = 0; k < GJ; k++) w[k] = wload(k, ro);
            auto fma6 = [&](float wj, int j) {
                psi_f2 w2 = {wj, wj};
#pragma unroll
                for (int n = 0; n < NB; n++)
#pragma unroll
                    for (int e = 0; e < 6; e++) T2[n][e] = __builtin_elementwise_fma(w2, Ab[n][j * 6 + e], T2[n][e]);
            };
            int j0 = 0;
#pragma nounroll
            for (; j0 + GJ <= m.J; j0 += GJ) {
                ro += j0 + GJ < m.J ? GJ * 256 : 0;
#pragma unroll
                for (int k = 0; k < GJ; k++) {
                    fma6(w[k], j0 + k);
                    w[k] = wload(k, ro);
                }
            }
#pragma unroll
            for (int k = 0; k < GJ; k++)
                if (j0 + k < m.J) fma6(w[k], j0 + k);
        } else {
            constexpr int G2 = 12, PS = NB == 1 ? 2 : 1;
            static_assert(G2 % (2 * PS) == 0, "a group is a whole number of set pairs");
            float w[G2];
#pragma unroll
            for (int k = 0; k < G2; k++) w[k] = wload(k, ro);
            psi_f2 P0[NB][PS][6], P1[NB][PS][6];
            auto aload = [&](psi_f2 (&P)[NB][PS][6], int j, int ts, int jn) {
#pragma unroll
                for (int n = 0; n < NB; n++)
#pragma unroll
                    for (int q = 0; q < PS; q++) {
                        const psi_f2 *row = j + q >= ts && j + q >= jn ? psi_zero_row : Ab[n] + (j + q) * 6;
#pragma unroll
                        for (int e = 0; e < 6; e++) P[n][q][e] = row[e];
                    }
            };
            auto fmas = [&](const psi_f2 (&P)[NB][PS][6], const float *wk) {
#pragma unroll
                for (int q = 0; q < PS; q++) {
                    const psi_f2 w2 = {wk[q], wk[q]};
#pragma unroll
                    for (int n = 0; n < NB; n++)
#pragma unroll
                        for (int e = 0; e < 6; e++) T2[n][e] = __builtin_elementwise_fma(w2, P[n][q][e], T2[n][e]);
                }
            };
            const int ngroups = (m.J + G2 - 1) / G2;
            aload(P0, 0, (ngroups - 1) * G2, m.J);
            auto group = [&](int g, int ts, int jn) {
                const int j0 = g * G2;
                ro += g + 1 < ngroups ? G2 * 256 : 0;
#pragma unroll
                for (int k = 0; k < G2; k += 2 * PS) {
                    aload(P1, j0 + k + PS, ts, jn);
                    __builtin_amdgcn_sched_barrier(0);
                    fmas(P0, w + k);
#pragma unroll
                    for (int q = 0; q < PS; q++) w[k + q] = wload(k + q, ro);
                    __builtin_amdgcn_sched_barrier(0);
                    aload(P0, j0 + k + 2 * PS, ts, jn);
                    __builtin_amdgcn_sched_barrier(0);
                    fmas(P1, w + k + PS);
#pragma unroll
                    for (int q = 0; q < PS; q++) w[k + PS + q] = wload(k + PS + q, ro);
                    __builtin_amdgcn_sched_barrier(0);
                }
            };
            if (m.J == 55) {
#pragma unroll
                for (int g = 0; g < 5; g++) group(g, 4 * G2, 55);
            } else if (ngroups == 5) {
#pragma unroll
                for (int g = 0; g < 5; g++) group(g, 4 * G2, m.J);
            } else {
#pragma nounroll
                for (int g = 0; g < ngroups; g++) group(g, (ngroups - 1) * G2, m.J);
            }
        }
    }
};
typedef PsiBlendN<1> PsiBlend;

__device__ __forceinline__ float psi_dot3p(float a, float b, float c, float d, float x, float y, float z)
{
    return __builtin_fmaf(c, z, __builtin_fmaf(b, y, a * x)) + d;
}
__device__ __forceinline__ float psi_dot3(float a, float b, float c, float x, float y, float z)
{
    return __builtin_fmaf(c, z, __builtin_fmaf(b, y, a * x));
}

struct PsiSkinNoEpilogue {
    __device__ __forceinline__ void backward(int, int, unsigned, const psi_f2 (&)[6], const float *) {}
    __device__ __forceinline__ void store(float *verts, size_t body_off, int, int, unsigned v12, float x, float y, float z) const
    {
        if (verts) psi_st(verts + body_off, v12, psi_p3{x, y, z});
    }
    __device__ __forceinline__ void vertex(int, int, int, float, float, float, bool) {}
    __device__ __forceinline__ void finish(int, int, int, int) {}
};

template <int NB, PsiBlendForm FORM, class Epi>
__device__ __forceinline__ void psi_skin_fwd_body(const LbsDev &m, const float *__restrict__ As, const float *__restrict__ v_posed,
                                                  const float *__restrict__ transl, const float *__restrict__ cam_ext, int B,
                                                  float *__restrict__ verts, Epi &epi, int vblock, int b0, int nvb)
{
    const int v = vblock * PSI_SKIN_BLK + threadIdx.x;
    const bool live = v < m.V;
    const unsigned v12 = (unsigned)v * 12u;
    int bs[NB];
#pragma unroll
    for (int n = 0; n < NB; n++) bs[n] = min(b0 + n, B - 1);
    PsiBlendN<NB> bl;
    bl.issue(m, As, bs, v);
    psi_p3 pp[NB];
#pragma unroll
    for (int n = 0; n < NB; n++) pp[n] = psi_ld<psi_p3>(v_posed + (size_t)bs[n] * m.Npad, v12);
    psi_f2 T2[NB][6];
    bl.template blend<FORM>(m, bl.commit(m), v, T2);
#pragma unroll
    for (int n = 0; n < NB; n++) {
        const int b = bs[n];
        const bool on = n == 0 || b0 + n < B;
        const float px = pp[n].x, py = pp[n].y, pz = pp[n].z;
        float x = psi_dot3p(T2[n][0].x, T2[n][0].y, T2[n][1].x, T2[n][1].y, px, py, pz);
        float y = psi_dot3p(T2[n][2].x, T2[n][2].y, T2[n][3].x, T2[n][3].y, px, py, pz);
        float z = psi_dot3p(T2[n][4].x, T2[n][4].y, T2[n][5].x, T2[n][5].y, px, py, pz);
        if (transl) {
            x += transl[(size_t)b * 3 + 0];
            y += transl[(size_t)b * 3 + 1];
            z += transl[(size_t)b * 3 + 2];
        }
        if (cam_ext) {
            const float *C = cam_ext + (size_t)b * 16;
            float X = psi_dot3p(C[0], C[1], C[2], C[3], x, y, z);
            float Y = psi_dot3p(C[4], C[5], C[6], C[7], x, y, z);
            float Z = psi_dot3p(C[8], C[9], C[10], C[11], x, y, z);
            x = X; y = Y; z = Z;
        }
        epi.vertex(n, b, v, x, y, z, live && on);
        if (on) epi.backward(n, b, v12, T2[n], cam_ext ? cam_ext + (size_t)b * 16 : nullptr);
        if (live && on) epi.store(verts, (size_t)b * m.V * 3, b, v, v12, x, y, z);
    }
#pragma unroll
    for (int n = 0; n < NB; n++) {
        if (n > 0) __syncthreads();
        if (n == 0 || b0 + n < B) epi.finish(n, bs[n], vblock, nvb);
    }
}

template <class Epi, int NB = 1>
__global__ __launch_bounds__(PSI_SKIN_BLK, 6) void psi_skin_fwd_kernel(LbsDev m, const float *__restrict__ As, const float *__restrict__ v_posed,
                                                                     const float *__restrict__ transl, const float *__restrict__ cam_ext,
                                                                     int B, float *__restrict__ verts, Epi epi)
{
    psi_skin_fwd_body<NB, PsiBlendPipelined>(m, As, v_posed, transl, cam_ext, B, verts, epi, (int)blockIdx.x, (int)blockIdx.y * NB, (int)gridDim.x);
}

struct PsiGradFromMemory {
    const float *g_verts;
    int V;
    __device__ __forceinline__ void prepare(int, int) {}
    __device__ __forceinline__ void load(int b, int v, float &gx, float &gy, float &gz) const
    {
        const float *g = g_verts + ((size_t)b * V + v) * 3;
        gx = g[0]; gy = g[1]; gz = g[2];
    }
    struct Pre { float g[3]; };
    __device__ __forceinline__ Pre issue(int b, int v, bool live) const
    {
        Pre p = {{0.0f, 0.0f, 0.0f}};
        if (live) load(b, v, p.g[0], p.g[1], p.g[2]);
        return p;
    }
    __device__ __forceinline__ void issue_late(Pre &, int) const {}
    __device__ __forceinline__ void take(const Pre &p, int, int, float &gx, float &gy, float &gz) const { gx = p.g[0]; gy = p.g[1]; gz = p.g[2]; }
};

template <class Src, PsiBlendForm FORM = PsiBlendCompact>
__global__ __launch_bounds__(PSI_SKIN_BLK, 6) void psi_skin_bwd_v_kernel(LbsDev m, const float *__restrict__ As, Src src,
                                                                       const float *__restrict__ cam_ext, int B, float *__restrict__ gl,
                                                                       float *__restrict__ g_vp, float *__restrict__ gt_part)
{
    const int v = blockIdx.x * PSI_SKIN_BLK + threadIdx.x;
    const int b = blockIdx.y;
    PSI_TRACE(30, 30);
    PSI_SSTOP(11);
    typename Src::Pre pre = src.issue(b, v, v < m.V);
    PsiBlend bl;
    const int bs1[1] = {b};
    bl.issue(m, As, bs1, v);
    src.issue_late(pre, b);
    PSI_SSTOP(12);
    psi_f2 T2n[1][6];
    bl.template blend<FORM>(m, bl.commit(m), v, T2n);
    const psi_f2 (&T2)[6] = T2n[0];
    PSI_SSTOP(13);
    src.prepare(b, 1);
    PSI_SSTOP(14);
    __shared__ float sh[PSI_SKIN_BLK / 64][3];
    float lx = 0, ly = 0, lz = 0;
    if (v < m.V) {
        float gx, gy, gz;
        src.take(pre, b, v, gx, gy, gz);
        if (cam_ext) {
            const float *C = cam_ext + (size_t)b * 16;
            lx = psi_dot3(C[0], C[4], C[8], gx, gy, gz);
            ly = psi_dot3(C[1], C[5], C[9], gx, gy, gz);
            lz = psi_dot3(C[2], C[6], C[10], gx, gy, gz);
        } else {
            lx = gx; ly = gy; lz = gz;
        }
    }
    {
        psi_st(gl + (size_t)b * m.Npad, (unsigned)v * 12u, psi_p3{lx, ly, lz});
        psi_st(g_vp + (size_t)b * m.Npad, (unsigned)v * 12u,
               psi_p3{psi_dot3(T2[0].x, T2[2].x, T2[4].x, lx, ly, lz), psi_dot3(T2[0].y, T2[2].y, T2[4].y, lx, ly, lz),
                      psi_dot3(T2[1].x, T2[3].x, T2[5].x, lx, ly, lz)});
    }
    float sx = psi_wave_sum(lx), sy = psi_wave_sum(ly), sz = psi_wave_sum(lz);
    if ((threadIdx.x & 63) == 0) {
        sh[threadIdx.x >> 6][0] = sx;
        sh[threadIdx.x >> 6][1] = sy;
        sh[threadIdx.x >> 6][2] = sz;
    }
    __syncthreads();
    if (threadIdx.x < 3) {
        float s = 0;
        for (int ww = 0; ww < PSI_SKIN_BLK / 64; ww++) s += sh[ww][threadIdx.x];
        gt_part[((size_t)blockIdx.x * B + b) * 4 + threadIdx.x] = s;
    }
}


constexpr int PSI_SKIN_MB = 8;
constexpr int PSI_SKIN_MB_MIN_B = 128;

template <bool COMPRESSED>
struct PsiLaneWeights;
template <>
struct PsiLaneWeights<false> {
    psi_f2 w2[PSI_JP / 2];
    __device__ __forceinline__ void load(const LbsDev &m, int v)
    {
        __amdgpu_buffer_rsrc_t rs = __builtin_amdgcn_make_buffer_rsrc((void *)m.WT, 0, PSI_JP * m.Vpad * 4, 0x00020000);
#pragma unroll
        for (int j = 0; j < PSI_JP / 2; j++) {
            w2[j].x = __builtin_bit_cast(float, __builtin_amdgcn_raw_buffer_load_b32(rs, v * 4, (2 * j) * m.Vpad * 4, 0));
            w2[j].y = __builtin_bit_cast(float, __builtin_amdgcn_raw_buffer_load_b32(rs, v * 4, (2 * j + 1) * m.Vpad * 4, 0));
        }
    }
    __device__ __forceinline__ void blend(const LbsDev &m, const psi_f2 (*sA)[6], psi_f2 (&T2)[6]) const
    {
#pragma unroll
        for (int e = 0; e < 6; e++) T2[e] = (psi_f2){0.0f, 0.0f};
#pragma unroll
        for (int c = 0; c < PSI_JP / 8; c++) {
            if (c * 8 < m.J) {
#pragma unroll
                for (int jj = c * 4; jj < c * 4 + 4; jj++) {
#pragma unroll
                    for (int e = 0; e < 6; e++) {
                        const psi_f2 a = sA[2 * jj][e];
                        asm("v_pk_fma_f32 %0, %1, %2, %0 op_sel:[0,0,0] op_sel_hi:[0,1,1]" : "+v"(T2[e]) : "v"(w2[jj]), "v"(a));
                    }
#pragma unroll
                    for (int e = 0; e < 6; e++) {
                        const psi_f2 a = sA[2 * jj + 1][e];
                        asm("v_pk_fma_f32 %0, %1, %2, %0 op_sel:[1,0,0] op_sel_hi:[1,1,1]" : "+v"(T2[e]) : "v"(w2[jj]), "v"(a));
                    }
                }
            }
        }
    }
};
template <>
struct PsiLaneWeights<true> {
    float wk[PSI_WNZ];
    unsigned jk[PSI_WNZ / 4];
    __device__ __forceinline__ void load(const LbsDev &m, int v)
    {
#pragma unroll
        for (int k = 0; k < PSI_WNZ; k++) wk[k] = m.Wc[(size_t)k * m.Vpad + v];
#pragma unroll
        for (int k = 0; k < PSI_WNZ / 4; k++) jk[k] = m.Wj[(size_t)k * m.Vpad + v];
    }
    __device__ __forceinline__ void blend(const LbsDev &, const psi_f2 (*sA)[6], psi_f2 (&T2)[6]) const
    {
#pragma unroll
        for (int e = 0; e < 6; e++) T2[e] = (psi_f2){0.0f, 0.0f};
#pragma unroll
        for (int k = 0; k < PSI_WNZ; k++) {
            if (__builtin_amdgcn_ballot_w64(wk[k] != 0.0f) == 0) break;
            psi_f2 w2 = {wk[k], wk[k]};
            const int jj = (jk[k >> 2] >> (8 * (k & 3))) & 0xff;
#pragma unroll
            for (int e = 0; e < 6; e++) T2[e] = __builtin_elementwise_fma(w2, sA[jj][e], T2[e]);
        }
    }
};

__device__ __forceinline__ void psi_stage_transforms(const LbsDev &m, const float *__restrict__ As, int b, psi_f2 (*sA)[6])
{
    for (int idx = threadIdx.x; idx < PSI_JP * 6; idx += PSI_SKIN_BLK)
        sA[idx / 6][idx % 6] = idx < m.J * 6 ? *(const psi_f2 *)(As + ((size_t)b * m.J) * 12 + idx * 2) : (psi_f2){0.0f, 0.0f};
}

template <class Src, bool COMPRESSED>
__global__ __launch_bounds__(PSI_SKIN_BLK, 4) void psi_skin_bwd_v_mb_kernel(LbsDev m, const float *__restrict__ As, Src src,
                                                                          const float *__restrict__ cam_ext, int B, float *__restrict__ gl,
                                                                          float *__restrict__ g_vp, float *__restrict__ gt_part)
{
    const int v = blockIdx.x * PSI_SKIN_BLK + threadIdx.x;
    const int b0 = blockIdx.y * PSI_SKIN_MB;
    src.prepare(b0, min(PSI_SKIN_MB, B - b0));
    __shared__ psi_f2 sA[2][PSI_JP][6];
    __shared__ float sh[2][PSI_SKIN_BLK / 64][3];
    PsiLaneWeights<COMPRESSED> lw;
    lw.load(m, v);
    const int nb = min(PSI_SKIN_MB, B - b0);
#pragma nounroll
    for (int bb = 0; bb < nb; bb++) {
        const int b = b0 + bb;
        psi_stage_transforms(m, As, b, sA[bb & 1]);
        float lx = 0, ly = 0, lz = 0;
        if (v < m.V) {
            float gx, gy, gz;
            src.load(b, v, gx, gy, gz);
            if (cam_ext) {
                const float *C = cam_ext + (size_t)b * 16;
                lx = psi_dot3(C[0], C[4], C[8], gx, gy, gz);
                ly = psi_dot3(C[1], C[5], C[9], gx, gy, gz);
                lz = psi_dot3(C[2], C[6], C[10], gx, gy, gz);
            } else {
                lx = gx; ly = gy; lz = gz;
            }
        }
        float sx = psi_wave_sum(lx), sy = psi_wave_sum(ly), sz = psi_wave_sum(lz);
        if ((threadIdx.x & 63) == 0) {
            sh[bb & 1][threadIdx.x >> 6][0] = sx;
            sh[bb & 1][threadIdx.x >> 6][1] = sy;
            sh[bb & 1][threadIdx.x >> 6][2] = sz;
        }
        __syncthreads();
        psi_f2 T2[6];
        lw.blend(m, sA[bb & 1], T2);
        {
            float *o = gl + (size_t)b * m.Npad + (size_t)v * 3;
            o[0] = lx; o[1] = ly; o[2] = lz;
            float *p = g_vp + (size_t)b * m.Npad + (size_t)v * 3;
            p[0] = psi_dot3(T2[0].x, T2[2].x, T2[4].x, lx, ly, lz);
            p[1] = psi_dot3(T2[0].y, T2[2].y, T2[4].y, lx, ly, lz);
            p[2] = psi_dot3(T2[1].x, T2[3].x, T2[5].x, lx, ly, lz);
        }
        if (threadIdx.x < 3) {
            float s = 0;
            for (int ww = 0; ww < PSI_SKIN_BLK / 64; ww++) s += sh[bb & 1][ww][threadIdx.x];
            gt_part[((size_t)blockIdx.x * B + b) * 4 + threadIdx.x] = s;
        }
    }
}


template <class Src>
static inline void psi_launch_skin_bwd_v_mb(const LbsDev &m, const float *As, Src src, const float *cam_ext, int B, float *gl, float *g_vp,
                                            float *gt_part, hipStream_t st)
{
    const dim3 grid(m.Vpad / PSI_SKIN_BLK, (B + PSI_SKIN_MB - 1) / PSI_SKIN_MB);
    if (m.Wc)
        hipLaunchKernelGGL((psi_skin_bwd_v_mb_kernel<Src, true>), grid, dim3(PSI_SKIN_BLK), 0, st, m, As, src, cam_ext, B, gl, g_vp, gt_part);
    else
        hipLaunchKernelGGL((psi_skin_bwd_v_mb_kernel<Src, false>), grid, dim3(PSI_SKIN_BLK), 0, st, m, As, src, cam_ext, B, gl, g_vp, gt_part);
}
```

Measured before the change: 12140.

## Defer off-critical-path head work into cross-block wait windows

Adds an ORD template mode, on by default, that reorders the clustered head kernels. In the forward head, the loss partials and the body/hand pose vector setup move after the cross-block hx exchange, so they run while the last block waits for its peers. In the backward head, the pose backward is split into a rotation part and a betas/pose/PCA part. The second part runs during the hx_gh1 wait, and the inspection stores move to the end of the kernel. It also turns many multiply-adds into explicit fmaf, which can change rounding slightly and adds template variants and code complexity.

```diff
diff --git a/psi-release_amd/csrc/fit.hip b/psi-release_amd/csrc/fit.hip
--- a/psi-release_amd/csrc/fit.hip
+++ b/psi-release_amd/csrc/fit.hip
@@ -258,9 +258,10 @@
     return __uint_as_float((unsigned)w);
 }
 
-template <int C, bool LINKS_IN_HEAD>
+template <int C, bool LINKS_IN_HEAD, bool ORD>
 __global__ __launch_bounds__(HB) void head_fwd_kernel(FitDev f, PsiLbsView lv)
 {
+    constexpr bool LATE = ORD && C > 1;
     constexpr int NS = NH / C;
     constexpr int NQ = NS / 4;
     constexpr int KSPL = HB / NQ;
@@ -304,7 +305,7 @@
     }
     __syncthreads();
     HSTOP(1);
-    if (c == 0) {
+    auto loss_partials = [&]() {
         float dr = t < XD ? fabsf(f.xhr[(size_t)b * XD + t] - sx[t]) : 0.0f;
         float sr = block_sum(dr, red);
         float dz = t < NZ ? sx[19 + t] * sx[19 + t] : 0.0f;
@@ -313,8 +314,8 @@
             f.recpart[b] = sr;
             f.vppart[b] = sz;
         }
-    }
-    if (last) {
+    };
+    auto body_vector_part = [&]() {
         if (t >= 64 && t < 64 + 9) {
             int e = 66 + (t - 64);
             spose[e] = f.pose_mean[e];
@@ -328,6 +329,10 @@
             spose[75 + e] = a + f.pose_mean[75 + e];
         }
         psi_pose_fwd_rest(lv.m, sbetas, sJ);
+    };
+    if (!LATE) {
+        if (c == 0) loss_partials();
+        if (last) body_vector_part();
     }
     HSTOP(2);
     const float *z = sx + 19;
@@ -386,27 +391,35 @@
     }
     __syncthreads();
     HSTOP(5);
-    if (t < 128) {
+    {
         float a = 0.0f;
-        const float *p = (const float *)part3;
-#pragma unroll
-        for (int ks = 0; ks < KS3; ks++) a += p[ks * 128 + t];
+        if (t < 128) {
+            const float *p = (const float *)part3;
+#pragma unroll
+            for (int ks = 0; ks < KS3; ks++) a += p[ks * 128 + t];
+        }
         if (C == 1) {
-            so6[t] = a + b3v;
+            if (t < 128) so6[t] = a + b3v;
         } else if (!last) {
-            hx_put(f.hx_o6 + ((size_t)b * C + c) * 128 + t, a, tag);
+            if (t < 128) hx_put(f.hx_o6 + ((size_t)b * C + c) * 128 + t, a, tag);
+            if (LATE && c == 0) loss_partials();
+            return;
         } else {
-            unsigned long long *p8 = f.hx_o6 + (size_t)b * C * 128 + t;
+            unsigned long long *p8 = f.hx_o6 + (size_t)b * C * 128 + (t & 127);
             unsigned long long w[C - 1 ? C - 1 : 1];
-#pragma unroll
-            for (int cc = 0; cc < C - 1; cc++) w[cc] = hx_peek(p8 + cc * 128);
-            float o = b3v;
-#pragma unroll
-            for (int cc = 0; cc < C - 1; cc++) o += hx_value(p8 + cc * 128, w[cc], tag, f.hx_err);
-            so6[t] = o + a;
-        }
-    }
-    if (C > 1 && !last) return;
+            if (t < 128) {
+#pragma unroll
+                for (int cc = 0; cc < C - 1; cc++) w[cc] = hx_peek(p8 + cc * 128);
+            }
+            if (LATE) body_vector_part();
+            if (t < 128) {
+                float o = b3v;
+#pragma unroll
+                for (int cc = 0; cc < C - 1; cc++) o += hx_value(p8 + cc * 128, w[cc], tag, f.hx_err);
+                so6[t] = o + a;
+            }
+        }
+    }
     __syncthreads();
     HSTOP(6);
     if (t < NJ6) f.o6[(size_t)b * 128 + t] = so6[t];
@@ -1246,7 +1259,7 @@
     }
 };
 
-template <int C, bool ADAM>
+template <int C, bool ADAM, bool ORD>
 __global__ __launch_bounds__(HB) void head_bwd_adam_kernel(FitDev f, PsiLbsView lv, float *__restrict__ g_out)
 {
     constexpr int NS = NH / C, NQ = NS / 4;
@@ -1299,18 +1312,50 @@
             bc2_sqrt = (float)sqrt(bc2);
         }
     }
-    psi_pose_bwd_body(lv.m, f.pose + (size_t)b * f.J * 3, lv.R, lv.Jl, lv.G, lv.gA + (size_t)b * PSI_JP * 16, lv.gfeat + (size_t)b * lv.m.Kpad, b,
-                      sgbetas, sgpose, sgrot);
+    __shared__ PsiPoseBwdShared psh;
+    const float *gfeat_b = lv.gfeat + (size_t)b * lv.m.Kpad;
+    PsiPoseBwdPre pre = psi_pose_bwd_issue(lv.m, f.pose + (size_t)b * f.J * 3, lv.Jl, lv.G, b, !ORD, !ORD, psh);
+    if (ORD) {
+        float gR[9];
+        psi_pose_bwd_rot(lv.m, pre, psh, lv.gA + (size_t)b * PSI_JP * 16, gfeat_b, true, sgrot, gR);
+    } else {
+        psi_pose_bwd_finish(lv.m, pre, psh, lv.gA + (size_t)b * PSI_JP * 16, gfeat_b, sgbetas, sgpose, sgrot);
+    }
+    auto inspection = [&]() {
+        for (int i = t; i < f.J * 9; i += HB) f.g_rot[(size_t)b * f.J * 9 + i] = sgrot[i];
+        for (int i = t; i < f.J * 3; i += HB) f.g_pose[(size_t)b * f.J * 3 + i] = sgpose[i];
+        if (t < f.NB) f.g_betas[(size_t)b * f.NB + t] = sgbetas[t];
+    };
+    auto adam_operands = [&]() {
+        const int i = t - 64;
+        const bool pca = i >= 0 && i < 2 * f.ncomp, left = i < f.ncomp;
+        const int ii = left ? i : i - f.ncomp;
+        float cv[45];
+        if (pca) {
+            const float *comp = (left ? f.lhc : f.rhc) + ii * 45;
+#pragma unroll
+            for (int e = 0; e < 45; e++) cv[e] = comp[e];
+        }
+        float gR[9];
+        for (int e = 0; e < 9; e++) gR[e] = t < lv.m.J ? sgrot[t * 9 + e] : 0.0f;
+        psi_pose_bwd_rest(lv.m, pre, psh, gfeat_b, gR, sgbetas, sgpose);
+        __syncthreads();
+        if (pca) {
+            const float *gp = sgpose + (left ? 75 : 120);
+            float a = 0;
+#pragma unroll
+            for (int e = 0; e < 45; e++) a = fmaf(cv[e], gp[e], a);
+            sgx[(left ? 51 : 63) + ii] = a;
+        } else if (t >= 160 && t < 160 + 10) {
+            sgx[9 + (t - 160)] = sgbetas[t - 160];
+        }
+    };
     const float *x = f.x + (size_t)b * XD;
     if (t < XD) { sx[t] = x[t]; sgx[t] = 0.0f; }
     if (t < 128) sg6[t] = 0.0f;
     __syncthreads();
     TSTOP(2);
-    if (c == 0) {
-        for (int i = t; i < f.J * 9; i += HB) f.g_rot[(size_t)b * f.J * 9 + i] = sgrot[i];
-        for (int i = t; i < f.J * 3; i += HB) f.g_pose[(size_t)b * f.J * 3 + i] = sgpose[i];
-        if (t < f.NB) f.g_betas[(size_t)b * f.NB + t] = sgbetas[t];
-    }
+    if (!ORD && c == 0) inspection();
     if (t == 0) {
         float g6[6];
         gs_backward(sx + 3, sgrot, g6);
@@ -1319,17 +1364,17 @@
         float g6[6];
         gs_backward(o6v, sgrot + t * 9, g6);
         for (int i = 0; i < 6; i++) sg6[(t - 1) * 6 + i] = g6[i];
-    } else if (t >= 64 && t < 64 + 2 * f.ncomp) {
+    } else if (!ORD && t >= 64 && t < 64 + 2 * f.ncomp) {
         int i = t - 64;
         const float *comp = i < f.ncomp ? f.lhc : f.rhc;
         int ii = i < f.ncomp ? i : i - f.ncomp;
         const float *gp = sgpose + (i < f.ncomp ? 75 : 120);
         float a = 0;
-        for (int e = 0; e < 45; e++) a += comp[ii * 45 + e] * gp[e];
+        for (int e = 0; e < 45; e++) a = fmaf(comp[ii * 45 + e], gp[e], a);
         sgx[(i < f.ncomp ? 51 : 63) + ii] = a;
     } else if (t >= 128 && t < 128 + 3) {
         sgx[t - 128] = gtv;
-    } else if (t >= 160 && t < 160 + 10) {
+    } else if (!ORD && t >= 160 && t < 160 + 10) {
         sgx[9 + (t - 160)] = sgbetas[t - 160];
     }
     __syncthreads();
@@ -1342,6 +1387,7 @@
         for (int o = o0 + PRE3; o < o1; o++) a += *(const f4 *)(w3 + (size_t)o * NH) * sg6[o];
         part4[os3 * NQ + og3] = a;
     }
+    if (ORD && last) psi_pose_bwd_issue_rest(lv.m, f.pose + (size_t)b * f.J * 3, true, true, pre);
     __syncthreads();
     if (t < NS) {
         float a = 0.0f;
@@ -1376,6 +1422,7 @@
         for (int q = 1; q < KQ; q++) a += p[q * NH + t];
         if (C == 1) {
             sga1[t] = a * (h1[t] > 0.0f ? 1.0f : 0.2f);
+            if (ORD) adam_operands();
         } else if (!last) {
             hx_put(f.hx_gh1 + ((size_t)b * C + c) * NH + t, a, tag);
             return;
@@ -1384,6 +1431,7 @@
             unsigned long long w[C - 1 ? C - 1 : 1];
 #pragma unroll
             for (int cc = 0; cc < C - 1; cc++) w[cc] = hx_peek(p8 + (size_t)cc * NH);
+            if (ORD) adam_operands();
             float o = 0.0f;
 #pragma unroll
             for (int cc = 0; cc < C - 1; cc++) o += hx_value(p8 + (size_t)cc * NH, w[cc], tag, f.hx_err);
@@ -1414,6 +1462,7 @@
     if (C > 1 && t == 0) f.hx_epoch[f.B + b] = tag;
     if (!ADAM) {
         if (t < XD) g_out[(size_t)b * XD + t] = sgx[t];
+        if (ORD) inspection();
         return;
     }
     if (ta >= 0 && ta < XD) {
@@ -1430,6 +1479,7 @@
         float denom = sqrtf(v) / bc2_sqrt + f.eps;
         f.x[o] = sx[ta] - step_size * (m / denom);
     }
+    if (ORD) inspection();
 }
 
 __global__ void sdf_to_cells_kernel(const float *__restrict__ src, float *__restrict__ dst, int D)
@@ -1469,7 +1519,7 @@
 constexpr int GRAPH_UNROLL = PSI_GRAPH_UNROLL;
 
 struct FitKnobs {
-    bool split_scene, keep_verts, no_fused_bwd, sdf_linear, scene_skin_first, bwdv_mb, no_pen_skip, bwd_pf1, chain_in_head;
+    bool split_scene, keep_verts, no_fused_bwd, sdf_linear, scene_skin_first, bwdv_mb, no_pen_skip, bwd_pf1, chain_in_head, tail_order0;
     int head_cluster, skin_nb, ska_nbody, search_lanes, search_spw;
 #ifdef PSI_HEAD_STOPS
     int head_stop, tail_stop, skin_stop;
@@ -1487,6 +1537,7 @@
     k.no_pen_skip = is("PSI_FIT_PEN_SKIP", '0');
     k.bwd_pf1 = is("PSI_FIT_BWD_PF", '1');
     k.chain_in_head = is("PSI_FIT_CHAIN_IN_HEAD", '1');
+    k.tail_order0 = is("PSI_FIT_TAIL_ORDER", '0');
     k.sdf_linear = is("PSI_SDF_LINEAR", '1');
     k.scene_skin_first = is("PSI_SCENE_ORDER", '1');
     k.bwdv_mb = is("PSI_BWDV_MB", '1');
@@ -1671,15 +1722,15 @@
     bool dp_no_graph;
 };
 
-template <bool LINKS_IN_HEAD>
+template <bool LINKS_IN_HEAD, bool ORD>
 static void launch_head_fwd(const FitDev &f, const PsiLbsView &lv, hipStream_t st)
 {
     const dim3 g(f.B * f.hc), blk(HB);
     switch (f.hc) {
-    case 8: hipLaunchKernelGGL((head_fwd_kernel<8, LINKS_IN_HEAD>), g, blk, 0, st, f, lv); break;
-    case 4: hipLaunchKernelGGL((head_fwd_kernel<4, LINKS_IN_HEAD>), g, blk, 0, st, f, lv); break;
-    case 2: hipLaunchKernelGGL((head_fwd_kernel<2, LINKS_IN_HEAD>), g, blk, 0, st, f, lv); break;
-    default: hipLaunchKernelGGL((head_fwd_kernel<1, true>), g, blk, 0, st, f, lv); break;
+    case 8: hipLaunchKernelGGL((head_fwd_kernel<8, LINKS_IN_HEAD, ORD>), g, blk, 0, st, f, lv); break;
+    case 4: hipLaunchKernelGGL((head_fwd_kernel<4, LINKS_IN_HEAD, ORD>), g, blk, 0, st, f, lv); break;
+    case 2: hipLaunchKernelGGL((head_fwd_kernel<2, LINKS_IN_HEAD, ORD>), g, blk, 0, st, f, lv); break;
+    default: hipLaunchKernelGGL((head_fwd_kernel<1, true, true>), g, blk, 0, st, f, lv); break;
     }
 }
 
@@ -1688,24 +1739,33 @@
     const FitDev &f = e->d;
     const PsiChainPlan &cp = e->mode.chain;
     const bool role = cp.n_links_wg > 0 && f.hc > 1;
-    if (role) launch_head_fwd<false>(f, e->lv, st);
-    else launch_head_fwd<true>(f, e->lv, st);
+    const bool ord = !e->knobs.tail_order0;
+    if (role && ord) launch_head_fwd<false, true>(f, e->lv, st);
+    else if (role) launch_head_fwd<false, false>(f, e->lv, st);
+    else if (ord) launch_head_fwd<true, true>(f, e->lv, st);
+    else launch_head_fwd<true, false>(f, e->lv, st);
     PSI_CHECK_LAUNCH("head_fwd_kernel");
     psi_mark("head_fwd_kernel", st);
     return role ? psi_lbs_blend_forward_links(e->lbs, f.B, e->lbs_ws, cp.n_links_wg, cp.bodies_per_wave, st)
                 : psi_lbs_blend_forward(e->lbs, f.B, e->lbs_ws, st);
 }
 
-template <bool ADAM>
-static void launch_head_bwd(const FitDev &f, const PsiLbsView &lv, float *g_out, hipStream_t st)
+template <bool ADAM, bool ORD>
+static void launch_head_bwd_ord(const FitDev &f, const PsiLbsView &lv, float *g_out, hipStream_t st)
 {
     const dim3 g(f.B * f.hc), blk(HB);
     switch (f.hc) {
-    case 8: hipLaunchKernelGGL((head_bwd_adam_kernel<8, ADAM>), g, blk, 0, st, f, lv, g_out); break;
-    case 4: hipLaunchKernelGGL((head_bwd_adam_kernel<4, ADAM>), g, blk, 0, st, f, lv, g_out); break;
-    case 2: hipLaunchKernelGGL((head_bwd_adam_kernel<2, ADAM>), g, blk, 0, st, f, lv, g_out); break;
-    default: hipLaunchKernelGGL((head_bwd_adam_kernel<1, ADAM>), g, blk, 0, st, f, lv, g_out); break;
-    }
+    case 8: hipLaunchKernelGGL((head_bwd_adam_kernel<8, ADAM, ORD>), g, blk, 0, st, f, lv, g_out); break;
+    case 4: hipLaunchKernelGGL((head_bwd_adam_kernel<4, ADAM, ORD>), g, blk, 0, st, f, lv, g_out); break;
+    case 2: hipLaunchKernelGGL((head_bwd_adam_kernel<2, ADAM, ORD>), g, blk, 0, st, f, lv, g_out); break;
+    default: hipLaunchKernelGGL((head_bwd_adam_kernel<1, ADAM, ORD>), g, blk, 0, st, f, lv, g_out); break;
+    }
+}
+template <bool ADAM>
+static void launch_head_bwd(const psi_fit_engine *e, float *g_out, hipStream_t st)
+{
+    if (e->knobs.tail_order0) launch_head_bwd_ord<ADAM, false>(e->d, e->lv, g_out, st);
+    else launch_head_bwd_ord<ADAM, true>(e->d, e->lv, g_out, st);
 }
 
 enum class FitStats {
@@ -1832,7 +1892,7 @@
     hipLaunchKernelGGL(fit_reduce_kernel, dim3(psi_cdiv(nred * PSI_RSPL, 256)), dim3(256), 0, st, f, e->lv, stats);
     PSI_CHECK_LAUNCH("fit_reduce_kernel");
     psi_mark("reduce_partials_kernel", st);
-    launch_head_bwd<true>(f, e->lv, nullptr, st);
+    launch_head_bwd<true>(e, nullptr, st);
     PSI_CHECK_LAUNCH("head_bwd_adam_kernel");
     psi_mark("head_bwd_adam_kernel", st);
     return 0;
@@ -1865,7 +1925,7 @@
     psi_mark("skin_bwd_v_grad_kernel", st);
     int rc = psi_lbs_backward_joint_parts(e->lbs, f.B, e->lbs_ws, f.g_transl, st);
     if (rc) return rc;
-    launch_head_bwd<true>(f, e->lv, nullptr, st);
+    launch_head_bwd<true>(e, nullptr, st);
     PSI_CHECK_LAUNCH("head_bwd_adam_kernel");
     psi_mark("head_bwd_adam_kernel", st);
     return 0;
@@ -2371,7 +2431,7 @@
     PSI_CHECK_LAUNCH("skin_bwd_v_kernel");
     int rc = psi_lbs_backward_joint_parts(e->lbs, f.B, e->lbs_ws, f.g_transl, st);
     if (rc) return rc;
-    launch_head_bwd<false>(f, e->lv, d_grad_x75, st);
+    launch_head_bwd<false>(e, d_grad_x75, st);
     PSI_CHECK_LAUNCH("head_bwd_kernel");
     return 0;
 }
diff --git a/psi-release_amd/csrc/lbs_device.h b/psi-release_amd/csrc/lbs_device.h
--- a/psi-release_amd/csrc/lbs_device.h
+++ b/psi-release_amd/csrc/lbs_device.h
@@ -224,13 +224,10 @@
     float sgb[32][32];
 };
 
-__device__ __forceinline__ PsiPoseBwdPre psi_pose_bwd_issue(const LbsDev &m, const float *pose_b, const float *__restrict__ Jls,
-                                                            const float *__restrict__ Gs, int b, bool want_betas, bool want_pose,
-                                                            PsiPoseBwdShared &sh)
+__device__ __forceinline__ void psi_pose_bwd_issue_rest(const LbsDev &m, const float *pose_b, bool want_betas, bool want_pose, PsiPoseBwdPre &p)
 {
     const int j = threadIdx.x, nthr = blockDim.x;
     const bool act = j < m.J;
-    PsiPoseBwdPre p;
     for (int e = 0; e < 3; e++) p.aa[e] = 0.0f;
     if (act && want_pose)
         for (int e = 0; e < 3; e++) p.aa[e] = pose_b[j * 3 + e];
@@ -246,6 +243,16 @@
             const int q = bpart * per + i;
             if (i < per && q < nq) p.js[i] = m.J_s[(size_t)q * m.NB + bl];
         }
+}
+
+__device__ __forceinline__ PsiPoseBwdPre psi_pose_bwd_issue(const LbsDev &m, const float *pose_b, const float *__restrict__ Jls,
+                                                            const float *__restrict__ Gs, int b, bool want_betas, bool want_pose,
+                                                            PsiPoseBwdShared &sh)
+{
+    const int j = threadIdx.x, nthr = blockDim.x;
+    const bool act = j < m.J;
+    PsiPoseBwdPre p;
+    psi_pose_bwd_issue_rest(m, pose_b, want_betas, want_pose, p);
     p.cp0 = act ? m.child_ptr[j] : 0;
     p.cp1 = act ? m.child_ptr[j + 1] : 0;
     p.par = act ? m.parents[j] : -1;
@@ -273,8 +280,8 @@
     return p;
 }
 
-__device__ __forceinline__ void psi_pose_bwd_finish(const LbsDev &m, const PsiPoseBwdPre &pre, PsiPoseBwdShared &sh, const float *gA_b,
-                                                    const float *gfeat_b, float *g_betas_b, float *g_pose_b, float *g_rot_b)
+__device__ __forceinline__ void psi_pose_bwd_rot(const LbsDev &m, const PsiPoseBwdPre &pre, PsiPoseBwdShared &sh, const float *gA_b,
+                                                 const float *gfeat_b, bool want_rot, float *g_rot_b, float (&gR)[9])
 {
     const int j = threadIdx.x, nthr = blockDim.x;
     const bool act = j < m.J;
@@ -288,17 +295,9 @@
     float (&sgrel)[PSI_JP][3] = sh.sgrel;
     int (&sChild)[PSI_JP] = sh.sChild;
     float gf9[9];
-    const float *aa = pre.aa;
     for (int e = 0; e < 9; e++) gf9[e] = 0.0f;
-    if (act && (g_pose_b || g_rot_b) && j >= 1)
+    if (act && want_rot && j >= 1)
         for (int e = 0; e < 9; e++) gf9[e] = gfeat_b[m.NB + (j - 1) * 9 + e];
-    constexpr int JSP = PSI_POSE_JSP;
-    const int nq = m.J * 3;
-    const int npart = m.NB > 0 ? min(32, max(1, nthr / m.NB)) : 1;
-    const int per = (nq + npart - 1) / npart;
-    const bool par_ok = m.NB <= 32, js_pre = g_betas_b && par_ok && per <= JSP && j < npart * m.NB;
-    const int bpart = m.NB > 0 ? j / m.NB : 0, bl = j - bpart * m.NB;
-    const float *js = pre.js;
     const int cp0 = pre.cp0, cp1 = pre.cp1, par = pre.par;
     float G[12], gJ[3] = {0, 0, 0};
     for (int e = 0; e < 12; e++) G[e] = pre.G[e];
@@ -313,13 +312,13 @@
         float go[9], w[3];
         for (int r = 0; r < 3; r++) {
             w[r] = gA[r * 4 + 3];
-            for (int c = 0; c < 3; c++) go[r * 3 + c] = gA[r * 4 + c] - w[r] * Jl[c];
+            for (int c = 0; c < 3; c++) go[r * 3 + c] = fmaf(-w[r], Jl[c], gA[r * 4 + c]);
         }
         for (int c = 0; c < 3; c++)
-            gJ[c] = -(G[0 * 4 + c] * gA[0 * 4 + 3] + G[1 * 4 + c] * gA[1 * 4 + 3] + G[2 * 4 + c] * gA[2 * 4 + 3]);
+            gJ[c] = -fmaf(G[2 * 4 + c], gA[2 * 4 + 3], fmaf(G[1 * 4 + c], gA[1 * 4 + 3], G[0 * 4 + c] * gA[0 * 4 + 3]));
         for (int r = 0; r < 3; r++) {
             for (int c = 0; c < 3; c++)
-                sX[j][r * 3 + c] = go[r * 3 + 0] * G[c * 4 + 0] + go[r * 3 + 1] * G[c * 4 + 1] + go[r * 3 + 2] * G[c * 4 + 2] + w[r] * G[c * 4 + 3];
+                sX[j][r * 3 + c] = fmaf(w[r], G[c * 4 + 3], fmaf(go[r * 3 + 2], G[c * 4 + 2], fmaf(go[r * 3 + 1], G[c * 4 + 1], go[r * 3 + 0] * G[c * 4 + 0])));
             sX[j][9 + r] = w[r];
         }
     }
@@ -344,21 +343,21 @@
     }
     __syncthreads();
     PSI_PSTOP(22);
-    float gR[9], grel[3] = {0, 0, 0};
+    float grel[3] = {0, 0, 0};
     for (int e = 0; e < 9; e++) gR[e] = 0.0f;
     if (act) {
         float gG[12];
         for (int r = 0; r < 3; r++) {
             const float wr = sS[j][9 + r];
             float T[3];
-            for (int k = 0; k < 3; k++) T[k] = sS[j][r * 3 + k] - wr * G[k * 4 + 3];
-            for (int c = 0; c < 3; c++) gG[r * 4 + c] = T[0] * G[0 * 4 + c] + T[1] * G[1 * 4 + c] + T[2] * G[2 * 4 + c];
+            for (int k = 0; k < 3; k++) T[k] = fmaf(-wr, G[k * 4 + 3], sS[j][r * 3 + k]);
+            for (int c = 0; c < 3; c++) gG[r * 4 + c] = fmaf(T[2], G[2 * 4 + c], fmaf(T[1], G[1 * 4 + c], T[0] * G[0 * 4 + c]));
             gG[r * 4 + 3] = wr;
         }
         if (par >= 0) {
             for (int r = 0; r < 3; r++) {
-                for (int c = 0; c < 3; c++) gR[r * 3 + c] = P[0 * 4 + r] * gG[0 * 4 + c] + P[1 * 4 + r] * gG[1 * 4 + c] + P[2 * 4 + r] * gG[2 * 4 + c];
-                grel[r] = P[0 * 4 + r] * gG[0 * 4 + 3] + P[1 * 4 + r] * gG[1 * 4 + 3] + P[2 * 4 + r] * gG[2 * 4 + 3];
+                for (int c = 0; c < 3; c++) gR[r * 3 + c] = fmaf(P[2 * 4 + r], gG[2 * 4 + c], fmaf(P[1 * 4 + r], gG[1 * 4 + c], P[0 * 4 + r] * gG[0 * 4 + c]));
+                grel[r] = fmaf(P[2 * 4 + r], gG[2 * 4 + 3], fmaf(P[1 * 4 + r], gG[1 * 4 + 3], P[0 * 4 + r] * gG[0 * 4 + 3]));
             }
         } else {
             for (int r = 0; r < 3; r++) {
@@ -377,6 +376,28 @@
     }
     __syncthreads();
     PSI_PSTOP(23);
+    if (act && want_rot) {
+        if (j >= 1)
+            for (int e = 0; e < 9; e++) gR[e] += gf9[e];
+        if (g_rot_b)
+            for (int e = 0; e < 9; e++) g_rot_b[j * 9 + e] = gR[e];
+    }
+}
+
+__device__ __forceinline__ void psi_pose_bwd_rest(const LbsDev &m, const PsiPoseBwdPre &pre, PsiPoseBwdShared &sh, const float *gfeat_b,
+                                                  const float (&gR)[9], float *g_betas_b, float *g_pose_b)
+{
+    const int j = threadIdx.x, nthr = blockDim.x;
+    const bool act = j < m.J;
+    float (&sgJ)[PSI_JP][3] = sh.sgJ;
+    const float *aa = pre.aa;
+    constexpr int JSP = PSI_POSE_JSP;
+    const int nq = m.J * 3;
+    const int npart = m.NB > 0 ? min(32, max(1, nthr / m.NB)) : 1;
+    const int per = (nq + npart - 1) / npart;
+    const bool par_ok = m.NB <= 32, js_pre = g_betas_b && par_ok && per <= JSP && j < npart * m.NB;
+    const int bpart = m.NB > 0 ? j / m.NB : 0, bl = j - bpart * m.NB;
+    const float *js = pre.js;
     if (g_betas_b) {
         float (&sgb)[32][32] = sh.sgb;
         if (js_pre) {
@@ -384,7 +405,7 @@
 #pragma unroll
             for (int i = 0; i < JSP; i++) {
                 const int q = bpart * per + i;
-                if (i < per && q < nq) a += (&sgJ[0][0])[q] * js[i];
+                if (i < per && q < nq) a = fmaf((&sgJ[0][0])[q], js[i], a);
             }
             sgb[bpart][bl] = a;
         }
@@ -393,7 +414,7 @@
             const int q1 = min(nq, (part + 1) * per);
             float a = 0.0f;
 #pragma unroll 8
-            for (int q = part * per; q < q1; q++) a += (&sgJ[0][0])[q] * m.J_s[(size_t)q * m.NB + l];
+            for (int q = part * per; q < q1; q++) a = fmaf((&sgJ[0][0])[q], m.J_s[(size_t)q * m.NB + l], a);
             sgb[part][l] = a;
         }
         __syncthreads();
@@ -402,42 +423,44 @@
             if (par_ok) {
                 for (int part = 0; part < npart; part++) a += sgb[part][l];
             } else {
-                for (int q = 0; q < nq; q++) a += (&sgJ[0][0])[q] * m.J_s[(size_t)q * m.NB + l];
+                for (int q = 0; q < nq; q++) a = fmaf((&sgJ[0][0])[q], m.J_s[(size_t)q * m.NB + l], a);
             }
             g_betas_b[l] = a;
         }
     }
     PSI_PSTOP(24);
-    if (act && (g_pose_b || g_rot_b)) {
-        if (j >= 1)
-            for (int e = 0; e < 9; e++) gR[e] += gf9[e];
-        if (g_rot_b)
-            for (int e = 0; e < 9; e++) g_rot_b[j * 9 + e] = gR[e];
-    }
     if (act && g_pose_b) {
         float x = aa[0] + 1e-8f, y = aa[1] + 1e-8f, z = aa[2] + 1e-8f;
-        float th = sqrtf(x * x + y * y + z * z);
+        float th = sqrtf(fmaf(z, z, fmaf(y, y, x * x)));
         float d[3] = {aa[0] / th, aa[1] / th, aa[2] / th};
         float s = sinf(th), c = cosf(th), c1 = 1.0f - c;
         float K[9] = {0, -d[2], d[1], d[2], 0, -d[0], -d[1], d[0], 0};
         float KK[9];
         for (int r = 0; r < 3; r++)
-            for (int q = 0; q < 3; q++) KK[r * 3 + q] = K[r * 3 + 0] * K[0 * 3 + q] + K[r * 3 + 1] * K[1 * 3 + q] + K[r * 3 + 2] * K[2 * 3 + q];
+            for (int q = 0; q < 3; q++) KK[r * 3 + q] = fmaf(K[r * 3 + 2], K[2 * 3 + q], fmaf(K[r * 3 + 1], K[1 * 3 + q], K[r * 3 + 0] * K[0 * 3 + q]));
         float gs = 0, gc1 = 0;
-        for (int e = 0; e < 9; e++) { gs += gR[e] * K[e]; gc1 += gR[e] * KK[e]; }
+        for (int e = 0; e < 9; e++) { gs = fmaf(gR[e], K[e], gs); gc1 = fmaf(gR[e], KK[e], gc1); }
         float gK[9];
         for (int r = 0; r < 3; r++)
             for (int q = 0; q < 3; q++) {
                 float a = 0;
-                for (int k = 0; k < 3; k++) a += gR[r * 3 + k] * K[q * 3 + k] + K[k * 3 + r] * gR[k * 3 + q];
-                gK[r * 3 + q] = s * gR[r * 3 + q] + c1 * a;
+                for (int k = 0; k < 3; k++) a = fmaf(K[k * 3 + r], gR[k * 3 + q], fmaf(gR[r * 3 + k], K[q * 3 + k], a));
+                gK[r * 3 + q] = fmaf(c1, a, s * gR[r * 3 + q]);
             }
         float gd[3] = {gK[7] - gK[5], gK[2] - gK[6], gK[3] - gK[1]};
-        float gth = gs * c + gc1 * s;
-        gth -= (gd[0] * aa[0] + gd[1] * aa[1] + gd[2] * aa[2]) / (th * th);
+        float gth = fmaf(gc1, s, gs * c);
+        gth -= fmaf(gd[2], aa[2], fmaf(gd[1], aa[1], gd[0] * aa[0])) / (th * th);
         float ga[3] = {gd[0] / th + gth * x / th, gd[1] / th + gth * y / th, gd[2] / th + gth * z / th};
         for (int q = 0; q < 3; q++) g_pose_b[j * 3 + q] = ga[q];
     }
+}
+
+__device__ __forceinline__ void psi_pose_bwd_finish(const LbsDev &m, const PsiPoseBwdPre &pre, PsiPoseBwdShared &sh, const float *gA_b,
+                                                    const float *gfeat_b, float *g_betas_b, float *g_pose_b, float *g_rot_b)
+{
+    float gR[9];
+    psi_pose_bwd_rot(m, pre, sh, gA_b, gfeat_b, g_pose_b || g_rot_b, g_rot_b, gR);
+    psi_pose_bwd_rest(m, pre, sh, gfeat_b, gR, g_betas_b, g_pose_b);
 }
 
 __device__ __forceinline__ void psi_pose_bwd_body(const LbsDev &m, const float *pose_b,
```

Result: no change. 12140 (median of 4 runs) (+0.1%).
